# vlongle/pixie

Hardware: AMD Instinct MI355X
Metric: voxels/s (128^3 U-Net fwd) + MPM particle-steps/s (higher is better)
Workload: dtype f32 (operands split fp16 hi+lo, 3 f16 MFMAs/product, fp32 accumulate); 1 GPU; 128^3x64 feature grid -> SegmentationUNet+RegressionUNet forward (+argmax/one-hot combine), 1 scene per GPU per step; grid=128, feature_channels=64, parallelism=scene-parallel x1, executor=c+hip_graph

## Files before the change

### include/pixie_hip.h

```cpp
#ifndef PIXIE_HIP_H
#define PIXIE_HIP_H

#include <stdint.h>

#ifdef __cplusplus
extern "C" {
#endif

const char* pixie_last_error(void);
const char* pixie_build_arch(void);

typedef struct pixie_mpm pixie_mpm;

int pixie_mpm_create(pixie_mpm** out, int n_particles, int n_grid, double grid_lim);
int pixie_mpm_destroy(pixie_mpm* h);
int pixie_mpm_regrid(pixie_mpm* h, int n_grid, double grid_lim, void* stream);

int pixie_mpm_set_field(pixie_mpm* h, const char* name, const void* d_src, int64_t count, void* stream);
int pixie_mpm_get_field(pixie_mpm* h, const char* name, void* d_dst, int64_t count, void* stream);
int pixie_mpm_fill_field(pixie_mpm* h, const char* name, double value, void* stream);

int pixie_mpm_set_scalar(pixie_mpm* h, const char* key, double value);
int pixie_mpm_get_scalar(pixie_mpm* h, const char* key, double* value);

int pixie_mpm_update_mass(pixie_mpm* h, void* stream);
int pixie_mpm_finalize_mu_lam(pixie_mpm* h, int with_bulk, void* stream);
int pixie_mpm_apply_additional_params(pixie_mpm* h, const double point[3], const double size[3], double E,
                                      double nu, double density, int material, void* stream);
int pixie_mpm_apply_additional_params_batch(pixie_mpm* h, int64_t n_boxes, const float* d_boxes, const float* d_params,
                                            const int32_t* d_material, void* stream);

enum { PIXIE_BC_SURFACE = 0, PIXIE_BC_CUBOID = 1, PIXIE_BC_BBOX = 2 };
typedef struct pixie_bc_desc {
    int32_t type;
    int32_t surface_type;
    int32_t reset;
    int32_t pad_;
    double point[3], size[3], velocity[3], normal[3];
    double start_time, end_time, friction;
} pixie_bc_desc;
int pixie_mpm_add_bc(pixie_mpm* h, const pixie_bc_desc* bc);

enum { PIXIE_PM_IMPULSE = 0, PIXIE_PM_TRANSLATION = 1, PIXIE_PM_ROTATION = 2 };
typedef struct pixie_pmod_desc {
    int32_t type;
    int32_t pad_;
    double point[3], size[3];
    double force[3];
    double velocity[3];
    double normal[3], h1[3], h2[3];
    double half_height, radius, rotation_scale, translation_scale;
    double start_time, end_time;
} pixie_pmod_desc;
int pixie_mpm_add_particle_modifier(pixie_mpm* h, const pixie_pmod_desc* pm, void* stream);

int pixie_mpm_step(pixie_mpm* h, double dt, int n_substeps, void* stream);

typedef struct pixie_mpm_batch pixie_mpm_batch;
typedef struct pixie_batch_sched {
    double dt;
    int32_t steps_per_chunk;
    int32_t n_chunks;
    int32_t n_out;
    int32_t pad_;
    double shift[3], scale, mean[3];
    double inv_rotation[9];
    float* d_pos;
    float* d_cov;
} pixie_batch_sched;
int pixie_mpm_batch_create(pixie_mpm_batch** out, pixie_mpm* const* handles, int n_handles);
int pixie_mpm_batch_step(pixie_mpm_batch* b, double dt, int n_substeps, void* stream);
int pixie_mpm_batch_run(pixie_mpm_batch* b, const pixie_batch_sched* per_scene, int n_scenes, void* stream);
typedef struct pixie_batch_splat_out {
    float* d_log_scale;
    float* d_quat;
} pixie_batch_splat_out;
int pixie_mpm_batch_run_splats(pixie_mpm_batch* b, const pixie_batch_sched* per_scene, const pixie_batch_splat_out* splats ,
                               int n_scenes, void* stream);
int pixie_mpm_batch_destroy(pixie_mpm_batch* b);

int pixie_mpm_export_cov(pixie_mpm* h, float* d_cov , void* stream);
int pixie_mpm_export_R(pixie_mpm* h, float* d_R , void* stream);
int pixie_mpm_export_frame(pixie_mpm* h, int n_out, const double shift[3], double scale, const double mean[3],
                           const double inv_rotation[9], float* d_pos , float* d_cov ,
                           void* stream);
int pixie_splat_from_cov(const float* d_cov , int64_t n, float* d_log_scale , float* d_quat ,
                         void* stream);
int pixie_mpm_export_frame_splats(pixie_mpm* h, int n_out, const double shift[3], double scale, const double mean[3],
                                  const double inv_rotation[9], float* d_pos , float* d_cov ,
                                  float* d_log_scale , float* d_quat , void* stream);
int pixie_mpm_out_of_bounds(pixie_mpm* h, int64_t* count, void* stream);


typedef struct pixie_conv_desc {
    const float* d_in0; int32_t c0;
    const float* d_in1; int32_t c1;
    int32_t in_d, in_h, in_w;
    int32_t upsample;
    int32_t stride;
    int32_t ksize;
    const float* d_pro_a; const float* d_pro_b;
    const float* d_gamma; const float* d_beta;
    int32_t act;
    const float* d_w; const float* d_bias;
    int32_t c_out;
    const float* d_residual;
    float* d_out;
    const void* d_w16;
    const uint32_t* d_in_amax0; const uint32_t* d_in_amax1;
    float in_bound;
    float* d_out_stats;
    uint32_t* d_out_amax;
    void* d_workspace;
    int32_t out_d, out_h, out_w;
    const float* d_skip_in0; int32_t skip_c0;
    const float* d_skip_in1; int32_t skip_c1;
    const void* d_skip_w16; const float* d_skip_bias;
    const uint32_t* d_skip_amax0; const uint32_t* d_skip_amax1;
    int32_t w16_subpixel;
} pixie_conv_desc;

int pixie_conv_cout_padded(int c_out);
int pixie_conv_pack_weights(const float* d_w_oidhw, float* d_w_packed, int c_out, int c_in, int ksize, void* stream);
int64_t pixie_conv_packed16_bytes(int c_out, int c_in, int ksize);
int pixie_conv_pack_weights_f16x2(const float* d_w_oidhw, void* d_packed, int c_out, int c_in, int ksize, void* stream);
int64_t pixie_conv_subpixel_bytes(int c_out, int c_in);
int pixie_conv_pack_weights_subpixel(const float* d_w_oidhw, void* d_packed, int c_out, int c_in, void* stream);
int pixie_conv3d_forward(const pixie_conv_desc* desc, void* stream);
int64_t pixie_conv_stats_floats(const pixie_conv_desc* desc);
int64_t pixie_conv_workspace_bytes(const pixie_conv_desc* desc);
int pixie_stats_finalize(const float* d_stats, const pixie_conv_desc* desc, double* d_sums, void* stream);
int pixie_conv_skip_foldable(const pixie_conv_desc* desc);

int pixie_channel_sums(const float* d_x, int channels, int64_t spatial, double* d_sums, void* stream);
int pixie_channel_stats(const float* d_x, int channels, int64_t spatial, double* d_sums, uint32_t* d_amax, void* stream);
int pixie_tensor_amax(const float* d_x, int64_t count, uint32_t* d_slot, void* stream);
int pixie_norm_finalize(const double* d_sums, int channels, int64_t spatial, int mode, int groups, double eps,
                        const float* d_weight, const float* d_bias, float* d_a, float* d_b, void* stream);

int pixie_attention_forward(const float* d_qkv, float* d_out, int channels, int tokens, void* stream);

int pixie_channel_affine(const float* d_x, const float* d_a, const float* d_b, float* d_y, int channels,
                         int64_t spatial, void* stream);

int pixie_voxel_grid_to_ncdhw(const void* d_feat_dhwc_f16, int d, int h, int w, int channels, float* d_out_cdhw, void* stream);

int pixie_projector_conv0(const void* d_feat_dhwc_f16, int64_t voxels, int channels, int n_networks, const void* const* d_w16,
                          const float* const* d_bias, float* const* d_out, int c_out, void* stream);

int pixie_pack_fields(const float* d_cont, const int32_t* d_seg_pred, int64_t n_scenes, int64_t spatial, void* d_wire, int64_t wire_bytes,
                      void* stream);

int pixie_combine_predictions(const float* d_logits, int num_classes, const float* d_cont, int64_t spatial,
                              float* d_combined, int32_t* d_argmax , void* stream);

int pixie_combine_class_ids(const int32_t* d_seg_pred, int num_classes, const float* d_cont, int64_t spatial, float* d_combined,
                            void* stream);

typedef struct pixie_unet pixie_unet;
typedef struct pixie_unet_config {
    int32_t feature_channels, cond_dim, model_channels, num_res_blocks;
    int32_t n_channel_mult; int32_t channel_mult[8];
    int32_t n_attention_resolutions; int32_t attention_resolutions[8];
    int32_t grid_size;
    int32_t out_channels;
    int32_t precision;
} pixie_unet_config;

int pixie_unet_create(pixie_unet** out, const pixie_unet_config* cfg);
int pixie_unet_destroy(pixie_unet* h);
int pixie_unet_param_count(const pixie_unet* h);
int pixie_unet_param_info(const pixie_unet* h, int index, const char** key, int64_t* numel, int32_t* ndim, int64_t shape[5]);
int pixie_unet_set_param(pixie_unet* h, const char* key, const float* d_values, int64_t numel);
int64_t pixie_unet_workspace_bytes(pixie_unet* h, int d, int hh, int w);
int pixie_unet_forward(pixie_unet* h, const float* d_feat, const float* d_proj0, int d, int hh, int w, float* d_out,
                       void* d_workspace, int64_t workspace_bytes, void* stream);
int pixie_unet_set_option(pixie_unet* h, const char* key, int value);

typedef struct pixie_field_desc {
    const float* d_pred;
    const uint8_t* d_mask;
    const float* d_axis_x; const float* d_axis_y; const float* d_axis_z;
    int32_t n_classes, d, h, w;
    double min_spacing;
    double density_min, density_max, E_min, E_max, nu_min, nu_max;
} pixie_field_desc;
int pixie_field_to_particles(const pixie_field_desc* field, const float* d_pos, int n, int k, double nn_distance_threshold,
                             int weighted, int default_material, int default_part_label, float* d_density, float* d_E,
                             float* d_nu, int32_t* d_material, int32_t* d_part_label, float* d_conf, float* d_nearest,
                             void* d_scratch, void* stream);

int pixie_unscale_prediction(const float* d_pred, int channels, int64_t spatial, double density_min, double density_max,
                             double E_min, double E_max, double nu_min, double nu_max, float* d_out, void* stream);
int64_t pixie_field_points_scratch_bytes(const pixie_field_desc* field);
int pixie_field_points(const pixie_field_desc* field, int64_t capacity, float* d_xyz , float* d_density, float* d_E,
                       float* d_nu, int32_t* d_material, float* d_conf, int64_t* d_count, void* d_scratch, void* stream);

int pixie_dbscan_roots(const float* d_pos_sorted, const int32_t* d_orig_index, const int32_t* d_cell_start, int n, int nx, int ny, int nz,
                       const double lo[3], double cell_size, double eps, int min_samples, int32_t* d_core_scratch,
                       int32_t* d_parent_scratch, int32_t* d_root, void* stream);

int pixie_fill_densify(const float* d_pos, const float* d_opacity, const float* d_cov6, int n, int grid_n, double grid_dx,
                       int32_t* d_grid_count, float* d_grid_density, void* stream);
int pixie_fill_dense_cells(int32_t* d_grid_count, const float* d_grid_density, int grid_n, double grid_dx, double density_thres,
                           int max_particles_per_cell, float* d_new_particles , int64_t max_samples,
                           uint64_t* d_counter, uint32_t seed, void* stream);
int pixie_fill_internal_cells(int32_t* d_grid_count, const float* d_grid_density, int grid_n, double grid_dx, int max_particles_per_cell,
                              int exclude_dir, int ray_cast_dir, double threshold, float* d_new_particles, int64_t max_samples,
                              uint64_t* d_counter, uint32_t seed, void* stream);
int pixie_particle_volume(const float* d_pos, int n, int grid_n, double grid_dx, int32_t* d_grid_count_scratch, float* d_vol, void* stream);
int pixie_nearest_particle(const float* d_pos, int n, const float* d_new_pos, int n_new, int32_t* d_nearest, void* stream);

#ifdef PIXIE_DIAG
int pixie_mpm_phase(pixie_mpm* h, int phase, double dt, void* stream);

int pixie_mpm_kernel_times(pixie_mpm* h, double* particle_ms, double* grid_ms, int64_t* n_launches);

int pixie_conv_kernel_variant(const pixie_conv_desc* desc, int* slices);

int pixie_conv_tile_geometry(const pixie_conv_desc* desc, int32_t out[10]);
#endif

#ifdef __cplusplus
}
#endif
#endif
```

### pixie_amd/_lib.py

```python
from __future__ import annotations

import ctypes as C
import os

_HERE = os.path.dirname(os.path.abspath(__file__))
LIB_PATH = os.path.join(_HERE, "libpixie_hip.so")
DIAG_LIB_PATH = os.path.join(_HERE, "libpixie_hip_diag.so")


class PixieHipError(RuntimeError):
    pass


class BCDesc(C.Structure):
    _fields_ = [("type", C.c_int32), ("surface_type", C.c_int32), ("reset", C.c_int32), ("pad_", C.c_int32),
                ("point", C.c_double * 3), ("size", C.c_double * 3), ("velocity", C.c_double * 3),
                ("normal", C.c_double * 3), ("start_time", C.c_double), ("end_time", C.c_double),
                ("friction", C.c_double)]


class PModDesc(C.Structure):
    _fields_ = [("type", C.c_int32), ("pad_", C.c_int32),
                ("point", C.c_double * 3), ("size", C.c_double * 3), ("force", C.c_double * 3),
                ("velocity", C.c_double * 3), ("normal", C.c_double * 3), ("h1", C.c_double * 3),
                ("h2", C.c_double * 3), ("half_height", C.c_double), ("radius", C.c_double),
                ("rotation_scale", C.c_double), ("translation_scale", C.c_double),
                ("start_time", C.c_double), ("end_time", C.c_double)]


class ConvDesc(C.Structure):
    _fields_ = [("d_in0", C.c_void_p), ("c0", C.c_int32),
                ("d_in1", C.c_void_p), ("c1", C.c_int32),
                ("in_d", C.c_int32), ("in_h", C.c_int32), ("in_w", C.c_int32),
                ("upsample", C.c_int32), ("stride", C.c_int32), ("ksize", C.c_int32),
                ("d_pro_a", C.c_void_p), ("d_pro_b", C.c_void_p),
                ("d_gamma", C.c_void_p), ("d_beta", C.c_void_p),
                ("act", C.c_int32),
                ("d_w", C.c_void_p), ("d_bias", C.c_void_p),
                ("c_out", C.c_int32),
                ("d_residual", C.c_void_p), ("d_out", C.c_void_p),
                ("d_w16", C.c_void_p), ("d_in_amax0", C.c_void_p), ("d_in_amax1", C.c_void_p),
                ("in_bound", C.c_float),
                ("d_out_stats", C.c_void_p), ("d_out_amax", C.c_void_p),
                ("d_workspace", C.c_void_p),
                ("out_d", C.c_int32), ("out_h", C.c_int32), ("out_w", C.c_int32),
                ("d_skip_in0", C.c_void_p), ("skip_c0", C.c_int32),
                ("d_skip_in1", C.c_void_p), ("skip_c1", C.c_int32),
                ("d_skip_w16", C.c_void_p), ("d_skip_bias", C.c_void_p),
                ("d_skip_amax0", C.c_void_p), ("d_skip_amax1", C.c_void_p),
                ("w16_subpixel", C.c_int32)]


class UNetConfigC(C.Structure):
    _fields_ = [("feature_channels", C.c_int32), ("cond_dim", C.c_int32), ("model_channels", C.c_int32), ("num_res_blocks", C.c_int32),
                ("n_channel_mult", C.c_int32), ("channel_mult", C.c_int32 * 8),
                ("n_attention_resolutions", C.c_int32), ("attention_resolutions", C.c_int32 * 8),
                ("grid_size", C.c_int32), ("out_channels", C.c_int32), ("precision", C.c_int32)]


class BatchSched(C.Structure):
    _fields_ = [("dt", C.c_double), ("steps_per_chunk", C.c_int32), ("n_chunks", C.c_int32), ("n_out", C.c_int32), ("pad_", C.c_int32),
                ("shift", C.c_double * 3), ("scale", C.c_double), ("mean", C.c_double * 3), ("inv_rotation", C.c_double * 9),
                ("d_pos", C.c_void_p), ("d_cov", C.c_void_p)]


class BatchSplatOut(C.Structure):
    _fields_ = [("d_log_scale", C.c_void_p), ("d_quat", C.c_void_p)]


class FieldDesc(C.Structure):
    _fields_ = [("d_pred", C.c_void_p), ("d_mask", C.c_void_p),
                ("d_axis_x", C.c_void_p), ("d_axis_y", C.c_void_p), ("d_axis_z", C.c_void_p),
                ("n_classes", C.c_int32), ("d", C.c_int32), ("h", C.c_int32), ("w", C.c_int32),
                ("min_spacing", C.c_double),
                ("density_min", C.c_double), ("density_max", C.c_double), ("E_min", C.c_double), ("E_max", C.c_double),
                ("nu_min", C.c_double), ("nu_max", C.c_double)]


_VP, _I, _I64, _D, _S = C.c_void_p, C.c_int, C.c_int64, C.c_double, C.c_char_p
_D3 = C.POINTER(C.c_double)
SIGNATURES = {
    "pixie_last_error": (C.c_char_p, []),
    "pixie_build_arch": (C.c_char_p, []),
    "pixie_mpm_create": (_I, [C.POINTER(_VP), _I, _I, _D]),
    "pixie_mpm_destroy": (_I, [_VP]),
    "pixie_mpm_regrid": (_I, [_VP, _I, _D, _VP]),
    "pixie_mpm_set_field": (_I, [_VP, _S, _VP, _I64, _VP]),
    "pixie_mpm_get_field": (_I, [_VP, _S, _VP, _I64, _VP]),
    "pixie_mpm_fill_field": (_I, [_VP, _S, _D, _VP]),
    "pixie_mpm_set_scalar": (_I, [_VP, _S, _D]),
    "pixie_mpm_get_scalar": (_I, [_VP, _S, C.POINTER(_D)]),
    "pixie_mpm_update_mass": (_I, [_VP, _VP]),
    "pixie_mpm_finalize_mu_lam": (_I, [_VP, _I, _VP]),
    "pixie_mpm_apply_additional_params": (_I, [_VP, _D3, _D3, _D, _D, _D, _I, _VP]),
    "pixie_mpm_apply_additional_params_batch": (_I, [_VP, _I64, _VP, _VP, _VP, _VP]),
    "pixie_mpm_add_bc": (_I, [_VP, C.POINTER(BCDesc)]),
    "pixie_mpm_add_particle_modifier": (_I, [_VP, C.POINTER(PModDesc), _VP]),
    "pixie_mpm_step": (_I, [_VP, _D, _I, _VP]),
    "pixie_mpm_export_cov": (_I, [_VP, _VP, _VP]),
    "pixie_mpm_export_R": (_I, [_VP, _VP, _VP]),
    "pixie_mpm_export_frame": (_I, [_VP, _I, _D3, _D, _D3, C.POINTER(C.c_double), _VP, _VP, _VP]),
    "pixie_mpm_out_of_bounds": (_I, [_VP, C.POINTER(_I64), _VP]),
    "pixie_mpm_batch_create": (_I, [C.POINTER(_VP), C.POINTER(_VP), _I]),
    "pixie_mpm_batch_step": (_I, [_VP, _D, _I, _VP]),
    "pixie_mpm_batch_run": (_I, [_VP, C.POINTER(BatchSched), _I, _VP]),
    "pixie_mpm_batch_run_splats": (_I, [_VP, C.POINTER(BatchSched), C.POINTER(BatchSplatOut), _I, _VP]),
    "pixie_splat_from_cov": (_I, [_VP, _I64, _VP, _VP, _VP]),
    "pixie_mpm_export_frame_splats": (_I, [_VP, _I, _D3, _D, _D3, C.POINTER(C.c_double), _VP, _VP, _VP, _VP, _VP]),
    "pixie_mpm_batch_destroy": (_I, [_VP]),
    "pixie_pack_fields": (_I, [_VP, _VP, _I64, _I64, _VP, _I64, _VP]),
    "pixie_conv_cout_padded": (_I, [_I]),
    "pixie_conv_pack_weights": (_I, [_VP, _VP, _I, _I, _I, _VP]),
    "pixie_conv_packed16_bytes": (_I64, [_I, _I, _I]),
    "pixie_conv_pack_weights_f16x2": (_I, [_VP, _VP, _I, _I, _I, _VP]),
    "pixie_conv_subpixel_bytes": (_I64, [_I, _I]),
    "pixie_conv_pack_weights_subpixel": (_I, [_VP, _VP, _I, _I, _VP]),
    "pixie_conv3d_forward": (_I, [C.POINTER(ConvDesc), _VP]),
    "pixie_conv_stats_floats": (_I64, [C.POINTER(ConvDesc)]),
    "pixie_conv_workspace_bytes": (_I64, [C.POINTER(ConvDesc)]),
    "pixie_stats_finalize": (_I, [_VP, C.POINTER(ConvDesc), _VP, _VP]),
    "pixie_channel_stats": (_I, [_VP, _I, _I64, _VP, _VP, _VP]),
    "pixie_tensor_amax": (_I, [_VP, _I64, _VP, _VP]),
    "pixie_channel_sums": (_I, [_VP, _I, _I64, _VP, _VP]),
    "pixie_norm_finalize": (_I, [_VP, _I, _I64, _I, _I, _D, _VP, _VP, _VP, _VP, _VP]),
    "pixie_attention_forward": (_I, [_VP, _VP, _I, _I, _VP]),
    "pixie_channel_affine": (_I, [_VP, _VP, _VP, _VP, _I, _I64, _VP]),
    "pixie_projector_conv0": (_I, [_VP, _I64, _I, _I, C.POINTER(_VP), C.POINTER(_VP), C.POINTER(_VP), _I, _VP]),
    "pixie_conv_skip_foldable": (_I, [C.POINTER(ConvDesc)]),
    "pixie_unet_create": (_I, [C.POINTER(_VP), C.POINTER(UNetConfigC)]),
    "pixie_unet_destroy": (_I, [_VP]),
    "pixie_unet_param_count": (_I, [_VP]),
    "pixie_unet_param_info": (_I, [_VP, _I, C.POINTER(_S), C.POINTER(_I64), C.POINTER(C.c_int32), C.POINTER(_I64)]),
    "pixie_unet_set_param": (_I, [_VP, _S, _VP, _I64]),
    "pixie_unet_workspace_bytes": (_I64, [_VP, _I, _I, _I]),
    "pixie_unet_set_option": (_I, [_VP, _S, _I]),
    "pixie_unet_forward": (_I, [_VP, _VP, _VP, _I, _I, _I, _VP, _VP, _I64, _VP]),
    "pixie_combine_class_ids": (_I, [_VP, _I, _VP, _I64, _VP, _VP]),
    "pixie_combine_predictions": (_I, [_VP, _I, _VP, _I64, _VP, _VP, _VP]),
    "pixie_voxel_grid_to_ncdhw": (_I, [_VP, _I, _I, _I, _I, _VP, _VP]),
    "pixie_unscale_prediction": (_I, [_VP, _I, _I64, _D, _D, _D, _D, _D, _D, _VP, _VP]),
    "pixie_field_points_scratch_bytes": (_I64, [C.POINTER(FieldDesc)]),
    "pixie_field_points": (_I, [C.POINTER(FieldDesc), _I64, _VP, _VP, _VP, _VP, _VP, _VP, _VP, _VP, _VP]),
    "pixie_fill_densify": (_I, [_VP, _VP, _VP, _I, _I, _D, _VP, _VP, _VP]),
    "pixie_fill_dense_cells": (_I, [_VP, _VP, _I, _D, _D, _I, _VP, _I64, _VP, C.c_uint32, _VP]),
    "pixie_fill_internal_cells": (_I, [_VP, _VP, _I, _D, _I, _I, _I, _D, _VP, _I64, _VP, C.c_uint32, _VP]),
    "pixie_particle_volume": (_I, [_VP, _I, _I, _D, _VP, _VP, _VP]),
    "pixie_nearest_particle": (_I, [_VP, _I, _VP, _I, _VP, _VP]),
    "pixie_dbscan_roots": (_I, [_VP, _VP, _VP, _I, _I, _I, _I, C.POINTER(_D), _D, _D, _I, _VP, _VP, _VP, _VP]),
    "pixie_field_to_particles": (_I, [C.POINTER(FieldDesc), _VP, _I, _I, _D, _I, _I, _I, _VP, _VP, _VP, _VP, _VP, _VP, _VP, _VP, _VP]),
}

DIAG_SIGNATURES = {
    "pixie_mpm_phase": (_I, [_VP, _I, _D, _VP]),
    "pixie_mpm_kernel_times": (_I, [_VP, C.POINTER(_D), C.POINTER(_D), C.POINTER(_I64)]),
    "pixie_conv_kernel_variant": (C.c_int, [C.POINTER(ConvDesc), C.POINTER(C.c_int)]),
    "pixie_conv_tile_geometry": (C.c_int, [C.POINTER(ConvDesc), C.POINTER(C.c_int32)]),
}

_libs = {}


def load(diag: bool = False):
    if diag in _libs:
        return _libs[diag]
    path = DIAG_LIB_PATH if diag else LIB_PATH
    if not os.path.exists(path):
        raise PixieHipError(
            f"{path} not found: build it with `python -m pixie_amd.build` (hipcc, gfx950). "
            "pixie_amd has no CPU fallback.")
    import torch
    lib = C.CDLL(path)
    for name, (res, args) in list(SIGNATURES.items()) + (list(DIAG_SIGNATURES.items()) if diag else []):
        fn = getattr(lib, name)
        fn.restype = res
        fn.argtypes = args
    _libs[diag] = lib
    return lib


def check(rc: int, what: str = "", lib=None):
    if rc != 0:
        msg = (lib or load()).pixie_last_error()
        raise PixieHipError(f"{what}: {msg.decode() if msg else 'unknown error'}")


def current_stream_ptr():
    import torch
    try:
        return C.c_void_p(torch._C._cuda_getCurrentRawStream(torch.cuda.current_device()))
    except AttributeError:
        return C.c_void_p(torch.cuda.current_stream().cuda_stream)


def d3(v):
    return (C.c_double * 3)(*[float(x) for x in v])
```

### pixie_amd/csrc/conv3d_f16x3.hip

```cpp
#include <hip/hip_runtime.h>

#include <cstdlib>
#include <map>
#include <string>
#include <type_traits>

#include "../../include/pixie_hip.h"
#include "common.h"

namespace pixie {

typedef float f32x16 __attribute__((ext_vector_type(16)));
typedef _Float16 f16x8 __attribute__((ext_vector_type(8)));

constexpr int kW16HeaderU4 = 4;

struct Conv16Args {
    const float* in0; const float* in1;
    int c0, cin;
    int ID, IH, IW;
    int LD, LH, LW;
    int ups;
    int stride;
    int OD, OH, OW;
    const float* pro_a; const float* pro_b; const float* gamma; const float* beta;
    int act;
    const uint4* w16;
    const float* wf;
    const float* bias;
    int cout, coutp;
    const float* residual; float* out;
    const unsigned* amax0; const unsigned* amax1;
    float in_bound;
    int TX, TY, TZ, lTX, lTY;
    int tiles_x, tiles_y, tiles_z, n_tiles;
    int HX, HY, HZ, HYX, CS;
    unsigned mHX, mHYX;
    float* stats; unsigned* out_amax;
    float* partial; int chunks_per_slice;
    int epi_lds;
    const float* sk_in0; const float* sk_in1;
    int sk_c0, sk_cin;
    const uint4* sk_w16; const float* sk_bias;
    const unsigned* sk_amax0; const unsigned* sk_amax1;
};

__device__ __forceinline__ int fast_div16(int n, int d, unsigned magic) {
    return (d == 1) ? n : (int)__umulhi((unsigned)n, magic);
}
__device__ __forceinline__ float act16(float t, int act) {
    if (act == 1) return t > 0.0f ? t : 0.02f * t;
    if (act == 2) return t / (1.0f + __expf(-t));
    return t;
}
__device__ __forceinline__ int scale_exponent(float bound) {
    const unsigned bits = __float_as_uint(bound);
    const int eb = (int)((bits >> 23) & 0xffu) - 127;
    if (!(bound > 0.0f) || eb > 100) return 0;
    int e = 14 - eb;
    return e > 100 ? 100 : (e < -100 ? -100 : e);
}
__device__ __forceinline__ float pow2i(int e) { return __uint_as_float((unsigned)(e + 127) << 23); }

template <int KS, int MB, int NB, bool EX = false, bool SP = false>
__device__ __forceinline__ void conv3d_f16x3_body(const Conv16Args& A) {
    static_assert(!SP || (KS == 3 && NB == 4 && !EX), "sub-pixel path: 3^3, two x parities x two voxel blocks per wave");
    extern __shared__ uint4 smem16[];
    constexpr int PAD = (KS == 3) ? 1 : 0;
    constexpr int NW = 4, NT = 64 * NW;
    const int bufsz = 4 * A.CS;

    const int tid = threadIdx.x;
    const int lane = tid & 63;
    const int wave = tid >> 6;
    const int kh = lane >> 5;
    const int l31 = lane & 31;

    int t = blockIdx.x;
    {
        const int per = (A.n_tiles + 7) >> 3;
        const int cand = (t & 7) * per + (t >> 3);
        if ((A.n_tiles & 7) == 0) t = cand;
    }
    int par = 0;
    if constexpr (SP) { par = t & 3; t >>= 2; }
    const int py = par & 1, pz = par >> 1;
    const int tx = t % A.tiles_x; t /= A.tiles_x;
    const int ty = t % A.tiles_y;
    const int tz = t / A.tiles_y;
    const int ox0 = tx * A.TX, oy0 = ty * A.TY, oz0 = tz * A.TZ;
    const int cout0 = blockIdx.y * (MB * 32);
    const int lx0 = SP ? ox0 - 1 : ox0 * A.stride - PAD;
    const int ly0 = SP ? oy0 - 1 + py : oy0 * A.stride - PAD;
    const int lz0 = SP ? oz0 - 1 + pz : oz0 * A.stride - PAD;
    const size_t ISP = (size_t)A.ID * A.IH * A.IW;
    const size_t OSP = (size_t)A.OD * A.OH * A.OW;

    int voff[NB];
    int ovox[NB];
    bool valid[NB];
#pragma unroll
    for (int nb = 0; nb < NB; ++nb) {
        if constexpr (SP) {
            const int px = nb >> 1;
            const int j = (wave * 2 + (nb & 1)) * 32 + l31;
            int x = j & (A.TX - 1);
            int y = (j >> A.lTX) & (A.TY - 1);
            int z = j >> (A.lTX + A.lTY);
            const int gx = 2 * (ox0 + x) + px, gy = 2 * (oy0 + y) + py, gz = 2 * (oz0 + z) + pz;
            const bool v = (z < A.TZ) && (gx < A.OW) && (gy < A.OH) && (gz < A.OD);
            if (!v) { x = 0; y = 0; z = 0; }
            voff[nb] = (z * A.HY + y) * A.HX + x + px + kh * A.CS;
            ovox[nb] = v ? (gz * A.OH + gy) * A.OW + gx : 0;
            valid[nb] = v;
            continue;
        }
        const int j = (wave * NB + nb) * 32 + l31;
        int x = j & (A.TX - 1);
        int y = (j >> A.lTX) & (A.TY - 1);
        int z = j >> (A.lTX + A.lTY);
        const bool v = (z < A.TZ) && (ox0 + x < A.OW) && (oy0 + y < A.OH) && (oz0 + z < A.OD);
        if (!v) { x = 0; y = 0; z = 0; }
        voff[nb] = ((z * A.HY + y) * A.HX + x) * A.stride + kh * A.CS;
        ovox[nb] = ((oz0 + z) * A.OH + (oy0 + y)) * A.OW + ox0 + x;
        valid[nb] = v;
    }

    float bound = A.in_bound;
    if (A.amax0) {
        bound = __uint_as_float(*A.amax0);
        if (A.amax1) bound = fmaxf(bound, __uint_as_float(*A.amax1));
    }
    const int ex = EX ? 0 : scale_exponent(bound);
    const float sx = pow2i(ex);

    f32x16 acc[MB][NB];
#pragma unroll
    for (int mb = 0; mb < MB; ++mb)
#pragma unroll
        for (int nb = 0; nb < NB; ++nb)
#pragma unroll
            for (int r = 0; r < 16; ++r) acc[mb][nb][r] = 0.0f;

    const int KG = A.cin >> 3;
    const size_t tap_stride = (size_t)KG * A.coutp;
    const size_t plane = (size_t)(SP ? 64 : KS * KS * KS) * tap_stride;
    const uint4* wHi = A.w16 + kW16HeaderU4 + (size_t)kh * A.coutp + cout0 + l31 + (size_t)(par * 16) * tap_stride;
    const uint4* wLo = wHi + plane;
    const float* wF = A.wf + (size_t)kh * A.coutp + cout0 + l31;

    constexpr int TAPS = KS * KS * KS;
    auto stage_chunk = [&](int c_base, uint4* buf, int stid, int nthr) {
        uint4* bHi = buf;
        uint4* bLo = buf + 2 * A.CS;
        float pa[16], pb[16];
        {
            float pv = 0.0f;
            if (A.pro_a) pv = (lane & 16) ? A.pro_b[c_base + (lane & 15)] : A.pro_a[c_base + (lane & 15)];
#pragma unroll
            for (int j = 0; j < 16; ++j) {
                pa[j] = __int_as_float(__builtin_amdgcn_readlane(__float_as_int(pv), j));
                pb[j] = __int_as_float(__builtin_amdgcn_readlane(__float_as_int(pv), 16 + j));
            }
        }
        const bool has_aff = A.gamma != nullptr;
        for (int v0 = stid; v0 < A.CS; v0 += 2 * nthr) {
            float val[2][16];
            float gm[2], bt[2];
            int sidx[2];
            bool ok[2];
#pragma unroll
            for (int u = 0; u < 2; ++u) {
                const int vox = v0 + u * nthr;
                int rem = vox;
                const int hz = fast_div16(rem, A.HYX, A.mHYX);
                rem -= hz * A.HYX;
                const int hy = fast_div16(rem, A.HX, A.mHX);
                const int hx = rem - hy * A.HX;
                const int lz = lz0 + hz, ly = ly0 + hy, lx = lx0 + hx;
                ok[u] = vox < A.CS && (unsigned)lz < (unsigned)A.LD && (unsigned)ly < (unsigned)A.LH && (unsigned)lx < (unsigned)A.LW;
                sidx[u] = ok[u] ? ((lz >> A.ups) * A.IH + (ly >> A.ups)) * A.IW + (lx >> A.ups) : 0;
            }
#pragma unroll
            for (int u = 0; u < 2; ++u) {
#pragma unroll
                for (int j = 0; j < 16; ++j) {
                    const int cg = c_base + j;
                    const float* src = (cg < A.c0) ? (A.in0 + (size_t)cg * ISP) : (A.in1 + (size_t)(cg - A.c0) * ISP);
                    val[u][j] = src[sidx[u]];
                }
                gm[u] = 1.0f; bt[u] = 0.0f;
                if (has_aff) { gm[u] = A.gamma[sidx[u]]; bt[u] = A.beta[sidx[u]]; }
            }
            auto convert = [&](auto has_pro, auto act_c) {
#pragma unroll
                for (int u = 0; u < 2; ++u) {
                    const int vox = v0 + u * nthr;
                    if (EX) {
                        float* bF = reinterpret_cast<float*>(buf);
#pragma unroll
                        for (int j = 0; j < 16; ++j) {
                            float t = val[u][j];
                            if (decltype(has_pro)::value) t = t * pa[j] + pb[j];
                            t = t * gm[u] + bt[u];
                            const float sc = ok[u] ? act16(t, decltype(act_c)::value) : 0.0f;
                            if (vox < A.CS) bF[j * A.CS + vox] = sc;
                        }
                        continue;
                    }
                    f16x8 vh[2], vl[2];
#pragma unroll
                    for (int j = 0; j < 16; ++j) {
                        float t = val[u][j];
                        if (decltype(has_pro)::value) t = t * pa[j] + pb[j];
                        t = t * gm[u] + bt[u];
                        const float sc = ok[u] ? act16(t, decltype(act_c)::value) * sx : 0.0f;
                        const _Float16 h = (_Float16)sc;
                        vh[j >> 3][j & 7] = h;
                        vl[j >> 3][j & 7] = (_Float16)(sc - (float)h);
                    }
                    if (vox < A.CS) {
                        bHi[vox] = __builtin_bit_cast(uint4, vh[0]);
                        bHi[A.CS + vox] = __builtin_bit_cast(uint4, vh[1]);
                        bLo[vox] = __builtin_bit_cast(uint4, vl[0]);
                        bLo[A.CS + vox] = __builtin_bit_cast(uint4, vl[1]);
                    }
                }
            };
            using T = std::true_type; using F = std::false_type;
            if (A.pro_a) {
                if (A.act == 1) convert(T{}, std::integral_constant<int, 1>{});
                else if (A.act == 2) convert(T{}, std::integral_constant<int, 2>{});
                else convert(T{}, std::integral_constant<int, 0>{});
            } else {
                if (A.act == 1) convert(F{}, std::integral_constant<int, 1>{});
                else if (A.act == 2) convert(F{}, std::integral_constant<int, 2>{});
                else convert(F{}, std::integral_constant<int, 0>{});
            }
        }
    };
    auto mfma_chunk = [&](int c_base, const uint4* buf) {
        __builtin_amdgcn_s_setprio(3);
        if constexpr (EX) {
            const float* ldsF = reinterpret_cast<const float*>(buf);
            const size_t tapw = (size_t)A.cin * A.coutp;
            const float* wc = wF + (size_t)c_base * A.coutp;
            float a[8][MB], an[8][MB];
#pragma unroll
            for (int kp = 0; kp < 8; ++kp)
#pragma unroll
                for (int mb = 0; mb < MB; ++mb) a[kp][mb] = wc[(size_t)(2 * kp) * A.coutp + mb * 32];
#pragma unroll 1
            for (int zy = 0; zy < KS * KS; ++zy) {
                const int dz = zy / KS, dy = zy - dz * KS;
                const int rowoff = (dz * A.HY + dy) * A.HX;
#pragma unroll
                for (int dx = 0; dx < KS; ++dx) {
                    const int tap = zy * KS + dx;
                    const int nxt = (tap + 1 < TAPS) ? tap + 1 : tap;
#pragma unroll
                    for (int kp = 0; kp < 8; ++kp)
#pragma unroll
                        for (int mb = 0; mb < MB; ++mb) an[kp][mb] = wc[(size_t)nxt * tapw + (size_t)(2 * kp) * A.coutp + mb * 32];
                    __builtin_amdgcn_sched_barrier(0);
#pragma unroll
                    for (int kp = 0; kp < 8; ++kp) {
                        float b[NB];
#pragma unroll
                        for (int nb = 0; nb < NB; ++nb) b[nb] = ldsF[voff[nb] + rowoff + dx + 2 * kp * A.CS];
#pragma unroll
                        for (int mb = 0; mb < MB; ++mb)
#pragma unroll
                            for (int nb = 0; nb < NB; ++nb)
                                acc[mb][nb] = __builtin_amdgcn_mfma_f32_32x32x2f32(a[kp][mb], b[nb], acc[mb][nb], 0, 0, 0);
                    }
#pragma unroll
                    for (int kp = 0; kp < 8; ++kp)
#pragma unroll
                        for (int mb = 0; mb < MB; ++mb) a[kp][mb] = an[kp][mb];
                }
            }
            __builtin_amdgcn_s_setprio(0);
            return;
        }
        const uint4* ldsHi = buf;
        const uint4* ldsLo = buf + 2 * A.CS;
        const uint4* wh = wHi + (size_t)(c_base >> 3) * A.coutp;
        const uint4* wl = wLo + (size_t)(c_base >> 3) * A.coutp;
        if constexpr (SP) {
            f16x8 ah[MB], al[MB];
#pragma unroll
            for (int mb = 0; mb < MB; ++mb) {
                ah[mb] = __builtin_bit_cast(f16x8, wh[mb * 32]);
                al[mb] = __builtin_bit_cast(f16x8, wl[mb * 32]);
            }
#pragma unroll 1
            for (int zy = 0; zy < 4; ++zy) {
                const int rowoff = ((zy >> 1) * A.HY + (zy & 1)) * A.HX;
                const int zyn = zy < 3 ? zy + 1 : 3;
#pragma unroll
                for (int q = 0; q < 4; ++q) {
                    const int ex = q >> 1, px = q & 1;
                    const size_t nxt = (q < 3) ? (size_t)(((q + 1) & 1) * 8 + zy * 2 + ((q + 1) >> 1)) * tap_stride : (size_t)(zyn * 2) * tap_stride;
                    f16x8 ahn[MB], aln[MB];
#pragma unroll
                    for (int mb = 0; mb < MB; ++mb) {
                        ahn[mb] = __builtin_bit_cast(f16x8, wh[nxt + mb * 32]);
                        aln[mb] = __builtin_bit_cast(f16x8, wl[nxt + mb * 32]);
                    }
                    __builtin_amdgcn_sched_barrier(0);
                    f16x8 bh[2], bl[2];
#pragma unroll
                    for (int s = 0; s < 2; ++s) {
                        bh[s] = __builtin_bit_cast(f16x8, ldsHi[voff[px * 2 + s] + rowoff + ex]);
                        bl[s] = __builtin_bit_cast(f16x8, ldsLo[voff[px * 2 + s] + rowoff + ex]);
                    }
#pragma unroll
                    for (int mb = 0; mb < MB; ++mb)
#pragma unroll
                        for (int s = 0; s < 2; ++s)
                            acc[mb][px * 2 + s] = __builtin_amdgcn_mfma_f32_32x32x16_f16(al[mb], bh[s], acc[mb][px * 2 + s], 0, 0, 0);
#pragma unroll
                    for (int mb = 0; mb < MB; ++mb)
#pragma unroll
                        for (int s = 0; s < 2; ++s)
                            acc[mb][px * 2 + s] = __builtin_amdgcn_mfma_f32_32x32x16_f16(ah[mb], bl[s], acc[mb][px * 2 + s], 0, 0, 0);
#pragma unroll
                    for (int mb = 0; mb < MB; ++mb)
#pragma unroll
                        for (int s = 0; s < 2; ++s)
                            acc[mb][px * 2 + s] = __builtin_amdgcn_mfma_f32_32x32x16_f16(ah[mb], bh[s], acc[mb][px * 2 + s], 0, 0, 0);
#pragma unroll
                    for (int mb = 0; mb < MB; ++mb) { ah[mb] = ahn[mb]; al[mb] = aln[mb]; }
                }
            }
            __builtin_amdgcn_s_setprio(0);
            return;
        }
        f16x8 ah[MB], al[MB];
#pragma unroll
        for (int mb = 0; mb < MB; ++mb) {
            ah[mb] = __builtin_bit_cast(f16x8, wh[mb * 32]);
            al[mb] = __builtin_bit_cast(f16x8, wl[mb * 32]);
        }
#pragma unroll 1
        for (int zy = 0; zy < KS * KS; ++zy) {
            const int dz = zy / KS, dy = zy - dz * KS;
            const int rowoff = (dz * A.HY + dy) * A.HX;
#pragma unroll
            for (int dx = 0; dx < KS; ++dx) {
                const int tap = zy * KS + dx;
                const int nxt = (tap + 1 < TAPS) ? tap + 1 : tap;
                f16x8 ahn[MB], aln[MB];
#pragma unroll
                for (int mb = 0; mb < MB; ++mb) {
                    ahn[mb] = __builtin_bit_cast(f16x8, wh[(size_t)nxt * tap_stride + mb * 32]);
                    aln[mb] = __builtin_bit_cast(f16x8, wl[(size_t)nxt * tap_stride + mb * 32]);
                }
                __builtin_amdgcn_sched_barrier(0);
                f16x8 bh[NB], bl[NB];
#pragma unroll
                for (int nb = 0; nb < NB; ++nb) {
                    bh[nb] = __builtin_bit_cast(f16x8, ldsHi[voff[nb] + rowoff + dx]);
                    bl[nb] = __builtin_bit_cast(f16x8, ldsLo[voff[nb] + rowoff + dx]);
                }
#pragma unroll
                for (int mb = 0; mb < MB; ++mb)
#pragma unroll
                    for (int nb = 0; nb < NB; ++nb)
                        acc[mb][nb] = __builtin_amdgcn_mfma_f32_32x32x16_f16(al[mb], bh[nb], acc[mb][nb], 0, 0, 0);
#pragma unroll
                for (int mb = 0; mb < MB; ++mb)
#pragma unroll
                    for (int nb = 0; nb < NB; ++nb)
                        acc[mb][nb] = __builtin_amdgcn_mfma_f32_32x32x16_f16(ah[mb], bl[nb], acc[mb][nb], 0, 0, 0);
#pragma unroll
                for (int mb = 0; mb < MB; ++mb)
#pragma unroll
                    for (int nb = 0; nb < NB; ++nb)
                        acc[mb][nb] = __builtin_amdgcn_mfma_f32_32x32x16_f16(ah[mb], bh[nb], acc[mb][nb], 0, 0, 0);
#pragma unroll
                for (int mb = 0; mb < MB; ++mb) { ah[mb] = ahn[mb]; al[mb] = aln[mb]; }
            }
        }
        __builtin_amdgcn_s_setprio(0);
    };

    float inv2 = 0.0f;
    {
        const int c_begin = A.partial ? (int)blockIdx.z * A.chunks_per_slice * 16 : 0;
        const int c_end = A.partial ? min(A.cin, c_begin + A.chunks_per_slice * 16) : A.cin;
        for (int c_base = c_begin; c_base < c_end; c_base += 16) {
            __syncthreads();
            stage_chunk(c_base, smem16, tid, NT);
            __syncthreads();
            mfma_chunk(c_base, smem16);
        }
        if (!EX && !SP && A.sk_w16) {
            float sb = __uint_as_float(*A.sk_amax0);
            if (A.sk_amax1) sb = fmaxf(sb, __uint_as_float(*A.sk_amax1));
            const int ex2 = scale_exponent(sb);
            const float sx2 = pow2i(ex2);
            const float inv_main = __uint_as_float(A.w16[0].x) * pow2i(-ex);
            inv2 = __uint_as_float(A.sk_w16[0].x) * pow2i(-ex2);
            const float ratio = inv_main / inv2;
#pragma unroll
            for (int mb = 0; mb < MB; ++mb)
#pragma unroll
                for (int nb = 0; nb < NB; ++nb)
#pragma unroll
                    for (int r = 0; r < 16; ++r) acc[mb][nb][r] *= ratio;
            const int KG2 = A.sk_cin >> 3;
            const uint4* w2Hi = A.sk_w16 + kW16HeaderU4 + (size_t)kh * A.coutp + cout0 + l31;
            const uint4* w2Lo = w2Hi + (size_t)KG2 * A.coutp;
            const int centre = (KS == 3) ? (A.HY + 1) * A.HX + 1 : 0;
            const int tvox = A.TX * A.TY * A.TZ;
            for (int c2 = 0; c2 < A.sk_cin; c2 += 16) {
                f16x8 ah[MB], al[MB];
#pragma unroll
                for (int mb = 0; mb < MB; ++mb) {
                    ah[mb] = __builtin_bit_cast(f16x8, w2Hi[(size_t)(c2 >> 3) * A.coutp + mb * 32]);
                    al[mb] = __builtin_bit_cast(f16x8, w2Lo[(size_t)(c2 >> 3) * A.coutp + mb * 32]);
                }
                __syncthreads();
                uint4* bHi = smem16;
                uint4* bLo = smem16 + 2 * A.CS;
                for (int j = tid; j < tvox; j += NT) {
                    const int x = j & (A.TX - 1), y = (j >> A.lTX) & (A.TY - 1), z = j >> (A.lTX + A.lTY);
                    const bool okv = (ox0 + x < A.OW) && (oy0 + y < A.OH) && (oz0 + z < A.OD);
                    const size_t sidx = okv ? ((size_t)(oz0 + z) * A.IH + (oy0 + y)) * A.IW + ox0 + x : 0;
                    float val[16];
#pragma unroll
                    for (int q = 0; q < 16; ++q) {
                        const int cg = c2 + q;
                        const float* src = (cg < A.sk_c0) ? (A.sk_in0 + (size_t)cg * ISP) : (A.sk_in1 + (size_t)(cg - A.sk_c0) * ISP);
                        val[q] = src[sidx];
                    }
                    f16x8 vh[2], vl[2];
#pragma unroll
                    for (int q = 0; q < 16; ++q) {
                        const float sc = okv ? val[q] * sx2 : 0.0f;
                        const _Float16 hq = (_Float16)sc;
                        vh[q >> 3][q & 7] = hq;
                        vl[q >> 3][q & 7] = (_Float16)(sc - (float)hq);
                    }
                    const int slot = (z * A.HY + y) * A.HX + x + centre;
                    bHi[slot] = __builtin_bit_cast(uint4, vh[0]);
                    bHi[A.CS + slot] = __builtin_bit_cast(uint4, vh[1]);
                    bLo[slot] = __builtin_bit_cast(uint4, vl[0]);
                    bLo[A.CS + slot] = __builtin_bit_cast(uint4, vl[1]);
                }
                __syncthreads();
                f16x8 bh[NB], bl[NB];
#pragma unroll
                for (int nb = 0; nb < NB; ++nb) {
                    bh[nb] = __builtin_bit_cast(f16x8, bHi[voff[nb] + centre]);
                    bl[nb] = __builtin_bit_cast(f16x8, bLo[voff[nb] + centre]);
                }
#pragma unroll
                for (int mb = 0; mb < MB; ++mb)
#pragma unroll
                    for (int nb = 0; nb < NB; ++nb)
                        acc[mb][nb] = __builtin_amdgcn_mfma_f32_32x32x16_f16(al[mb], bh[nb], acc[mb][nb], 0, 0, 0);
#pragma unroll
                for (int mb = 0; mb < MB; ++mb)
#pragma unroll
                    for (int nb = 0; nb < NB; ++nb)
                        acc[mb][nb] = __builtin_amdgcn_mfma_f32_32x32x16_f16(ah[mb], bl[nb], acc[mb][nb], 0, 0, 0);
#pragma unroll
                for (int mb = 0; mb < MB; ++mb)
#pragma unroll
                    for (int nb = 0; nb < NB; ++nb)
                        acc[mb][nb] = __builtin_amdgcn_mfma_f32_32x32x16_f16(ah[mb], bh[nb], acc[mb][nb], 0, 0, 0);
            }
        }
    }

    const float inv = EX ? 1.0f : (A.sk_w16 ? inv2 : __uint_as_float(A.w16[0].x) * pow2i(-ex));
    if (A.partial) {
        float* dst = A.partial + (size_t)blockIdx.z * A.cout * OSP;
#pragma unroll
        for (int mb = 0; mb < MB; ++mb)
#pragma unroll
            for (int r = 0; r < 16; ++r) {
                const int co = cout0 + mb * 32 + (r & 3) + 8 * (r >> 2) + 4 * kh;
                if (co < A.cout) {
#pragma unroll
                    for (int nb = 0; nb < NB; ++nb)
                        if (valid[nb]) dst[(size_t)co * OSP + ovox[nb]] = acc[mb][nb][r] * inv;
                }
            }
        return;
    }
    float* red = reinterpret_cast<float*>(smem16);
    float wmax = 0.0f;
    const bool full = SP ? (A.epi_lds && cout0 + MB * 32 <= A.cout && (A.TX & 1) == 0 && (A.OW & 3) == 0 && NW * 64 <= A.TX * A.TY * A.TZ &&
                            2 * (ox0 + A.TX) <= A.OW && 2 * (oy0 + A.TY) <= A.OH && 2 * (oz0 + A.TZ) <= A.OD)
                         : (A.epi_lds && cout0 + MB * 32 <= A.cout && (A.TX & 3) == 0 && (A.OW & 3) == 0 && NW * NB * 32 <= A.TX * A.TY * A.TZ &&
                            ox0 + A.TX <= A.OW && oy0 + A.TY <= A.OH && oz0 + A.TZ <= A.OD);
    if (full) {
        __syncthreads();
        constexpr int LDO = NB * 32 + 4;
        float* ldsO = reinterpret_cast<float*>(smem16) + wave * (32 * LDO);
        red = reinterpret_cast<float*>(smem16) + NW * 32 * LDO;
        constexpr int LPR = NB * 8;
        constexpr int RPI = 32 / LPR;
        const int rsub = l31 / LPR, colq = 4 * (l31 % LPR), nbq = colq >> 5;
        const int jq = SP ? wave * 64 + (colq >> 1) : (wave * NB + nbq) * 32 + (colq & 31);
        const int xq = jq & (A.TX - 1), yq = (jq >> A.lTX) & (A.TY - 1), zq = jq >> (A.lTX + A.lTY);
        const size_t ovq = SP ? ((size_t)(2 * (oz0 + zq) + pz) * A.OH + (2 * (oy0 + yq) + py)) * A.OW + 2 * (ox0 + xq)
                              : ((size_t)(oz0 + zq) * A.OH + (oy0 + yq)) * A.OW + ox0 + xq;
        const bool has_res = A.residual != nullptr, has_stats = A.stats != nullptr;
#pragma unroll
        for (int mb = 0; mb < MB; ++mb) {
#pragma unroll
            for (int r = 0; r < 16; ++r)
#pragma unroll
                for (int nb = 0; nb < NB; ++nb)
                    ldsO[((r & 3) + 8 * (r >> 2) + 4 * kh) * LDO + (SP ? 2 * ((nb & 1) * 32 + l31) + (nb >> 1) : nb * 32 + l31)] = acc[mb][nb][r];
#pragma unroll 4
            for (int it = 0; it < 16 / RPI; ++it) {
                const int rowl = (2 * it + kh) * RPI + rsub;
                const int co = cout0 + mb * 32 + rowl;
                const float4 a4 = *reinterpret_cast<const float4*>(ldsO + rowl * LDO + colq);
                const float bv = (A.bias ? A.bias[co] : 0.0f) + (A.sk_bias ? A.sk_bias[co] : 0.0f);
                const size_t o = (size_t)co * OSP + ovq;
                float4 v4;
                v4.x = a4.x * inv + bv; v4.y = a4.y * inv + bv; v4.z = a4.z * inv + bv; v4.w = a4.w * inv + bv;
                if (has_res) {
                    const float4 r4 = *reinterpret_cast<const float4*>(A.residual + o);
                    v4.x += r4.x; v4.y += r4.y; v4.z += r4.z; v4.w += r4.w;
                }
                *reinterpret_cast<float4*>(A.out + o) = v4;
                if (has_stats) {
                    float s1 = (v4.x + v4.y) + (v4.z + v4.w);
                    float s2 = (v4.x * v4.x + v4.y * v4.y) + (v4.z * v4.z + v4.w * v4.w);
                    wmax = fmaxf(fmaxf(wmax, fmaxf(fabsf(v4.x), fabsf(v4.y))), fmaxf(fabsf(v4.z), fabsf(v4.w)));
#pragma unroll
                    for (int off = LPR / 2; off > 0; off >>= 1) { s1 += __shfl_xor(s1, off, 64); s2 += __shfl_xor(s2, off, 64); }
                    if ((l31 % LPR) == 0) { red[(wave * MB * 32 + mb * 32 + rowl) * 2] = s1; red[(wave * MB * 32 + mb * 32 + rowl) * 2 + 1] = s2; }
                }
            }
        }
    } else {
    if (A.stats) __syncthreads();
#pragma unroll
    for (int mb = 0; mb < MB; ++mb) {
#pragma unroll
        for (int r = 0; r < 16; ++r) {
            const int row = mb * 32 + (r & 3) + 8 * (r >> 2) + 4 * kh;
            const int co = cout0 + row;
            float s1 = 0.0f, s2 = 0.0f;
            if (co < A.cout) {
                const float bv = (A.bias ? A.bias[co] : 0.0f) + (A.sk_bias ? A.sk_bias[co] : 0.0f);
#pragma unroll
                for (int nb = 0; nb < NB; ++nb) {
                    if (valid[nb]) {
                        const size_t o = (size_t)co * OSP + ovox[nb];
                        float val = acc[mb][nb][r] * inv + bv;
                        if (A.residual) val += A.residual[o];
                        A.out[o] = val;
                        s1 += val; s2 += val * val; wmax = fmaxf(wmax, fabsf(val));
                    }
                }
            }
            if (A.stats) {
#pragma unroll
                for (int off = 16; off > 0; off >>= 1) { s1 += __shfl_xor(s1, off, 64); s2 += __shfl_xor(s2, off, 64); }
                if (l31 == 0) { red[(wave * MB * 32 + row) * 2] = s1; red[(wave * MB * 32 + row) * 2 + 1] = s2; }
            }
        }
    }
    }
    if (A.stats) {
        __syncthreads();
        if (tid < MB * 32 * 2) {
            float t = red[tid];
#pragma unroll
            for (int w = 1; w < NW; ++w) t += red[w * MB * 64 + tid];
            A.stats[((size_t)blockIdx.x * A.coutp + cout0) * 2 + tid] = t;
        }
        if (A.out_amax) {
#pragma unroll
            for (int off = 32; off > 0; off >>= 1) wmax = fmaxf(wmax, __shfl_xor(wmax, off, 64));
            if (lane == 0 && wmax > 0.0f) atomicMax(A.out_amax, __float_as_uint(wmax));
        }
    }
}

template <int KS, int MB, int NB>
__global__ __launch_bounds__(256, 2) void conv3d_f16x3_kernel(Conv16Args A) {
    conv3d_f16x3_body<KS, MB, NB>(A);
}
template <int KS, int MB, int NB>
__global__ __launch_bounds__(256, 2) void conv3d_exact_kernel(Conv16Args A) {
    conv3d_f16x3_body<KS, MB, NB, true>(A);
}
template <int MB>
__global__ __launch_bounds__(256, 2) void conv3d_f16x3_subpixel_kernel(Conv16Args A) {
    conv3d_f16x3_body<3, MB, 4, false, true>(A);
}
__global__ __launch_bounds__(256, 2) void conv3d_f16x3_c64_fullres_kernel(Conv16Args A) {
    conv3d_f16x3_body<3, 2, 4>(A);
}

__global__ __launch_bounds__(256) void stats_finalize_kernel(const float* __restrict__ stats, int n_tiles, int coutp, double* __restrict__ sums) {
    const int c = blockIdx.x;
    double s1 = 0.0, s2 = 0.0;
    for (int t = threadIdx.x; t < n_tiles; t += 256) {
        const float2 v = *reinterpret_cast<const float2*>(stats + ((size_t)t * coutp + c) * 2);
        s1 += v.x; s2 += v.y;
    }
    for (int off = 32; off > 0; off >>= 1) { s1 += __shfl_down(s1, off, 64); s2 += __shfl_down(s2, off, 64); }
    __shared__ double r[8];
    if ((threadIdx.x & 63) == 0) { r[2 * (threadIdx.x >> 6)] = s1; r[2 * (threadIdx.x >> 6) + 1] = s2; }
    __syncthreads();
    if (threadIdx.x == 0) { sums[2 * c] = r[0] + r[2] + r[4] + r[6]; sums[2 * c + 1] = r[1] + r[3] + r[5] + r[7]; }
}

__global__ __launch_bounds__(256) void splitk_reduce_kernel(const float* __restrict__ partial, int slices, long n_elems, long osp,
                                                            const float* __restrict__ bias, const float* residual, float* out) {
    const long i = (long)blockIdx.x * 256 + threadIdx.x;
    if (i >= n_elems) return;
    float v = partial[i];
    for (int s = 1; s < slices; ++s) v += partial[(size_t)s * n_elems + i];
    if (bias) v += bias[i / osp];
    if (residual) v += residual[i];
    out[i] = v;
}

__global__ __launch_bounds__(256) void amax_kernel(const float* __restrict__ x, long n, unsigned* __restrict__ slot) {
    float m = 0.0f;
    const long stride = (long)gridDim.x * 256 * 4;
    long i = ((long)blockIdx.x * 256 + threadIdx.x) * 4;
    if ((reinterpret_cast<size_t>(x) & 15) == 0) {
        for (; i + 3 < n; i += stride) {
            const float4 v = *reinterpret_cast<const float4*>(x + i);
            m = fmaxf(fmaxf(m, fabsf(v.x)), fmaxf(fabsf(v.y), fmaxf(fabsf(v.z), fabsf(v.w))));
        }
        for (long k = i; k < n && k < i + 4; ++k) m = fmaxf(m, fabsf(x[k]));
    } else {
        for (long k = (long)blockIdx.x * 256 + threadIdx.x; k < n; k += (long)gridDim.x * 256) m = fmaxf(m, fabsf(x[k]));
    }
    for (int off = 32; off > 0; off >>= 1) m = fmaxf(m, __shfl_down(m, off, 64));
    if ((threadIdx.x & 63) == 0 && m > 0.0f) atomicMax(slot, __float_as_uint(m));
}

__global__ void pack_weights_f16x2_kernel(const float* __restrict__ src, uint4* __restrict__ dst, int cout, int cin, int taps,
                                          int coutp, const unsigned* __restrict__ amax_bits) {
    const int KG = cin >> 3;
    const long total = (long)taps * KG * coutp;
    const long i = (long)blockIdx.x * blockDim.x + threadIdx.x;
    const int e = scale_exponent(__uint_as_float(*amax_bits));
    if (i == 0) dst[0] = make_uint4(__float_as_uint(pow2i(-e)), (unsigned)cout, (unsigned)cin, (unsigned)taps);
    if (i >= total) return;
    const float s = pow2i(e);
    const int co = (int)(i % coutp);
    const long row = i / coutp;
    const int kg = (int)(row % KG);
    const int tap = (int)(row / KG);
    f16x8 vh, vl;
#pragma unroll
    for (int j = 0; j < 8; ++j) {
        float w = 0.0f;
        if (co < cout) w = src[((long)co * cin + kg * 8 + j) * taps + tap] * s;
        const _Float16 h = (_Float16)w;
        vh[j] = h;
        vl[j] = (_Float16)(w - (float)h);
    }
    dst[kW16HeaderU4 + i] = __builtin_bit_cast(uint4, vh);
    dst[kW16HeaderU4 + total + i] = __builtin_bit_cast(uint4, vl);
}

__device__ __forceinline__ float subpixel_weight(const float* __restrict__ w27, int par, int tap) {
    int lo[3], hi[3];
#pragma unroll
    for (int ax = 0; ax < 3; ++ax) {
        const int p = (par >> (2 - ax)) & 1, e = (tap >> (2 - ax)) & 1;
        lo[ax] = e ? (p ? 2 : 1) : 0;
        hi[ax] = e ? 2 : (p ? 1 : 0);
    }
    float sum = 0.0f;
    for (int dz = lo[0]; dz <= hi[0]; ++dz)
        for (int dy = lo[1]; dy <= hi[1]; ++dy)
            for (int dx = lo[2]; dx <= hi[2]; ++dx) sum += w27[(dz * 3 + dy) * 3 + dx];
    return sum;
}
__global__ __launch_bounds__(256) void subpixel_amax_kernel(const float* __restrict__ src, long pairs, unsigned* __restrict__ slot) {
    const long i = (long)blockIdx.x * 256 + threadIdx.x;
    float m = 0.0f;
    if (i < pairs)
        for (int pt = 0; pt < 64; ++pt) m = fmaxf(m, fabsf(subpixel_weight(src + i * 27, pt >> 3, pt & 7)));
    for (int off = 32; off > 0; off >>= 1) m = fmaxf(m, __shfl_down(m, off, 64));
    if ((threadIdx.x & 63) == 0 && m > 0.0f) atomicMax(slot, __float_as_uint(m));
}
__global__ void pack_weights_subpixel_kernel(const float* __restrict__ src, uint4* __restrict__ dst, int cout, int cin, int coutp,
                                             const unsigned* __restrict__ amax_bits) {
    const int KG = cin >> 3;
    const long total = 64L * KG * coutp;
    const long i = (long)blockIdx.x * blockDim.x + threadIdx.x;
    const int e = scale_exponent(__uint_as_float(*amax_bits));
    if (i == 0) dst[0] = make_uint4(__float_as_uint(pow2i(-e)), (unsigned)cout, (unsigned)cin, 64u);
    if (i >= total) return;
    const float s = pow2i(e);
    const int co = (int)(i % coutp);
    const long row = i / coutp;
    const int kg = (int)(row % KG);
    const int pt = (int)(row / KG);
    f16x8 vh, vl;
#pragma unroll
    for (int j = 0; j < 8; ++j) {
        float w = 0.0f;
        if (co < cout) w = subpixel_weight(src + ((long)co * cin + kg * 8 + j) * 27, pt >> 3, pt & 7) * s;
        const _Float16 h = (_Float16)w;
        vh[j] = h;
        vl[j] = (_Float16)(w - (float)h);
    }
    dst[kW16HeaderU4 + i] = __builtin_bit_cast(uint4, vh);
    dst[kW16HeaderU4 + total + i] = __builtin_bit_cast(uint4, vl);
}

static unsigned magic_of16(int d) { return d <= 1 ? 0u : (unsigned)((0x100000000ull + (unsigned long long)d - 1) / (unsigned long long)d); }
static int ilog2_16(int v) { int l = 0; while ((1 << l) < v) ++l; return l; }
static int pow2_le16(int v, int cap) { int p = 1; while (p * 2 <= v && p * 2 <= cap) p *= 2; return p; }

template <int MB>
static int launch_subpixel(const Conv16Args& a, size_t lds_bytes, dim3 grid, hipStream_t st) {
    auto kern = conv3d_f16x3_subpixel_kernel<MB>;
    PX_CHECK_HIP(allow_max_dynamic_lds(reinterpret_cast<const void*>(kern)));
    hipLaunchKernelGGL(kern, grid, dim3(256), lds_bytes, st, a);
    PX_CHECK_HIP(hipGetLastError());
    return 0;
}

static bool conv16_subpixel(const pixie_conv_desc* d) {
    return d->d_w16 && d->w16_subpixel && d->upsample == 1 && d->ksize == 3 && d->stride == 1;
}

template <int KS, int MB, int NB>
static int launch_f16x3(const Conv16Args& a, size_t lds_bytes, dim3 grid, hipStream_t st) {
    auto kern = conv3d_f16x3_kernel<KS, MB, NB>;
    PX_CHECK_HIP(allow_max_dynamic_lds(reinterpret_cast<const void*>(kern)));
    hipLaunchKernelGGL(kern, grid, dim3(256), lds_bytes, st, a);
    PX_CHECK_HIP(hipGetLastError());
    return 0;
}

static void conv16_tiling(const pixie_conv_desc* d, Conv16Args& a, int& MB_out, int& NB_out, int* slices_out = nullptr) {
    a.ID = d->in_d; a.IH = d->in_h; a.IW = d->in_w;
    a.ups = d->upsample;
    a.LD = a.ID << a.ups; a.LH = a.IH << a.ups; a.LW = a.IW << a.ups;
    const int pad = d->ksize == 3 ? 1 : 0;
    a.stride = d->stride;
    a.OD = (a.LD + 2 * pad - d->ksize) / a.stride + 1; a.OH = (a.LH + 2 * pad - d->ksize) / a.stride + 1; a.OW = (a.LW + 2 * pad - d->ksize) / a.stride + 1;
    if (d->out_d > 0) a.OD = std::min(a.OD, (int)d->out_d);
    if (d->out_h > 0) a.OH = std::min(a.OH, (int)d->out_h);
    if (d->out_w > 0) a.OW = std::min(a.OW, (int)d->out_w);
    a.cout = d->c_out; a.coutp = pixie_conv_cout_padded(d->c_out);
    const int chunks = (d->c0 + d->c1) / 16;
    const int smax = d->d_workspace ? std::min(8, chunks / 2) : 1;
    if (conv16_subpixel(d)) {
        a.ups = 0; a.LD = a.ID; a.LH = a.IH; a.LW = a.IW;
        const int SD = (a.OD + 1) / 2, SH = (a.OH + 1) / 2, SW = (a.OW + 1) / 2;
        a.TX = pow2_le16(SW, 32);
        a.TY = pow2_le16(SH, std::max(1, std::min(4, 256 / a.TX)));
        a.TZ = std::max(1, std::min(SD, 256 / (a.TX * a.TY)));
        a.lTX = ilog2_16(a.TX); a.lTY = ilog2_16(a.TY);
        a.tiles_x = (SW + a.TX - 1) / a.TX; a.tiles_y = (SH + a.TY - 1) / a.TY; a.tiles_z = (SD + a.TZ - 1) / a.TZ;
        a.n_tiles = 4 * a.tiles_x * a.tiles_y * a.tiles_z;
        a.HX = a.TX + 2; a.HY = a.TY + 1; a.HZ = a.TZ + 1;
        a.HYX = a.HY * a.HX; a.CS = a.HZ * a.HYX;
        a.mHX = magic_of16(a.HX); a.mHYX = magic_of16(a.HYX);
        MB_out = (a.coutp >= 64) ? 2 : 1; NB_out = 4;
        int sl = 1;
        const long wgs = (long)a.n_tiles * ((a.coutp + MB_out * 32 - 1) / (MB_out * 32));
        while (sl * 2 <= smax && wgs * sl < 512) sl *= 2;
        if (slices_out) *slices_out = sl;
        return;
    }
    const long ovol = (long)a.OD * a.OH * a.OW;
    int MB = (a.coutp >= 64) ? 2 : 1;
    int NB = (a.stride == 2) ? 1 : 4;
    auto n_wg = [&](int mb, int nb) {
        const long tiles = (ovol + 128L * nb - 1) / (128L * nb);
        return tiles * ((a.coutp + mb * 32 - 1) / (mb * 32));
    };
    int slices = 1;
    if (smax >= 2 && n_wg(MB, NB) < 512) {
        bool found = false;
        for (int nb = NB; nb >= 1 && !found; nb /= 2) {
            for (int sl = 1; sl <= smax; sl *= 2)
                if (n_wg(MB, nb) * sl >= 512) { NB = nb; slices = sl; found = true; break; }
        }
        if (!found) { NB = 1; slices = 1; while (slices * 2 <= smax) slices *= 2; }
    } else {
        while (n_wg(MB, NB) < 512 && NB > 1) NB /= 2;
        if (n_wg(MB, NB) < 512 && MB > 1) MB = 1;
    }
    if (slices_out) *slices_out = slices;
    const int tile_vox = 128 * NB;
    a.TX = pow2_le16(a.OW, 32);
    a.TY = pow2_le16(a.OH, std::max(1, std::min(4, tile_vox / a.TX)));
    a.TZ = std::max(1, std::min(a.OD, tile_vox / (a.TX * a.TY)));
    a.lTX = ilog2_16(a.TX); a.lTY = ilog2_16(a.TY);
    a.tiles_x = (a.OW + a.TX - 1) / a.TX; a.tiles_y = (a.OH + a.TY - 1) / a.TY; a.tiles_z = (a.OD + a.TZ - 1) / a.TZ;
    a.n_tiles = a.tiles_x * a.tiles_y * a.tiles_z;
    a.HX = (a.TX - 1) * a.stride + d->ksize; a.HY = (a.TY - 1) * a.stride + d->ksize; a.HZ = (a.TZ - 1) * a.stride + d->ksize;
    a.HYX = a.HY * a.HX; a.CS = a.HZ * a.HYX;
    a.mHX = magic_of16(a.HX); a.mHYX = magic_of16(a.HYX);

    MB_out = MB; NB_out = NB;
}

static size_t conv16_epi_bytes(int MB, int NB) { return ((size_t)4 * 32 * (NB * 32 + 4) + (size_t)4 * MB * 32 * 2) * sizeof(float); }
static bool conv16_epi_lds(int MB, int NB, int slices) { return slices == 1 && conv16_epi_bytes(MB, NB) <= 80 * 1024; }

static void conv16_exact_tiling(const pixie_conv_desc* d, Conv16Args& a, int& MB_out, int& NB_out) {
    pixie_conv_desc probe = *d;
    probe.d_workspace = nullptr;
    probe.w16_subpixel = 0;
    int slices = 1;
    conv16_tiling(&probe, a, MB_out, NB_out, &slices);
}

int conv3d_f16x3_forward(const pixie_conv_desc* d, hipStream_t st) {
    PX_REQUIRE(d->stride == 1 || (d->stride == 2 && d->ksize == 3 && !d->upsample), "f16x3 conv: stride must be 1, or 2 for a 3^3 kernel");
    const int cin = d->c0 + d->c1;
    PX_REQUIRE(cin % 16 == 0 && d->c0 % 8 == 0, "f16x3 conv: c_in must be a multiple of 16 (got %d+%d)", d->c0, d->c1);
    PX_REQUIRE(d->d_in_amax0 != nullptr || d->in_bound > 0.0f, "f16x3 conv: needs d_in_amax0 or a positive in_bound");
    PX_REQUIRE(d->c1 == 0 || d->d_in_amax0 == nullptr || d->d_in_amax1 != nullptr, "f16x3 conv: second input needs its own amax slot");
    Conv16Args a{};
    a.in0 = d->d_in0; a.in1 = d->d_in1; a.c0 = d->c0; a.cin = cin;
    a.ID = d->in_d; a.IH = d->in_h; a.IW = d->in_w;
    a.ups = d->upsample;
    a.LD = a.ID << a.ups; a.LH = a.IH << a.ups; a.LW = a.IW << a.ups;
    const int pad = d->ksize == 3 ? 1 : 0;
    a.stride = d->stride;
    a.OD = (a.LD + 2 * pad - d->ksize) / a.stride + 1; a.OH = (a.LH + 2 * pad - d->ksize) / a.stride + 1; a.OW = (a.LW + 2 * pad - d->ksize) / a.stride + 1;
    if (d->out_d > 0) a.OD = std::min(a.OD, (int)d->out_d);
    if (d->out_h > 0) a.OH = std::min(a.OH, (int)d->out_h);
    if (d->out_w > 0) a.OW = std::min(a.OW, (int)d->out_w);
    a.pro_a = d->d_pro_a; a.pro_b = d->d_pro_b; a.gamma = d->d_gamma; a.beta = d->d_beta; a.act = d->act;
    a.w16 = reinterpret_cast<const uint4*>(d->d_w16); a.bias = d->d_bias; a.cout = d->c_out; a.coutp = pixie_conv_cout_padded(d->c_out);
    a.residual = d->d_residual; a.out = d->d_out;
    a.amax0 = d->d_in_amax0; a.amax1 = (d->c1 > 0) ? d->d_in_amax1 : nullptr; a.in_bound = d->in_bound;
    a.stats = d->d_out_stats; a.out_amax = d->d_out_amax;

    int MB = 0, NB = 0, slices = 1;
    const bool sp = d->w16_subpixel != 0;
    PX_REQUIRE(!sp || (conv16_subpixel(d) && !d->d_skip_w16), "f16x3 conv: sub-pixel weights need upsample = 1, ksize = 3, stride = 1 and no folded skip");
    conv16_tiling(d, a, MB, NB, &slices);
    if (d->d_skip_w16) {
        const int scin = d->skip_c0 + d->skip_c1;
        PX_REQUIRE(pixie_conv_skip_foldable(d), "f16x3 conv: this launch cannot fold a skip convolution (pixie_conv_skip_foldable)");
        PX_REQUIRE(d->d_skip_in0 && d->d_skip_amax0 && (d->skip_c1 == 0 || (d->d_skip_in1 && d->d_skip_amax1)), "f16x3 conv: folded skip needs its inputs and their amax slots");
        a.sk_in0 = d->d_skip_in0; a.sk_in1 = d->d_skip_in1; a.sk_c0 = d->skip_c0; a.sk_cin = scin;
        a.sk_w16 = reinterpret_cast<const uint4*>(d->d_skip_w16); a.sk_bias = d->d_skip_bias;
        a.sk_amax0 = d->d_skip_amax0; a.sk_amax1 = d->skip_c1 > 0 ? d->d_skip_amax1 : nullptr;
    }
    if (slices > 1) {
        a.partial = static_cast<float*>(d->d_workspace);
        a.chunks_per_slice = (cin / 16 + slices - 1) / slices;
        a.stats = nullptr; a.out_amax = nullptr;
    }

    size_t lds = (size_t)4 * a.CS * sizeof(uint4);
    PX_REQUIRE(lds <= 160 * 1024, "f16x3 conv: tile needs %zu B of LDS", lds);
    if (conv16_epi_lds(MB, NB, slices)) { a.epi_lds = 1; lds = std::max(lds, conv16_epi_bytes(MB, NB)); }
    const dim3 grid((unsigned)a.n_tiles, (unsigned)((a.coutp + MB * 32 - 1) / (MB * 32)), (unsigned)slices);
    if (slices > 1) {
        int rc = 1;
        if (sp) {
            rc = (MB == 2) ? launch_subpixel<2>(a, lds, grid, st) : launch_subpixel<1>(a, lds, grid, st);
        } else {
#define PX_CONV16_SK(KS_, MB_, NB_) \
            if (d->ksize == KS_ && MB == MB_ && NB == NB_) rc = launch_f16x3<KS_, MB_, NB_>(a, lds, grid, st);
            PX_CONV16_SK(3, 2, 4) PX_CONV16_SK(3, 2, 2) PX_CONV16_SK(3, 2, 1) PX_CONV16_SK(3, 1, 4) PX_CONV16_SK(3, 1, 2) PX_CONV16_SK(3, 1, 1)
            PX_CONV16_SK(1, 2, 4) PX_CONV16_SK(1, 2, 2) PX_CONV16_SK(1, 2, 1) PX_CONV16_SK(1, 1, 4) PX_CONV16_SK(1, 1, 2) PX_CONV16_SK(1, 1, 1)
#undef PX_CONV16_SK
        }
        if (rc) return rc;
        const long osp = (long)a.OD * a.OH * a.OW, n_elems = (long)a.cout * osp;
        hipLaunchKernelGGL(splitk_reduce_kernel, dim3((unsigned)((n_elems + 255) / 256)), dim3(256), 0, st, a.partial, slices, n_elems, osp,
                           a.bias, a.residual, a.out);
        PX_CHECK_HIP(hipGetLastError());
        return 0;
    }
    if (sp) return (MB == 2) ? launch_subpixel<2>(a, lds, grid, st) : launch_subpixel<1>(a, lds, grid, st);
    if (d->ksize == 3 && MB == 2 && NB == 4 && cin == 64 && d->c_out == 64 && d->stride == 1 && !d->upsample && d->c1 == 0 && !a.sk_w16 &&
        (long)a.OD * a.OH * a.OW >= 128L * 128 * 128) {
        auto kern = conv3d_f16x3_c64_fullres_kernel;
        PX_CHECK_HIP(allow_max_dynamic_lds(reinterpret_cast<const void*>(kern)));
        hipLaunchKernelGGL(kern, grid, dim3(256), lds, st, a);
        PX_CHECK_HIP(hipGetLastError());
        return 0;
    }
#define PX_CONV16_CASE(KS_, MB_, NB_) \
    if (d->ksize == KS_ && MB == MB_ && NB == NB_) return launch_f16x3<KS_, MB_, NB_>(a, lds, grid, st);
    PX_CONV16_CASE(3, 2, 4) PX_CONV16_CASE(3, 2, 2) PX_CONV16_CASE(3, 2, 1)
    PX_CONV16_CASE(3, 1, 4) PX_CONV16_CASE(3, 1, 2) PX_CONV16_CASE(3, 1, 1)
    PX_CONV16_CASE(1, 2, 4) PX_CONV16_CASE(1, 2, 2) PX_CONV16_CASE(1, 2, 1)
    PX_CONV16_CASE(1, 1, 4) PX_CONV16_CASE(1, 1, 2) PX_CONV16_CASE(1, 1, 1)
#undef PX_CONV16_CASE
    return set_error("f16x3 conv: no kernel variant for ksize=%d MB=%d NB=%d", d->ksize, MB, NB);
}

template <int KS, int MB, int NB>
static int launch_exact(const Conv16Args& a, size_t lds_bytes, dim3 grid, hipStream_t st) {
    auto kern = conv3d_exact_kernel<KS, MB, NB>;
    PX_CHECK_HIP(allow_max_dynamic_lds(reinterpret_cast<const void*>(kern)));
    hipLaunchKernelGGL(kern, grid, dim3(256), lds_bytes, st, a);
    PX_CHECK_HIP(hipGetLastError());
    return 0;
}

bool conv3d_exact_tiled_ok(const pixie_conv_desc* d) {
    const int cin = d->c0 + d->c1;
    return cin % 16 == 0 && (d->stride == 1 || (d->stride == 2 && d->ksize == 3 && !d->upsample)) && getenv("PIXIE_CONV_EXACT_V1") == nullptr;
}

int conv3d_exact_forward(const pixie_conv_desc* d, hipStream_t st) {
    Conv16Args a{};
    a.in0 = d->d_in0; a.in1 = d->d_in1; a.c0 = d->c0; a.cin = d->c0 + d->c1;
    a.pro_a = d->d_pro_a; a.pro_b = d->d_pro_b; a.gamma = d->d_gamma; a.beta = d->d_beta; a.act = d->act;
    a.wf = d->d_w; a.bias = d->d_bias;
    a.residual = d->d_residual; a.out = d->d_out;
    a.in_bound = 1.0f;
    int MB = 0, NB = 0;
    conv16_exact_tiling(d, a, MB, NB);
    size_t lds = (size_t)4 * a.CS * sizeof(uint4);
    PX_REQUIRE(lds <= 160 * 1024, "exact conv: tile needs %zu B of LDS", lds);
    if (conv16_epi_lds(MB, NB, 1)) { a.epi_lds = 1; lds = std::max(lds, conv16_epi_bytes(MB, NB)); }
    const dim3 grid((unsigned)a.n_tiles, (unsigned)((a.coutp + MB * 32 - 1) / (MB * 32)), 1u);
#define PX_CONVEX_CASE(KS_, MB_, NB_) \
    if (d->ksize == KS_ && MB == MB_ && NB == NB_) return launch_exact<KS_, MB_, NB_>(a, lds, grid, st);
    PX_CONVEX_CASE(3, 2, 4) PX_CONVEX_CASE(3, 2, 2) PX_CONVEX_CASE(3, 2, 1)
    PX_CONVEX_CASE(3, 1, 4) PX_CONVEX_CASE(3, 1, 2) PX_CONVEX_CASE(3, 1, 1)
    PX_CONVEX_CASE(1, 2, 4) PX_CONVEX_CASE(1, 2, 2) PX_CONVEX_CASE(1, 2, 1)
    PX_CONVEX_CASE(1, 1, 4) PX_CONVEX_CASE(1, 1, 2) PX_CONVEX_CASE(1, 1, 1)
#undef PX_CONVEX_CASE
    return set_error("exact conv: no kernel variant for ksize=%d MB=%d NB=%d", d->ksize, MB, NB);
}

}

using namespace pixie;

extern "C" int64_t pixie_conv_stats_floats(const pixie_conv_desc* d) {
    if (!d || !d->d_w16 || !(d->stride == 1 || (d->stride == 2 && d->ksize == 3)) || (d->ksize != 1 && d->ksize != 3)) return 0;
    Conv16Args a{};
    int MB = 0, NB = 0, slices = 1;
    conv16_tiling(d, a, MB, NB, &slices);
    return slices > 1 ? 0 : (int64_t)a.n_tiles * a.coutp * 2;
}

extern "C" int64_t pixie_conv_workspace_bytes(const pixie_conv_desc* d) {
    if (!d || !d->d_w16 || !(d->stride == 1 || (d->stride == 2 && d->ksize == 3)) || (d->ksize != 1 && d->ksize != 3)) return 0;
    pixie_conv_desc probe = *d;
    probe.d_workspace = reinterpret_cast<void*>(1);
    Conv16Args a{};
    int MB = 0, NB = 0, slices = 1;
    conv16_tiling(&probe, a, MB, NB, &slices);
    return slices > 1 ? (int64_t)slices * a.cout * a.OD * a.OH * a.OW * (int64_t)sizeof(float) : 0;
}

#ifdef PIXIE_DIAG
extern "C" int pixie_conv_kernel_variant(const pixie_conv_desc* d, int* slices_out) {
    if (slices_out) *slices_out = 1;
    if (!d || !d->d_w16 || !(d->stride == 1 || (d->stride == 2 && d->ksize == 3)) || (d->ksize != 1 && d->ksize != 3)) return 0;
    Conv16Args a{};
    int MB = 0, NB = 0, slices = 1;
    conv16_tiling(d, a, MB, NB, &slices);
    if (slices_out) *slices_out = slices;
    if (conv16_subpixel(d)) return 8300 + MB * 10 + NB;
    if (d->ksize == 3 && MB == 2 && NB == 4 && d->c0 + d->c1 == 64 && d->c_out == 64 && d->stride == 1 && !d->upsample && d->c1 == 0 && !d->d_skip_w16 &&
        (long)a.OD * a.OH * a.OW >= 128L * 128 * 128)
        return 9324;
    return d->ksize * 100 + MB * 10 + NB;
}

extern "C" int pixie_conv_tile_geometry(const pixie_conv_desc* d, int32_t out[10]) {
    if (!d || !out || (d->ksize != 1 && d->ksize != 3) || !(d->stride == 1 || (d->stride == 2 && d->ksize == 3 && !d->upsample))) return 1;
    if ((d->c0 + d->c1) % 16 != 0 || (d->d_w16 && d->c0 % 8 != 0)) return 1;
    if (!d->d_w16 && !conv3d_exact_tiled_ok(d)) return 1;
    Conv16Args a{};
    int MB = 0, NB = 0, slices = 1;
    if (d->d_w16) conv16_tiling(d, a, MB, NB, &slices);
    else conv16_exact_tiling(d, a, MB, NB);
    const int32_t v[10] = {a.TX, a.TY, a.TZ, a.tiles_x, a.tiles_y, a.tiles_z, conv16_epi_lds(MB, NB, slices) ? 1 : 0, slices, MB, NB};
    for (int i = 0; i < 10; ++i) out[i] = v[i];
    return 0;
}
#endif

extern "C" int pixie_conv_skip_foldable(const pixie_conv_desc* d) {
    if (!d || !d->d_w16 || d->stride != 1 || d->upsample || (d->ksize != 1 && d->ksize != 3)) return 0;
    const int scin = d->skip_c0 + d->skip_c1;
    if (scin <= 0 || scin % 16 != 0 || d->skip_c0 % 8 != 0 || (d->c0 + d->c1) % 16 != 0 || d->c0 % 8 != 0) return 0;
    Conv16Args a{};
    int MB = 0, NB = 0, slices = 1;
    conv16_tiling(d, a, MB, NB, &slices);
    return slices == 1 ? 1 : 0;
}

extern "C" int pixie_stats_finalize(const float* d_stats, const pixie_conv_desc* d, double* d_sums, void* stream) {
    PX_REQUIRE(d_stats && d && d_sums, "pixie_stats_finalize: null argument");
    Conv16Args a{};
    int MB = 0, NB = 0;
    conv16_tiling(d, a, MB, NB);
    hipLaunchKernelGGL(stats_finalize_kernel, dim3((unsigned)d->c_out), dim3(256), 0, as_stream(stream), d_stats, a.n_tiles, a.coutp, d_sums);
    PX_CHECK_HIP(hipGetLastError());
    return 0;
}

extern "C" int64_t pixie_conv_packed16_bytes(int c_out, int c_in, int ksize) {
    if (c_out <= 0 || c_in <= 0 || c_in % 8 != 0 || (ksize != 1 && ksize != 3)) return 0;
    const int64_t taps = (int64_t)ksize * ksize * ksize;
    return ((int64_t)kW16HeaderU4 + 2 * taps * (c_in / 8) * pixie_conv_cout_padded(c_out)) * (int64_t)sizeof(uint4);
}

extern "C" int pixie_tensor_amax(const float* d_x, int64_t count, uint32_t* d_slot, void* stream) {
    PX_REQUIRE(d_x && d_slot && count > 0, "pixie_tensor_amax: bad arguments");
    const int blocks = (int)std::min<int64_t>(2048, (count + 1023) / 1024);
    hipLaunchKernelGGL(amax_kernel, dim3(blocks), dim3(256), 0, as_stream(stream), d_x, (long)count, d_slot);
    PX_CHECK_HIP(hipGetLastError());
    return 0;
}

extern "C" int pixie_conv_pack_weights_f16x2(const float* d_w, void* d_packed, int c_out, int c_in, int ksize, void* stream) {
    PX_REQUIRE(d_w && d_packed && c_out > 0 && c_in > 0 && c_in % 8 == 0 && (ksize == 1 || ksize == 3),
               "pixie_conv_pack_weights_f16x2: bad arguments (c_in must be a multiple of 8)");
    hipStream_t st = as_stream(stream);
    const int taps = ksize * ksize * ksize;
    const int coutp = pixie_conv_cout_padded(c_out);
    unsigned* slot = reinterpret_cast<unsigned*>(d_packed) + 15;
    PX_CHECK_HIP(hipMemsetAsync(d_packed, 0, kW16HeaderU4 * sizeof(uint4), st));
    if (pixie_tensor_amax(d_w, (int64_t)c_out * c_in * taps, slot, stream)) return 1;
    const long total = (long)taps * (c_in / 8) * coutp;
    hipLaunchKernelGGL(pack_weights_f16x2_kernel, dim3(cdiv(total, 256)), dim3(256), 0, st, d_w, reinterpret_cast<uint4*>(d_packed), c_out,
                       c_in, taps, coutp, slot);
    PX_CHECK_HIP(hipGetLastError());
    return 0;
}

extern "C" int64_t pixie_conv_subpixel_bytes(int c_out, int c_in) {
    if (c_out <= 0 || c_in <= 0 || c_in % 16 != 0) return 0;
    return ((int64_t)kW16HeaderU4 + 2 * 64 * (int64_t)(c_in / 8) * pixie_conv_cout_padded(c_out)) * (int64_t)sizeof(uint4);
}

extern "C" int pixie_conv_pack_weights_subpixel(const float* d_w, void* d_packed, int c_out, int c_in, void* stream) {
    PX_REQUIRE(d_w && d_packed && c_out > 0 && c_in > 0 && c_in % 16 == 0,
               "pixie_conv_pack_weights_subpixel: bad arguments (c_in must be a multiple of 16)");
    hipStream_t st = as_stream(stream);
    const int coutp = pixie_conv_cout_padded(c_out);
    unsigned* slot = reinterpret_cast<unsigned*>(d_packed) + 15;
    PX_CHECK_HIP(hipMemsetAsync(d_packed, 0, kW16HeaderU4 * sizeof(uint4), st));
    const long pairs = (long)c_out * c_in;
    hipLaunchKernelGGL(subpixel_amax_kernel, dim3(cdiv(pairs, 256)), dim3(256), 0, st, d_w, pairs, slot);
    PX_CHECK_HIP(hipGetLastError());
    const long total = 64L * (c_in / 8) * coutp;
    hipLaunchKernelGGL(pack_weights_subpixel_kernel, dim3(cdiv(total, 256)), dim3(256), 0, st, d_w, reinterpret_cast<uint4*>(d_packed), c_out,
                       c_in, coutp, slot);
    PX_CHECK_HIP(hipGetLastError());
    return 0;
}
```

### pixie_amd/csrc/unet_exec.hip

```cpp
#include <hip/hip_runtime.h>

#include <algorithm>
#include <cmath>
#include <cstdlib>
#include <cstring>
#include <map>
#include <memory>
#include <stdexcept>
#include <string>
#include <tuple>
#include <unordered_map>
#include <vector>

#include "../../include/pixie_hip.h"
#include "common.h"

namespace pixie {
int channel_stats_prezeroed(const float* d_x, int channels, int64_t spatial, double* d_sums, uint32_t* d_amax, hipStream_t st);
int norm_finalize_cat(const double* d_sums0, int c0, const double* d_sums1, int c1, int64_t spatial, int mode, int groups, double eps,
                      const float* d_weight, const float* d_bias, float* d_a, float* d_b, hipStream_t st);
namespace {

enum { ACT_NONE = 0, ACT_LEAKY = 1, ACT_SILU = 2 };
enum Kind { CONV_IN, RES, DOWN, ATTN, UP };

struct Blk { Kind kind; std::string prefix; int cin, cout, sp; };
struct Plan {
    std::vector<std::vector<Blk>> in_blocks, out_blocks;
    std::vector<Blk> middle;
    int out_sp = 0;
};

struct Err : std::runtime_error { using std::runtime_error::runtime_error; };
[[noreturn]] void fail(const char* fmt, ...) {
    char buf[512];
    va_list ap; va_start(ap, fmt); vsnprintf(buf, sizeof buf, fmt, ap); va_end(ap);
    throw Err(buf);
}
void ok(int rc, const char* what) { if (rc != 0) fail("%s: %s", what, pixie_last_error()); }

bool has(const std::vector<int>& v, int x) { for (int e : v) if (e == x) return true; return false; }

struct Cfg {
    int feature_channels, cond_dim, model_channels, num_res_blocks;
    std::vector<int> mult, attn;
    int grid_size, out_channels, precision;
    bool has_projector() const { return feature_channels != cond_dim; }
    int projector_hidden() const { return feature_channels > cond_dim ? 128 : 0; }
};

Plan build_plan(const Cfg& c) {
    Plan p;
    const int mc = c.model_channels, nrb = c.num_res_blocks;
    auto name = [](const char* part, int idx, int sub) { return std::string("unet.") + part + "." + std::to_string(idx) + "." + std::to_string(sub); };
    p.in_blocks.push_back({Blk{CONV_IN, "unet.input_blocks.0.0", c.cond_dim, mc, c.grid_size}});
    std::vector<int> chans{mc}, sizes{c.grid_size};
    int ch = mc, ds = 1, sp = c.grid_size;
    for (size_t level = 0; level < c.mult.size(); ++level) {
        const int m = c.mult[level];
        for (int r = 0; r < nrb; ++r) {
            const int idx = (int)p.in_blocks.size();
            std::vector<Blk> seq{Blk{RES, name("input_blocks", idx, 0), ch, m * mc, sp}};
            ch = m * mc;
            if (has(c.attn, ds)) seq.push_back(Blk{ATTN, name("input_blocks", idx, 1), ch, ch, sp});
            p.in_blocks.push_back(seq);
            chans.push_back(ch);
        }
        if (level + 1 != c.mult.size()) {
            const int idx = (int)p.in_blocks.size();
            p.in_blocks.push_back({Blk{DOWN, name("input_blocks", idx, 0), ch, ch, sp}});
            chans.push_back(ch);
            sizes.push_back(sp);
            ds *= 2;
            sp = (sp + 1) / 2;
        }
    }
    p.middle = {Blk{RES, "unet.middle_block.0", ch, ch, sp}, Blk{ATTN, "unet.middle_block.1", ch, ch, sp}, Blk{RES, "unet.middle_block.2", ch, ch, sp}};
    for (int level = (int)c.mult.size() - 1; level >= 0; --level) {
        const int m = c.mult[level];
        for (int i = 0; i <= nrb; ++i) {
            const int idx = (int)p.out_blocks.size();
            const int ich = chans.back(); chans.pop_back();
            std::vector<Blk> seq{Blk{RES, name("output_blocks", idx, 0), ch + ich, mc * m, sp}};
            ch = mc * m;
            if (has(c.attn, ds)) seq.push_back(Blk{ATTN, name("output_blocks", idx, (int)seq.size()), ch, ch, sp});
            if (level && i == nrb) {
                seq.push_back(Blk{UP, name("output_blocks", idx, (int)seq.size()), ch, ch, sp});
                ds /= 2;
                sp = sizes.back(); sizes.pop_back();
            }
            p.out_blocks.push_back(seq);
        }
    }
    p.out_sp = sp;
    return p;
}

struct Param {
    std::string key;
    std::vector<int64_t> shape;
    int64_t numel = 1;
    bool norm = false;
    const float* d = nullptr;
    uint64_t version = 0;
};

std::vector<Param> param_table(const Cfg& c, const Plan& plan) {
    std::vector<Param> out;
    auto add = [&](const std::string& key, std::vector<int64_t> shape, bool norm) {
        Param p; p.key = key; p.shape = shape; p.norm = norm;
        for (int64_t s : shape) p.numel *= s;
        out.push_back(p);
    };
    auto conv = [&](const std::string& prefix, int cout, int cin, int k, int dims = 3) {
        std::vector<int64_t> s{cout, cin};
        for (int i = 0; i < dims; ++i) s.push_back(k);
        add(prefix + ".weight", s, false);
        add(prefix + ".bias", {cout}, false);
    };
    auto norm = [&](const std::string& prefix, std::vector<int64_t> shape) {
        add(prefix + ".weight", shape, true);
        add(prefix + ".bias", shape, true);
    };
    if (c.has_projector()) {
        const int hid = c.projector_hidden();
        if (!hid) {
            conv("projector.net.0", c.cond_dim, c.feature_channels, 1);
            norm("projector.net.1", {c.cond_dim});
        } else {
            conv("projector.net.0", hid, c.feature_channels, 1);
            norm("projector.net.1", {hid});
            conv("projector.net.3", hid, hid, 3);
            norm("projector.net.4", {hid});
            conv("projector.net.6", c.cond_dim, hid, 1);
            norm("projector.net.7", {c.cond_dim});
        }
    }
    auto emit = [&](const Blk& b) {
        const std::vector<int64_t> vol{b.sp, b.sp, b.sp};
        switch (b.kind) {
            case CONV_IN: conv(b.prefix, b.cout, b.cin, 3); break;
            case RES:
                norm(b.prefix + ".in_layers.0", vol);
                conv(b.prefix + ".in_layers.2", b.cout, b.cin, 3);
                norm(b.prefix + ".out_layers.0", vol);
                conv(b.prefix + ".out_layers.3", b.cout, b.cout, 3);
                if (b.cin != b.cout) conv(b.prefix + ".skip_connection", b.cout, b.cin, 1);
                break;
            case DOWN: conv(b.prefix + ".op", b.cout, b.cin, 3); break;
            case UP:   conv(b.prefix + ".conv", b.cout, b.cin, 3); break;
            case ATTN:
                norm(b.prefix + ".norm", {b.cin});
                conv(b.prefix + ".qkv", 3 * b.cin, b.cin, 1, 1);
                conv(b.prefix + ".proj_out", b.cin, b.cin, 1, 1);
                break;
        }
    };
    for (auto& seq : plan.in_blocks) for (auto& b : seq) emit(b);
    for (auto& b : plan.middle) emit(b);
    for (auto& seq : plan.out_blocks) for (auto& b : seq) emit(b);
    norm("unet.out.0", {plan.out_sp, plan.out_sp, plan.out_sp});
    conv("unet.out.2", c.out_channels, c.model_channels, 3);
    return out;
}

struct Arena {
    static constexpr int64_t kAlign = 256;
    char* base = nullptr;
    int64_t capacity = 0, peak = 0;
    std::map<int64_t, int64_t> free_;
    std::map<int64_t, int64_t> used_;

    void reset(char* b, int64_t cap) {
        base = b; capacity = cap; peak = 0;
        free_.clear(); used_.clear();
        free_[0] = cap;
    }
    int64_t alloc(int64_t bytes) {
        bytes = (bytes + kAlign - 1) / kAlign * kAlign;
        if (bytes == 0) bytes = kAlign;
        for (auto it = free_.begin(); it != free_.end(); ++it) {
            if (it->second < bytes) continue;
            const int64_t off = it->first, rest = it->second - bytes;
            free_.erase(it);
            if (rest > 0) free_[off + bytes] = rest;
            used_[off] = bytes;
            if (off + bytes > peak) peak = off + bytes;
            return off;
        }
        fail("pixie_unet_forward: the workspace is too small (%lld bytes; ask pixie_unet_workspace_bytes for this grid size)", (long long)capacity);
    }
    void release(int64_t off) {
        auto u = used_.find(off);
        if (u == used_.end()) return;
        int64_t size = u->second;
        used_.erase(u);
        auto next = free_.lower_bound(off);
        if (next != free_.end() && off + size == next->first) { size += next->second; next = free_.erase(next); }
        if (next != free_.begin()) {
            auto prev = std::prev(next);
            if (prev->first + prev->second == off) { prev->second += size; return; }
        }
        free_[off] = size;
    }
    template <class T> T* ptr(int64_t off) const { return reinterpret_cast<T*>(base + off); }
};

struct Exec;
struct Tens {
    Exec* ex = nullptr;
    float* p = nullptr;
    int64_t off = -1;
    int c = 0, d = 0, h = 0, w = 0;
    int64_t sums_off = -1;
    bool has_sums = false;
    double* sums = nullptr;
    uint32_t* slot = nullptr;
    int64_t spatial() const { return (int64_t)d * h * w; }
    ~Tens();
};
using TP = std::shared_ptr<Tens>;

struct Packed { void* d = nullptr; uint64_t version = ~0ull; };
struct Sized { int64_t bytes; int slots; int64_t zsum_doubles; };
struct Bound { float wmax = 0, bmax = 0; uint64_t wver = ~0ull, bver = ~0ull; };

}
}

using namespace pixie;

struct pixie_unet {
    Cfg cfg;
    Plan plan;
    std::vector<Param> params;
    std::unordered_map<std::string, int> index;
    std::unordered_map<std::string, Packed> packed32, packed16;
    std::unordered_map<std::string, Bound> bounds;
    uint32_t* d_bound_slots = nullptr;
    std::vector<uint32_t> h_bound_slots;
    std::map<std::tuple<int, int, int, bool>, Sized> sized;
    bool fuse_stats = true, split_k = true, fold_skip = true, subpixel = true;
    struct Replay { const float* feat; const float* proj0; float* out; void* ws; int d; uint64_t epoch; hipGraph_t graph; hipGraphExec_t exec; };
    bool use_graph = false;
    uint64_t epoch = 0;
    std::vector<Replay> replays;
    static constexpr size_t kMaxReplays = 4;
    void drop_replay(size_t i) {
        (void)hipGraphExecDestroy(replays[i].exec);
        (void)hipGraphDestroy(replays[i].graph);
        replays.erase(replays.begin() + (long)i);
    }

    const Param& param(const std::string& key) const {
        auto it = index.find(key);
        if (it == index.end()) fail("pixie_unet: no parameter named '%s'", key.c_str());
        return params[it->second];
    }
};

namespace pixie {
namespace {

struct Exec {
    pixie_unet* net = nullptr;
    Arena arena;
    bool dry = false;
    void* stream = nullptr;
    uint32_t* slots = nullptr;
    int slot_next = 0, slot_cap = 0;
    double* zsums = nullptr;
    int64_t zsum_next = 0, zsum_cap = 0;

    TP make(int c, int d, int h, int w) {
        auto t = std::make_shared<Tens>();
        t->ex = this; t->c = c; t->d = d; t->h = h; t->w = w;
        t->off = arena.alloc((int64_t)c * d * h * w * sizeof(float));
        t->p = arena.ptr<float>(t->off);
        return t;
    }
    TP external(const float* p, int c, int d, int h, int w) {
        auto t = std::make_shared<Tens>();
        t->ex = this; t->p = const_cast<float*>(p); t->c = c; t->d = d; t->h = h; t->w = w;
        return t;
    }
    uint32_t* new_slot() {
        if (!dry && slot_next >= slot_cap) fail("pixie_unet_forward: out of |x|max slots (internal sizing error)");
        return dry ? (slot_next++, nullptr) : slots + slot_next++;
    }
    struct Scratch {
        Exec* ex; int64_t off;
        Scratch(Exec* e, int64_t bytes) : ex(e), off(e->arena.alloc(bytes)) {}
        ~Scratch() { ex->arena.release(off); }
        template <class T> T* as() const { return ex->arena.ptr<T>(off); }
    };

    const float* P(const std::string& key) {
        const Param& p = net->param(key);
        if (!dry && !p.d) fail("pixie_unet_forward: parameter '%s' was never set", key.c_str());
        return p.d;
    }
    const void* w16(const std::string& key, bool subpixel = false) {
        const Param& p = net->param(key + ".weight");
        if (dry) return nullptr;
        Packed& e = net->packed16[subpixel ? key + "#subpixel" : key];
        if (e.version != p.version) {
            const int cout = (int)p.shape[0], cin = (int)p.shape[1], k = (int)p.shape[2];
            const int64_t nb = subpixel ? (k == 3 ? pixie_conv_subpixel_bytes(cout, cin) : 0) : pixie_conv_packed16_bytes(cout, cin, k);
            if (nb <= 0) fail("pixie_unet: '%s' cannot take the f16x3 packing (c_in %d)", key.c_str(), cin);
            if (!e.d && hipMalloc(&e.d, (size_t)nb) != hipSuccess) fail("pixie_unet: hipMalloc of %lld bytes failed", (long long)nb);
            if (!p.d) fail("pixie_unet_forward: parameter '%s.weight' was never set", key.c_str());
            if (subpixel) ok(pixie_conv_pack_weights_subpixel(p.d, e.d, cout, cin, stream), "pixie_conv_pack_weights_subpixel");
            else ok(pixie_conv_pack_weights_f16x2(p.d, e.d, cout, cin, k, stream), "pixie_conv_pack_weights_f16x2");
            e.version = p.version;
        }
        return e.d;
    }
    const float* w32(const std::string& key) {
        const Param& p = net->param(key + ".weight");
        if (dry) return nullptr;
        Packed& e = net->packed32[key];
        if (e.version != p.version) {
            const int cout = (int)p.shape[0], cin = (int)p.shape[1], k = (int)p.shape[2];
            int64_t taps = 1;
            for (size_t i = 2; i < p.shape.size(); ++i) taps *= p.shape[i];
            const int64_t nb = taps * cin * pixie_conv_cout_padded(cout) * (int64_t)sizeof(float);
            if (!e.d && hipMalloc(&e.d, (size_t)nb) != hipSuccess) fail("pixie_unet: hipMalloc of %lld bytes failed", (long long)nb);
            if (!p.d) fail("pixie_unet_forward: parameter '%s.weight' was never set", key.c_str());
            ok(pixie_conv_pack_weights(p.d, static_cast<float*>(e.d), cout, cin, k, stream), "pixie_conv_pack_weights");
            e.version = p.version;
        }
        return static_cast<const float*>(e.d);
    }
    float norm_bound(const std::string& key, int64_t count) {
        if (dry) return 1.0f;
        const Bound& b = net->bounds[key];
        return (float)(std::sqrt((double)count) * (double)b.wmax + (double)b.bmax + 1e-30);
    }

    void stats(const TP& t) {
        if (t->has_sums) return;
        t->has_sums = true;
        if (!dry && zsum_next + 2 * t->c > zsum_cap) fail("pixie_unet_forward: out of statistics space (internal sizing error)");
        t->sums = dry ? nullptr : zsums + zsum_next;
        zsum_next += 2 * t->c;
        t->slot = new_slot();
        if (!dry) ok(channel_stats_prezeroed(t->p, t->c, t->spatial(), t->sums, t->slot, as_stream(stream)), "pixie_channel_stats");
    }
    struct AB { std::shared_ptr<Scratch> mem; float* a; float* b; };
    AB norm_finalize(const double* sums, int c, int64_t spatial, int mode, int groups, const float* w, const float* b) {
        AB r;
        const int cpad = (c + 63) / 64 * 64;
        r.mem = std::make_shared<Scratch>(this, (int64_t)(cpad + c) * sizeof(float));
        r.a = r.mem->as<float>();
        r.b = r.a + cpad;
        if (!dry) ok(pixie_norm_finalize(sums, c, spatial, mode, groups, 1e-5, w, b, r.a, r.b, stream), "pixie_norm_finalize");
        return r;
    }

    bool f16_ok(const std::vector<TP>& parts, int stride) const {
        int cin = 0;
        for (auto& t : parts) cin += t->c;
        return net->cfg.precision == 0 && (stride == 1 || stride == 2) && cin % 16 == 0 && parts[0]->c % 8 == 0;
    }
    bool skip_foldable(const TP& x, int cout, int ksize, const std::vector<TP>& sp) const {
        pixie_conv_desc d;
        std::memset(&d, 0, sizeof d);
        d.c0 = x->c; d.in_d = x->d; d.in_h = x->h; d.in_w = x->w;
        d.stride = 1; d.ksize = ksize; d.c_out = cout;
        d.d_w16 = reinterpret_cast<const void*>(0x100);
        d.d_workspace = net->split_k ? reinterpret_cast<void*>(0x100) : nullptr;
        d.skip_c0 = sp[0]->c; d.skip_c1 = sp.size() > 1 ? sp[1]->c : 0;
        return pixie_conv_skip_foldable(&d) != 0;
    }

    struct ConvOpt {
        int stride = 1; bool upsample = false;
        const AB* pro = nullptr; std::string affine_store;
        int act = ACT_NONE; TP residual; float bound = 0.0f;
        int out_d = 0, out_h = 0, out_w = 0;
        float* out_ptr = nullptr;
        const std::vector<TP>* skip_parts = nullptr; std::string skip_key;
    };
    TP conv(const std::vector<TP>& parts, const std::string& wkey, int cout, int ksize, const ConvOpt& o) {
        const TP& x0 = parts[0];
        const Tens* x1 = parts.size() > 1 ? parts[1].get() : nullptr;
        const int up = o.upsample ? 2 : 1, pad = ksize == 3 ? 1 : 0;
        int od = (x0->d * up + 2 * pad - ksize) / o.stride + 1;
        int oh = (x0->h * up + 2 * pad - ksize) / o.stride + 1;
        int ow = (x0->w * up + 2 * pad - ksize) / o.stride + 1;
        pixie_conv_desc desc;
        std::memset(&desc, 0, sizeof desc);
        if (o.out_d) {
            od = std::min(od, o.out_d); oh = std::min(oh, o.out_h); ow = std::min(ow, o.out_w);
            desc.out_d = od; desc.out_h = oh; desc.out_w = ow;
        }
        const bool f16 = f16_ok(parts, o.stride);
        const bool raw = !o.pro && o.affine_store.empty();
        if (f16 && raw) for (auto& t : parts) stats(t);

        TP out = o.out_ptr ? external(o.out_ptr, cout, od, oh, ow) : make(cout, od, oh, ow);
        desc.d_in0 = x0->p; desc.c0 = x0->c;
        desc.d_in1 = x1 ? x1->p : nullptr; desc.c1 = x1 ? x1->c : 0;
        desc.in_d = x0->d; desc.in_h = x0->h; desc.in_w = x0->w;
        desc.upsample = o.upsample ? 1 : 0;
        desc.stride = o.stride;
        desc.ksize = ksize;
        if (o.pro) { desc.d_pro_a = o.pro->a; desc.d_pro_b = o.pro->b; }
        if (!o.affine_store.empty()) { desc.d_gamma = P(o.affine_store + ".weight"); desc.d_beta = P(o.affine_store + ".bias"); }
        desc.act = o.act;
        desc.d_bias = P(wkey + ".bias");
        desc.c_out = cout;
        desc.d_residual = o.residual ? o.residual->p : nullptr;
        desc.d_out = out->p;
        if (!f16) {
            desc.d_w = w32(wkey);
            if (!dry) ok(pixie_conv3d_forward(&desc, stream), "pixie_conv3d_forward");
            return out;
        }
        const bool sub = net->subpixel && o.upsample && ksize == 3 && o.stride == 1;
        desc.d_w16 = w16(wkey, sub);
        desc.w16_subpixel = sub ? 1 : 0;
        if (o.skip_parts) {
            const std::vector<TP>& sp = *o.skip_parts;
            desc.d_skip_in0 = sp[0]->p; desc.skip_c0 = sp[0]->c;
            desc.d_skip_in1 = sp.size() > 1 ? sp[1]->p : nullptr; desc.skip_c1 = sp.size() > 1 ? sp[1]->c : 0;
            desc.d_skip_w16 = w16(o.skip_key);
            desc.d_skip_bias = P(o.skip_key + ".bias");
            desc.d_skip_amax0 = sp[0]->slot; desc.d_skip_amax1 = sp.size() > 1 ? sp[1]->slot : nullptr;
            if (dry) desc.d_skip_w16 = reinterpret_cast<const void*>(0x100);
        }
        if (raw) {
            desc.d_in_amax0 = parts[0]->slot;
            desc.d_in_amax1 = x1 ? parts[1]->slot : nullptr;
        } else {
            desc.in_bound = o.bound;
        }
        std::unique_ptr<Scratch> workspace, tile_stats;
        if (dry) { desc.d_w16 = reinterpret_cast<const void*>(0x100); }
        if (net->split_k) {
            const int64_t wsb = pixie_conv_workspace_bytes(&desc);
            if (wsb > 0) { workspace.reset(new Scratch(this, wsb)); desc.d_workspace = workspace->as<void>(); if (dry) desc.d_workspace = reinterpret_cast<void*>(0x100); }
        }
        bool have_stats = false;
        if (net->fuse_stats) {
            uint32_t* slot = new_slot();
            const int64_t nfl = pixie_conv_stats_floats(&desc);
            if (nfl > 0) {
                tile_stats.reset(new Scratch(this, nfl * (int64_t)sizeof(float)));
                desc.d_out_stats = tile_stats->as<float>();
                desc.d_out_amax = slot;
                have_stats = true;
                out->slot = slot;
            }
        }
        if (!dry) ok(pixie_conv3d_forward(&desc, stream), "pixie_conv3d_forward");
        if (have_stats) {
            out->sums_off = arena.alloc((int64_t)cout * 2 * sizeof(double));
            out->sums = arena.ptr<double>(out->sums_off);
            out->has_sums = true;
            if (!dry) ok(pixie_stats_finalize(desc.d_out_stats, &desc, out->sums, stream), "pixie_stats_finalize");
        }
        return out;
    }

    AB norm_finalize_parts(const std::vector<TP>& parts, int64_t spatial) {
        for (auto& t : parts) stats(t);
        if (parts.size() == 1) return norm_finalize(parts[0]->sums, parts[0]->c, spatial, 0, 1, nullptr, nullptr);
        const int c0 = parts[0]->c, c1 = parts[1]->c, c = c0 + c1;
        AB r;
        const int cpad = (c + 63) / 64 * 64;
        r.mem = std::make_shared<Scratch>(this, (int64_t)(cpad + c) * sizeof(float));
        r.a = r.mem->as<float>();
        r.b = r.a + cpad;
        if (!dry) ok(norm_finalize_cat(parts[0]->sums, c0, parts[1]->sums, c1, spatial, 0, 1, 1e-5, nullptr, nullptr, r.a, r.b, as_stream(stream)),
                     "pixie_norm_finalize");
        return r;
    }
    TP res(const Blk& b, const std::vector<TP>& parts) {
        const std::string& p = b.prefix;
        const int64_t spatial = parts[0]->spatial();
        AB pro = norm_finalize_parts(parts, spatial);
        ConvOpt o1; o1.pro = &pro; o1.affine_store = p + ".in_layers.0"; o1.act = ACT_LEAKY; o1.bound = norm_bound(p + ".in_layers.0", spatial);
        TP h = conv(parts, p + ".in_layers.2", b.cout, 3, o1);
        stats(h);
        AB pro2 = norm_finalize(h->sums, b.cout, spatial, 0, 1, nullptr, nullptr);
        TP skip = parts[0];
        ConvOpt o2; o2.pro = &pro2; o2.affine_store = p + ".out_layers.0"; o2.act = ACT_LEAKY; o2.bound = norm_bound(p + ".out_layers.0", spatial);
        if (b.cin != b.cout) {
            if (net->fold_skip && f16_ok({h}, 1) && f16_ok(parts, 1) && skip_foldable(h, b.cout, 3, parts)) {
                skip.reset();
                for (auto& t : parts) stats(t);
                o2.skip_parts = &parts; o2.skip_key = p + ".skip_connection";
            } else {
                skip = conv(parts, p + ".skip_connection", b.cout, 1, ConvOpt{});
            }
        }
        o2.residual = skip;
        return conv({h}, p + ".out_layers.3", b.cout, 3, o2);
    }
    TP attn(const Blk& b, const TP& x) {
        const std::string& p = b.prefix;
        const int c = x->c;
        const int64_t spatial = x->spatial();
        stats(x);
        AB pro = norm_finalize(x->sums, c, spatial, 1, 32, P(p + ".norm.weight"), P(p + ".norm.bias"));
        ConvOpt o; o.pro = &pro; o.bound = norm_bound(p + ".norm", spatial * (c / 32));
        TP qkv = conv({x}, p + ".qkv", 3 * c, 1, o);
        TP att = make(c, x->d, x->h, x->w);
        if (!dry) ok(pixie_attention_forward(qkv->p, att->p, c, (int)spatial, stream), "pixie_attention_forward");
        qkv.reset();
        ConvOpt o2; o2.residual = x;
        return conv({att}, p + ".proj_out", c, 1, o2);
    }
    TP block(const Blk& b, const std::vector<TP>& parts, const Tens* up_to) {
        if (b.kind == RES) return res(b, parts);
        const TP& x = parts[0];
        if (b.kind == ATTN) return attn(b, x);
        if (b.kind == DOWN) { ConvOpt o; o.stride = 2; return conv({x}, b.prefix + ".op", b.cout, 3, o); }
        if (b.kind == UP) {
            ConvOpt o; o.upsample = true;
            if (up_to) { o.out_d = up_to->d; o.out_h = up_to->h; o.out_w = up_to->w; }
            return conv({x}, b.prefix + ".conv", b.cout, 3, o);
        }
        fail("pixie_unet: unexpected block kind");
    }

    TP forward(const float* d_feat, const float* d_proj0, int D, int H, int W, float* d_out) {
        const Cfg& c = net->cfg;
        const int64_t spatial = (int64_t)D * H * W;
        TP x;
        AB pro_in; const AB* pro_in_p = nullptr;
        int act_in = ACT_NONE; float bound_in = 0.0f;
        if (c.has_projector()) {
            const std::string q = "projector.net.";
            const int hid = c.projector_hidden();
            if (!hid) {
                const int g = std::max(c.cond_dim / 2, 1);
                x = conv({external(d_feat, c.feature_channels, D, H, W)}, q + "0", c.cond_dim, 1, ConvOpt{});
                stats(x);
                pro_in = norm_finalize(x->sums, c.cond_dim, spatial, 1, g, P(q + "1.weight"), P(q + "1.bias"));
                act_in = ACT_SILU;
                bound_in = norm_bound(q + "1", spatial * (c.cond_dim / g));
            } else {
                if (d_proj0) x = external(d_proj0, hid, D, H, W);
                else x = conv({external(d_feat, c.feature_channels, D, H, W)}, q + "0", hid, 1, ConvOpt{});
                stats(x);
                AB pro = norm_finalize(x->sums, hid, spatial, 1, 32, P(q + "1.weight"), P(q + "1.bias"));
                ConvOpt o; o.pro = &pro; o.act = ACT_SILU; o.bound = norm_bound(q + "1", spatial * (hid / 32));
                x = conv({x}, q + "3", hid, 3, o);
                stats(x);
                AB pro2 = norm_finalize(x->sums, hid, spatial, 1, 32, P(q + "4.weight"), P(q + "4.bias"));
                ConvOpt o2; o2.pro = &pro2; o2.act = ACT_SILU; o2.bound = norm_bound(q + "4", spatial * (hid / 32));
                x = conv({x}, q + "6", c.cond_dim, 1, o2);
                stats(x);
                pro_in = norm_finalize(x->sums, c.cond_dim, spatial, 1, 32, P(q + "7.weight"), P(q + "7.bias"));
                bound_in = norm_bound(q + "7", spatial * std::max(c.cond_dim / 32, 1));
            }
            pro_in_p = &pro_in;
        } else {
            x = external(d_feat, c.feature_channels, D, H, W);
        }
        const Plan& plan = net->plan;
        std::vector<TP> hs;
        const Blk& first = plan.in_blocks[0][0];
        ConvOpt of; of.pro = pro_in_p; of.act = act_in; of.bound = bound_in;
        TP h = conv({x}, first.prefix, first.cout, 3, of);
        x.reset();
        pro_in = AB{};
        hs.push_back(h);
        for (size_t i = 1; i < plan.in_blocks.size(); ++i) {
            for (const Blk& b : plan.in_blocks[i]) h = block(b, {h}, nullptr);
            hs.push_back(h);
        }
        for (const Blk& b : plan.middle) h = block(b, {h}, nullptr);
        for (auto& seq : plan.out_blocks) {
            TP skip = hs.back(); hs.pop_back();
            if (skip->d != h->d || skip->h != h->h || skip->w != h->w) fail("pixie_unet_forward: skip tensor and decoder tensor differ in size");
            std::vector<TP> parts{h, skip};
            h.reset(); skip.reset();
            for (const Blk& b : seq) {
                TP nh = block(b, parts, (b.kind == UP && !hs.empty()) ? hs.back().get() : nullptr);
                parts.clear();
                parts.push_back(nh);
            }
            h = parts[0];
        }
        stats(h);
        AB pro = norm_finalize(h->sums, h->c, h->spatial(), 0, 1, nullptr, nullptr);
        ConvOpt oo; oo.pro = &pro; oo.affine_store = "unet.out.0"; oo.act = ACT_LEAKY; oo.bound = norm_bound("unet.out.0", h->spatial());
        oo.out_ptr = d_out;
        return conv({h}, "unet.out.2", c.out_channels, 3, oo);
    }
};

Tens::~Tens() {
    if (!ex) return;
    if (off >= 0) ex->arena.release(off);
    if (sums_off >= 0) ex->arena.release(sums_off);
}

void refresh_bounds(pixie_unet* net, void* stream) {
    std::vector<std::pair<std::string, int>> todo;
    int n_norm = 0;
    for (const Param& p : net->params) {
        if (!p.norm || p.key.size() < 7 || p.key.compare(p.key.size() - 7, 7, ".weight") != 0) continue;
        const std::string key = p.key.substr(0, p.key.size() - 7);
        const Param& pb = net->param(key + ".bias");
        Bound& b = net->bounds[key];
        if (b.wver != p.version || b.bver != pb.version) todo.push_back({key, 2 * n_norm});
        ++n_norm;
    }
    if (todo.empty()) return;
    const size_t bytes = (size_t)2 * n_norm * sizeof(uint32_t);
    if (!net->d_bound_slots && hipMalloc(&net->d_bound_slots, bytes) != hipSuccess) fail("pixie_unet: hipMalloc failed");
    net->h_bound_slots.assign((size_t)2 * n_norm, 0u);
    hipStream_t s = as_stream(stream);
    if (hipMemsetAsync(net->d_bound_slots, 0, bytes, s) != hipSuccess) fail("pixie_unet: hipMemsetAsync failed");
    for (auto& t : todo) {
        const Param& pw = net->param(t.first + ".weight");
        const Param& pb = net->param(t.first + ".bias");
        if (!pw.d || !pb.d) fail("pixie_unet_forward: parameter '%s' was never set", t.first.c_str());
        ok(pixie_tensor_amax(pw.d, pw.numel, net->d_bound_slots + t.second, stream), "pixie_tensor_amax");
        ok(pixie_tensor_amax(pb.d, pb.numel, net->d_bound_slots + t.second + 1, stream), "pixie_tensor_amax");
    }
    if (hipMemcpyAsync(net->h_bound_slots.data(), net->d_bound_slots, bytes, hipMemcpyDeviceToHost, s) != hipSuccess ||
        hipStreamSynchronize(s) != hipSuccess)
        fail("pixie_unet: reading the normalisation bounds back failed: %s", hipGetErrorString(hipGetLastError()));
    for (auto& t : todo) {
        Bound& b = net->bounds[t.first];
        std::memcpy(&b.wmax, &net->h_bound_slots[t.second], 4);
        std::memcpy(&b.bmax, &net->h_bound_slots[t.second + 1], 4);
        b.wver = net->param(t.first + ".weight").version;
        b.bver = net->param(t.first + ".bias").version;
    }
}

__global__ void zero_head_kernel(uint4* p, int64_t n16) {
    const int64_t i = (int64_t)blockIdx.x * 256 + threadIdx.x;
    if (i < n16) p[i] = make_uint4(0u, 0u, 0u, 0u);
}

constexpr int64_t kSlotAlign = 256;
int64_t slot_region_bytes(int n_slots) { return ((int64_t)n_slots * 4 + kSlotAlign - 1) / kSlotAlign * kSlotAlign; }
int64_t zsum_region_bytes(int64_t n_doubles) { return (n_doubles * 8 + kSlotAlign - 1) / kSlotAlign * kSlotAlign; }

Sized size_pass(pixie_unet* net, int D, int H, int W, bool from_proj0) {
    auto key = std::make_tuple(D, H, W, from_proj0);
    auto it = net->sized.find(key);
    if (it != net->sized.end()) return it->second;
    Exec ex;
    ex.net = net; ex.dry = true; ex.stream = nullptr;
    ex.arena.reset(reinterpret_cast<char*>(0x10000000), (int64_t)1 << 50);
    {
        const float* fake = reinterpret_cast<const float*>(0x100);
        TP out = ex.forward(from_proj0 ? nullptr : fake, from_proj0 ? fake : nullptr, D, H, W, reinterpret_cast<float*>(0x100));
    }
    Sized r{ex.arena.peak + slot_region_bytes(ex.slot_next) + zsum_region_bytes(ex.zsum_next), ex.slot_next, ex.zsum_next};
    net->sized[key] = r;
    return r;
}

template <class F> int guarded(F f) {
    try { return f(); }
    catch (const std::exception& e) { return set_error("%s", e.what()); }
}

}
}

extern "C" int pixie_unet_create(pixie_unet** out, const pixie_unet_config* c) {
    PX_REQUIRE(out && c, "pixie_unet_create: null argument");
    PX_REQUIRE(c->n_channel_mult >= 1 && c->n_channel_mult <= 8 && c->n_attention_resolutions >= 0 && c->n_attention_resolutions <= 8,
               "pixie_unet_create: channel_mult needs 1..8 entries, attention_resolutions 0..8");
    PX_REQUIRE(c->feature_channels > 0 && c->cond_dim > 0 && c->model_channels > 0 && c->num_res_blocks > 0 && c->grid_size > 0 && c->out_channels > 0,
               "pixie_unet_create: non-positive size");
    PX_REQUIRE(c->precision == 0 || c->precision == 1, "pixie_unet_create: precision is 0 (f16x3) or 1 (exact fp32)");
    return guarded([&] {
        std::unique_ptr<pixie_unet> n(new pixie_unet);
        n->cfg.feature_channels = c->feature_channels; n->cfg.cond_dim = c->cond_dim; n->cfg.model_channels = c->model_channels;
        n->cfg.num_res_blocks = c->num_res_blocks; n->cfg.grid_size = c->grid_size; n->cfg.out_channels = c->out_channels;
        n->cfg.precision = c->precision;
        n->cfg.mult.assign(c->channel_mult, c->channel_mult + c->n_channel_mult);
        n->cfg.attn.assign(c->attention_resolutions, c->attention_resolutions + c->n_attention_resolutions);
        n->plan = build_plan(n->cfg);
        n->params = param_table(n->cfg, n->plan);
        for (size_t i = 0; i < n->params.size(); ++i) n->index[n->params[i].key] = (int)i;
        const char* fs = getenv("PIXIE_FUSE_STATS"); n->fuse_stats = !(fs && fs[0] == '0');
        const char* sk = getenv("PIXIE_CONV_SPLIT_K"); n->split_k = !(sk && sk[0] == '0');
        const char* fk = getenv("PIXIE_FOLD_SKIP"); n->fold_skip = !(fk && fk[0] == '0');
        const char* sx = getenv("PIXIE_CONV_SUBPIXEL"); n->subpixel = !(sx && sx[0] == '0');
        *out = n.release();
        return 0;
    });
}

extern "C" int pixie_unet_destroy(pixie_unet* h) {
    if (!h) return 0;
    for (auto& kv : h->packed16) if (kv.second.d) (void)hipFree(kv.second.d);
    for (auto& kv : h->packed32) if (kv.second.d) (void)hipFree(kv.second.d);
    if (h->d_bound_slots) (void)hipFree(h->d_bound_slots);
    while (!h->replays.empty()) h->drop_replay(0);
    delete h;
    return 0;
}

extern "C" int pixie_unet_param_count(const pixie_unet* h) { return h ? (int)h->params.size() : 0; }

extern "C" int pixie_unet_param_info(const pixie_unet* h, int i, const char** key, int64_t* numel, int32_t* ndim, int64_t shape[5]) {
    PX_REQUIRE(h && i >= 0 && i < (int)h->params.size(), "pixie_unet_param_info: index out of range");
    const Param& p = h->params[i];
    if (key) *key = p.key.c_str();
    if (numel) *numel = p.numel;
    if (ndim) *ndim = (int32_t)p.shape.size();
    if (shape) for (size_t k = 0; k < p.shape.size() && k < 5; ++k) shape[k] = p.shape[k];
    return 0;
}

extern "C" int pixie_unet_set_param(pixie_unet* h, const char* key, const float* d_values, int64_t numel) {
    PX_REQUIRE(h && key && d_values, "pixie_unet_set_param: null argument");
    auto it = h->index.find(key);
    PX_REQUIRE(it != h->index.end(), "pixie_unet_set_param: unexpected key '%s' (the reference's load_state_dict(strict=True) raises here too)", key);
    Param& p = h->params[it->second];
    PX_REQUIRE(numel == p.numel, "pixie_unet_set_param: '%s' has %lld elements, got %lld", key, (long long)p.numel, (long long)numel);
    p.d = d_values;
    ++p.version;
    ++h->epoch;
    return 0;
}

extern "C" int64_t pixie_unet_workspace_bytes(pixie_unet* h, int d, int hh, int w) {
    if (!h || d <= 0 || hh <= 0 || w <= 0) { set_error("pixie_unet_workspace_bytes: bad argument"); return -1; }
    int64_t bytes = -1;
    const int rc = guarded([&] {
        bytes = size_pass(h, d, hh, w, false).bytes;
        if (h->cfg.projector_hidden() > 0) bytes = std::max(bytes, size_pass(h, d, hh, w, true).bytes);
        return 0;
    });
    return rc == 0 ? bytes : -1;
}

extern "C" int pixie_unet_forward(pixie_unet* h, const float* d_feat, const float* d_proj0, int d, int hh, int w, float* d_out,
                                  void* d_workspace, int64_t workspace_bytes, void* stream) {
    PX_REQUIRE(h && d_out && d_workspace && (d_feat || d_proj0), "pixie_unet_forward: null argument");
    PX_REQUIRE(d == h->cfg.grid_size && hh == d && w == d,
               "pixie_unet_forward: the network was built for a %d^3 grid (its LayerNorm parameters have that shape), got %d x %d x %d", h->cfg.grid_size, d, hh, w);
    PX_REQUIRE(!d_proj0 || h->cfg.projector_hidden() > 0, "pixie_unet_forward: d_proj0 needs the hidden-128 projector (feature_channels > cond_dim)");
    PX_REQUIRE(d_feat || (d_proj0 && h->cfg.has_projector()), "pixie_unet_forward: d_feat is null");
    return guarded([&] {
        const auto sized = size_pass(h, d, hh, w, d_proj0 != nullptr);
        if (workspace_bytes < sized.bytes)
            fail("pixie_unet_forward: workspace of %lld bytes, this grid needs %lld (pixie_unet_workspace_bytes)", (long long)workspace_bytes, (long long)sized.bytes);
        auto launch_all = [&] {
            Exec ex;
            ex.net = h; ex.dry = false; ex.stream = stream;
            const int64_t slot_bytes = slot_region_bytes(sized.slots), head_bytes = slot_bytes + zsum_region_bytes(sized.zsum_doubles);
            ex.slots = static_cast<uint32_t*>(d_workspace);
            ex.slot_cap = sized.slots;
            ex.zsums = reinterpret_cast<double*>(static_cast<char*>(d_workspace) + slot_bytes);
            ex.zsum_cap = sized.zsum_doubles;
            hipLaunchKernelGGL(zero_head_kernel, dim3((unsigned)((head_bytes / 16 + 255) / 256)), dim3(256), 0, as_stream(stream),
                               static_cast<uint4*>(d_workspace), head_bytes / 16);
            if (hipGetLastError() != hipSuccess) fail("pixie_unet_forward: clearing the workspace head failed");
            ex.arena.reset(static_cast<char*>(d_workspace) + head_bytes, workspace_bytes - head_bytes);
            TP out = ex.forward(d_feat, d_proj0, d, hh, w, d_out);
        };
        if (h->use_graph) {
            for (size_t i = 0; i < h->replays.size(); ++i) {
                const pixie_unet::Replay& r = h->replays[i];
                if (r.feat != d_feat || r.proj0 != d_proj0 || r.out != d_out || r.ws != d_workspace || r.d != d) continue;
                if (r.epoch != h->epoch) { h->drop_replay(i); break; }
                if (hipGraphLaunch(r.exec, as_stream(stream)) != hipSuccess) fail("pixie_unet_forward: hipGraphLaunch failed: %s", hipGetErrorString(hipGetLastError()));
                if (i + 1 != h->replays.size()) std::rotate(h->replays.begin() + (long)i, h->replays.begin() + (long)i + 1, h->replays.end());
                return 0;
            }
        }
        if (h->use_graph && as_stream(stream) == nullptr)
            fail("pixie_unet_forward: option \"graph\" needs a non-default stream (the legacy stream cannot be captured); pass a created stream or set graph = 0");
        refresh_bounds(h, stream);
        launch_all();
        if (h->use_graph) {
            hipStream_t st = as_stream(stream);
            if (hipStreamBeginCapture(st, hipStreamCaptureModeThreadLocal) != hipSuccess)
                fail("pixie_unet_forward: cannot capture on this stream (graph replay needs a non-default stream): %s", hipGetErrorString(hipGetLastError()));
            hipGraph_t graph = nullptr;
            try { launch_all(); }
            catch (...) { (void)hipStreamEndCapture(st, &graph); if (graph) (void)hipGraphDestroy(graph); throw; }
            if (hipStreamEndCapture(st, &graph) != hipSuccess || !graph) fail("pixie_unet_forward: hipStreamEndCapture failed: %s", hipGetErrorString(hipGetLastError()));
            hipGraphExec_t exec = nullptr;
            if (hipGraphInstantiate(&exec, graph, nullptr, nullptr, 0) != hipSuccess) { (void)hipGraphDestroy(graph); fail("pixie_unet_forward: hipGraphInstantiate failed"); }
            if (h->replays.size() >= pixie_unet::kMaxReplays) h->drop_replay(0);
            h->replays.push_back(pixie_unet::Replay{d_feat, d_proj0, d_out, d_workspace, d, h->epoch, graph, exec});
        }
        return 0;
    });
}

extern "C" int pixie_unet_set_option(pixie_unet* h, const char* key, int value) {
    PX_REQUIRE(h && key, "pixie_unet_set_option: null argument");
    const std::string k(key);
    if (k == "graph") {
        h->use_graph = value != 0;
        if (!h->use_graph) while (!h->replays.empty()) h->drop_replay(0);
        return 0;
    }
    return set_error("pixie_unet_set_option: unknown key '%s' (known: graph)", key);
}
```

### pixie_amd/unet.py

```python
from __future__ import annotations

import ctypes as C
import math
import os
import warnings
import weakref
from typing import Dict, List, Optional, Sequence, Tuple

import torch
import torch.nn as nn

from . import _lib
from ._lib import ConvDesc, check
from .unet_plan import Block, UNetConfig, UNetPlan, build_plan, param_shapes, is_norm_key

ACT_NONE, ACT_LEAKY, ACT_SILU = 0, 1, 2
DEFAULT_PRECISION = os.environ.get("PIXIE_CONV_PRECISION", "f16x3")
_ZERO_INIT_SUFFIXES = (".out_layers.3.weight", ".out_layers.3.bias", ".proj_out.weight", ".proj_out.bias",
                       "unet.out.2.weight", "unet.out.2.bias")


def _ptr(t: Optional[torch.Tensor]):
    return C.c_void_p(t.data_ptr()) if t is not None else C.c_void_p(0)


def _addr(t: Optional[torch.Tensor]):
    return t.data_ptr() if t is not None else None


def fill_conv_desc(lib, alloc, parts: Sequence[torch.Tensor], packed_w, bias, cout: int, ksize: int, *, stride: int = 1,
                   upsample: bool = False, pro=None, affine=None, act: int = 0, residual=None, w16=None, in_amax=None,
                   in_bound: float = 0.0, out_amax=None, out_size=None, skip=None, subpixel: bool = False, split_k: bool = True,
                   addr=_addr):
    x0 = parts[0]
    x1 = parts[1] if len(parts) > 1 else None
    cin0, d, h, w = x0.shape
    up = 2 if upsample else 1
    pad = 1 if ksize == 3 else 0
    od = (d * up + 2 * pad - ksize) // stride + 1
    oh = (h * up + 2 * pad - ksize) // stride + 1
    ow = (w * up + 2 * pad - ksize) // stride + 1
    desc = ConvDesc()
    if out_size is not None:
        od, oh, ow = min(od, int(out_size[0])), min(oh, int(out_size[1])), min(ow, int(out_size[2]))
        desc.out_d, desc.out_h, desc.out_w = od, oh, ow
    out = alloc((cout, od, oh, ow), torch.float32)
    desc.d_in0 = addr(x0); desc.c0 = cin0
    desc.d_in1 = addr(x1)
    desc.c1 = x1.shape[0] if x1 is not None else 0
    desc.in_d, desc.in_h, desc.in_w = d, h, w
    desc.upsample = 1 if upsample else 0
    desc.stride = stride
    desc.ksize = ksize
    desc.d_pro_a = addr(pro[0]) if pro is not None else None
    desc.d_pro_b = addr(pro[1]) if pro is not None else None
    desc.d_gamma = addr(affine[0]) if affine is not None else None
    desc.d_beta = addr(affine[1]) if affine is not None else None
    desc.act = act
    desc.d_w = addr(packed_w)
    desc.d_w16 = addr(w16)
    desc.w16_subpixel = 1 if subpixel else 0
    desc.d_in_amax0 = addr(in_amax[0]) if in_amax else None
    desc.d_in_amax1 = addr(in_amax[1]) if in_amax and len(in_amax) > 1 else None
    desc.in_bound = float(in_bound)
    desc.d_bias = addr(bias)
    desc.c_out = cout
    desc.d_residual = addr(residual)
    desc.d_out = addr(out)
    if skip is not None:
        sp = skip["parts"]
        desc.d_skip_in0 = addr(sp[0]); desc.skip_c0 = sp[0].shape[0]
        desc.d_skip_in1 = addr(sp[1]) if len(sp) > 1 else None
        desc.skip_c1 = sp[1].shape[0] if len(sp) > 1 else 0
        desc.d_skip_w16 = addr(skip["w16"])
        desc.d_skip_bias = addr(skip["bias"])
        desc.d_skip_amax0 = addr(skip["amax"][0])
        desc.d_skip_amax1 = addr(skip["amax"][1]) if len(sp) > 1 else None
    stats = workspace = None
    if w16 is not None and split_k:
        wsb = lib.pixie_conv_workspace_bytes(C.byref(desc))
        if wsb > 0:
            workspace = alloc((wsb,), torch.uint8)
            desc.d_workspace = addr(workspace)
    if out_amax is not None and w16 is not None:
        nfl = lib.pixie_conv_stats_floats(C.byref(desc))
        if nfl > 0:
            stats = alloc((nfl,), torch.float32)
            desc.d_out_stats = addr(stats)
            desc.d_out_amax = addr(out_amax)
    return desc, out, stats, workspace


class HipOps:

    def __init__(self, device: torch.device):
        if device.type != "cuda":
            raise _lib.PixieHipError("pixie_amd U-Net operators run on a HIP device only (no CPU fallback)")
        self.device = device
        self.lib = _lib.load()
        self.split_k = os.environ.get("PIXIE_CONV_SPLIT_K", "1") != "0"
        self.record_variant = False
        self.last_variant = (0, 1)

    @property
    def stream(self):
        return _lib.current_stream_ptr()

    def pack_conv(self, weight: torch.Tensor) -> torch.Tensor:
        cout, cin = weight.shape[0], weight.shape[1]
        k = weight.shape[2]
        coutp = self.lib.pixie_conv_cout_padded(cout)
        w = weight.detach().to(self.device, torch.float32).contiguous()
        taps = 1
        for s in weight.shape[2:]:
            taps *= int(s)
        packed = torch.empty((taps, cin, coutp), device=self.device, dtype=torch.float32)
        check(self.lib.pixie_conv_pack_weights(_ptr(w), _ptr(packed), cout, cin, k, self.stream), "pixie_conv_pack_weights")
        return packed

    def pack_conv16(self, weight: torch.Tensor) -> torch.Tensor:
        cout, cin, k = weight.shape[0], weight.shape[1], weight.shape[2]
        nbytes = self.lib.pixie_conv_packed16_bytes(cout, cin, k)
        if nbytes <= 0:
            raise _lib.PixieHipError(f"f16x3 packing needs c_in % 8 == 0 (got {cin})")
        w = weight.detach().to(self.device, torch.float32).contiguous()
        packed = torch.empty(nbytes, device=self.device, dtype=torch.uint8)
        check(self.lib.pixie_conv_pack_weights_f16x2(_ptr(w), _ptr(packed), cout, cin, k, self.stream), "pixie_conv_pack_weights_f16x2")
        return packed

    def pack_conv_subpixel(self, weight: torch.Tensor) -> torch.Tensor:
        cout, cin = weight.shape[0], weight.shape[1]
        nbytes = self.lib.pixie_conv_subpixel_bytes(cout, cin) if tuple(weight.shape[2:]) == (3, 3, 3) else 0
        if nbytes <= 0:
            raise _lib.PixieHipError(f"sub-pixel packing needs a 3x3x3 weight with c_in % 16 == 0 (got {tuple(weight.shape)})")
        w = weight.detach().to(self.device, torch.float32).contiguous()
        packed = torch.empty(nbytes, device=self.device, dtype=torch.uint8)
        check(self.lib.pixie_conv_pack_weights_subpixel(_ptr(w), _ptr(packed), cout, cin, self.stream), "pixie_conv_pack_weights_subpixel")
        return packed

    @staticmethod
    def f16x3_ok(parts: Sequence[torch.Tensor], stride: int) -> bool:
        cin = sum(int(p.shape[0]) for p in parts)
        return stride in (1, 2) and cin % 16 == 0 and int(parts[0].shape[0]) % 8 == 0

    def conv(self, parts: Sequence[torch.Tensor], packed_w: Optional[torch.Tensor], bias: Optional[torch.Tensor], cout: int, ksize: int,
             stride: int = 1, upsample: bool = False, pro: Optional[Tuple[torch.Tensor, torch.Tensor]] = None,
             affine: Optional[Tuple[torch.Tensor, torch.Tensor]] = None, act: int = ACT_NONE,
             residual: Optional[torch.Tensor] = None, w16: Optional[torch.Tensor] = None,
             in_amax: Optional[Sequence[torch.Tensor]] = None, in_bound: float = 0.0,
             out_amax: Optional[torch.Tensor] = None, out_size: Optional[Tuple[int, int, int]] = None,
             skip: Optional[dict] = None, subpixel: bool = False):
        desc, out, stats, _ = fill_conv_desc(
            self.lib, lambda shape, dtype: torch.empty(shape, device=self.device, dtype=dtype), parts, packed_w, bias, cout, ksize,
            stride=stride, upsample=upsample, pro=pro, affine=affine, act=act, residual=residual, w16=w16, in_amax=in_amax,
            in_bound=in_bound, out_amax=out_amax, out_size=out_size, skip=skip, subpixel=subpixel, split_k=self.split_k)
        sums = None
        if self.record_variant:
            sl = C.c_int(1)
            self.last_variant = (int(_lib.load(diag=True).pixie_conv_kernel_variant(C.byref(desc), C.byref(sl))), int(sl.value))
        check(self.lib.pixie_conv3d_forward(C.byref(desc), self.stream), "pixie_conv3d_forward")
        if desc.d_out_stats:
            sums = torch.empty((cout, 2), device=self.device, dtype=torch.float64)
            check(self.lib.pixie_stats_finalize(_ptr(stats), C.byref(desc), _ptr(sums), self.stream), "pixie_stats_finalize")
        if out_amax is not None:
            return out, sums
        return out

    def skip_foldable(self, x: torch.Tensor, cout: int, ksize: int, skip_parts: Sequence[torch.Tensor]) -> bool:
        desc = ConvDesc()
        desc.c0 = x.shape[0]
        desc.in_d, desc.in_h, desc.in_w = (int(v) for v in x.shape[1:])
        desc.stride, desc.ksize, desc.c_out = 1, ksize, cout
        desc.d_w16 = 1
        desc.d_workspace = 1 if self.split_k else None
        desc.skip_c0 = skip_parts[0].shape[0]
        desc.skip_c1 = skip_parts[1].shape[0] if len(skip_parts) > 1 else 0
        return bool(self.lib.pixie_conv_skip_foldable(C.byref(desc)))

    def channel_sums(self, x: torch.Tensor) -> torch.Tensor:
        c = x.shape[0]
        spatial = x.numel() // c
        sums = torch.empty((c, 2), device=self.device, dtype=torch.float64)
        check(self.lib.pixie_channel_sums(_ptr(x), c, spatial, _ptr(sums), self.stream), "pixie_channel_sums")
        return sums

    def channel_stats(self, x: torch.Tensor, amax_slot: torch.Tensor) -> torch.Tensor:
        c = x.shape[0]
        spatial = x.numel() // c
        sums = torch.empty((c, 2), device=self.device, dtype=torch.float64)
        check(self.lib.pixie_channel_stats(_ptr(x), c, spatial, _ptr(sums), _ptr(amax_slot), self.stream), "pixie_channel_stats")
        return sums

    def norm_finalize(self, sums: torch.Tensor, spatial: int, mode: int, groups: int = 1, eps: float = 1e-5,
                      weight: Optional[torch.Tensor] = None, bias: Optional[torch.Tensor] = None):
        c = sums.shape[0]
        a = torch.empty(c, device=self.device, dtype=torch.float32)
        b = torch.empty(c, device=self.device, dtype=torch.float32)
        check(self.lib.pixie_norm_finalize(_ptr(sums), c, spatial, mode, groups, eps, _ptr(weight), _ptr(bias), _ptr(a), _ptr(b),
                                           self.stream), "pixie_norm_finalize")
        return a, b

    def attention(self, qkv: torch.Tensor, channels: int, tokens: int) -> torch.Tensor:
        out = torch.empty((channels, tokens), device=self.device, dtype=torch.float32)
        check(self.lib.pixie_attention_forward(_ptr(qkv), _ptr(out), channels, tokens, self.stream), "pixie_attention_forward")
        return out

    def projector_conv0(self, grid_dhwc_f16: torch.Tensor, nets: Sequence[Tuple[torch.Tensor, Optional[torch.Tensor]]], cout: int):
        d, h, w, c = (int(v) for v in grid_dhwc_f16.shape)
        g = grid_dhwc_f16.contiguous()
        outs = [torch.empty((cout, d, h, w), device=self.device, dtype=torch.float32) for _ in nets]
        n = len(nets)
        w_arr = (C.c_void_p * n)(*[t[0].data_ptr() for t in nets])
        b_arr = (C.c_void_p * n)(*[(t[1].data_ptr() if t[1] is not None else None) for t in nets])
        o_arr = (C.c_void_p * n)(*[o.data_ptr() for o in outs])
        check(self.lib.pixie_projector_conv0(_ptr(g), d * h * w, c, n, w_arr, b_arr, o_arr, cout, self.stream), "pixie_projector_conv0")
        return outs

    def combine(self, logits: torch.Tensor, cont: torch.Tensor):
        ncls = logits.shape[0]
        spatial = logits.numel() // ncls
        combined = torch.empty((3 + ncls,) + tuple(logits.shape[1:]), device=self.device, dtype=torch.float32)
        amax = torch.empty(tuple(logits.shape[1:]), device=self.device, dtype=torch.int32)
        check(self.lib.pixie_combine_predictions(_ptr(logits), ncls, _ptr(cont), spatial, _ptr(combined), _ptr(amax), self.stream),
              "pixie_combine_predictions")
        return combined, amax


class UNetRunner:

    def __init__(self, cfg: UNetConfig, params: Dict[str, torch.Tensor], ops, precision: Optional[str] = None):
        self.cfg = cfg
        self.plan: UNetPlan = build_plan(cfg)
        self.p = params
        self.ops = ops
        self.precision = precision or DEFAULT_PRECISION
        if self.precision not in ("f16x3", "f32"):
            raise ValueError(f"unknown conv precision {self.precision!r}")
        self._packed: Dict[str, Tuple[int, int, torch.Tensor]] = {}
        self._packed16: Dict[str, Tuple[int, int, torch.Tensor]] = {}
        self._bounds: Dict[str, Tuple[int, int, float, float]] = {}
        self.fuse_stats = os.environ.get("PIXIE_FUSE_STATS", "1") != "0"
        self.fold_skip = os.environ.get("PIXIE_FOLD_SKIP", "1") != "0"
        self.subpixel = os.environ.get("PIXIE_CONV_SUBPIXEL", "1") != "0"

    @property
    def _f16x3(self) -> bool:
        return self.precision == "f16x3" and hasattr(self.ops, "pack_conv16")

    def _w(self, key: str) -> torch.Tensor:
        t = self.p[key + ".weight"]
        ent = self._packed.get(key)
        if ent is None or ent[0] != t.data_ptr() or ent[1] != t._version:
            self._packed[key] = (t.data_ptr(), t._version, self.ops.pack_conv(t))
        return self._packed[key][2]

    def _w16(self, key: str, subpixel: bool = False) -> torch.Tensor:
        t = self.p[key + ".weight"]
        ck = key + "#subpixel" if subpixel else key
        ent = self._packed16.get(ck)
        if ent is None or ent[0] != t.data_ptr() or ent[1] != t._version:
            self._packed16[ck] = (t.data_ptr(), t._version, self.ops.pack_conv_subpixel(t) if subpixel else self.ops.pack_conv16(t))
        return self._packed16[ck][2]

    def _b(self, key: str) -> torch.Tensor:
        return self.p[key + ".bias"]

    def _absmax(self, key: str) -> Tuple[float, float]:
        w, bb = self.p[key + ".weight"], self.p[key + ".bias"]
        ent = self._bounds.get(key)
        if ent is None or ent[0] != w._version or ent[1] != bb._version:
            self._bounds[key] = (w._version, bb._version, float(w.abs().max()), float(bb.abs().max()))
            ent = self._bounds[key]
        return ent[2], ent[3]

    def _norm_bound(self, key: str, count: int) -> float:
        wmax, bmax = self._absmax(key)
        return math.sqrt(float(count)) * wmax + bmax + 1e-30

    _SLOT_POOL = 1024

    @classmethod
    def _new_slot(cls, cache: dict, device) -> torch.Tensor:
        pool = cache.get("_slots")
        if pool is None or cache["_next"] >= pool.numel():
            pool = cache["_slots"] = torch.zeros(cls._SLOT_POOL, dtype=torch.int32, device=device)
            cache["_next"] = 0
        i = cache["_next"]
        cache["_next"] = i + 1
        return pool[i:i + 1]

    @staticmethod
    def _remember(cache: dict, t: torch.Tensor, sums, slot) -> None:
        k = id(t)
        cache[k] = (sums, slot)
        weakref.finalize(t, cache.pop, k, None)

    def _stats(self, cache: dict, t: torch.Tensor):
        k = id(t)
        if k not in cache:
            if hasattr(self.ops, "channel_stats"):
                slot = self._new_slot(cache, t.device)
                self._remember(cache, t, self.ops.channel_stats(t, slot), slot)
            else:
                self._remember(cache, t, self.ops.channel_sums(t), None)
        return cache[k]

    def _sums(self, cache: dict, t: torch.Tensor) -> torch.Tensor:
        return self._stats(cache, t)[0]

    def _amax(self, cache: dict, t: torch.Tensor) -> torch.Tensor:
        return self._stats(cache, t)[1]

    def _conv(self, cache: dict, parts: List[torch.Tensor], wkey: str, cout: int, ksize: int, *, stride: int = 1,
              upsample: bool = False, pro=None, affine_key: Optional[str] = None, act: int = ACT_NONE,
              residual: Optional[torch.Tensor] = None, bound: float = 0.0, out_size=None, skip=None) -> torch.Tensor:
        ops = self.ops
        affine = (self.p[affine_key + ".weight"], self.p[affine_key + ".bias"]) if affine_key else None
        if not (self._f16x3 and ops.f16x3_ok(parts, stride)):
            return ops.conv(parts, self._w(wkey), self._b(wkey), cout, ksize, stride=stride, upsample=upsample, pro=pro,
                            affine=affine, act=act, residual=residual, **({"out_size": out_size} if out_size is not None else {}))
        if pro is None and affine is None:
            kw = dict(in_amax=[self._amax(cache, t) for t in parts])
        else:
            kw = dict(in_bound=bound)
        if out_size is not None:
            kw["out_size"] = out_size
        if skip is not None:
            kw["skip"] = skip
        sub = self.subpixel and upsample and ksize == 3 and stride == 1 and hasattr(ops, "pack_conv_subpixel")
        if sub:
            kw["subpixel"] = True
        if self.fuse_stats:
            slot = self._new_slot(cache, parts[0].device)
            out, sums = ops.conv(parts, None, self._b(wkey), cout, ksize, stride=stride, upsample=upsample, pro=pro, affine=affine,
                                 act=act, residual=residual, w16=self._w16(wkey, sub), out_amax=slot, **kw)
            if sums is not None:
                self._remember(cache, out, sums, slot)
            return out
        return ops.conv(parts, None, self._b(wkey), cout, ksize, stride=stride, upsample=upsample, pro=pro, affine=affine,
                        act=act, residual=residual, w16=self._w16(wkey, sub), **kw)

    def _res(self, b: Block, parts: List[torch.Tensor], cache: dict) -> torch.Tensor:
        ops, p = self.ops, b.prefix
        spatial = parts[0][0].numel()
        sums = torch.cat([self._sums(cache, t) for t in parts], dim=0) if len(parts) > 1 else self._sums(cache, parts[0])
        pro = ops.norm_finalize(sums, spatial, 0)
        h = self._conv(cache, parts, p + ".in_layers.2", b.cout, 3, pro=pro, affine_key=p + ".in_layers.0", act=ACT_LEAKY,
                       bound=self._norm_bound(p + ".in_layers.0", spatial))
        pro2 = ops.norm_finalize(self._sums(cache, h), spatial, 0)
        fold = None
        if b.cin != b.cout:
            if (self.fold_skip and self._f16x3 and ops.f16x3_ok([h], 1) and ops.f16x3_ok(parts, 1)
                    and ops.skip_foldable(h, b.cout, 3, parts)):
                skip = None
                fold = dict(parts=parts, w16=self._w16(p + ".skip_connection"), bias=self._b(p + ".skip_connection"),
                            amax=[self._amax(cache, t) for t in parts])
            else:
                skip = self._conv(cache, parts, p + ".skip_connection", b.cout, 1)
        else:
            skip = parts[0]
        return self._conv(cache, [h], p + ".out_layers.3", b.cout, 3, pro=pro2, affine_key=p + ".out_layers.0", act=ACT_LEAKY,
                          residual=skip, bound=self._norm_bound(p + ".out_layers.0", spatial), skip=fold)

    def _attn(self, b: Block, x: torch.Tensor, cache: dict) -> torch.Tensor:
        ops, p = self.ops, b.prefix
        c = x.shape[0]
        spatial = x[0].numel()
        pro = ops.norm_finalize(self._sums(cache, x), spatial, 1, groups=32, weight=self.p[p + ".norm.weight"],
                                bias=self.p[p + ".norm.bias"])
        qkv = self._conv(cache, [x], p + ".qkv", 3 * c, 1, pro=pro, bound=self._norm_bound(p + ".norm", spatial * (c // 32)))
        att = ops.attention(qkv.reshape(3 * c, spatial), c, spatial).reshape(x.shape)
        return self._conv(cache, [att], p + ".proj_out", c, 1, residual=x)

    def _block(self, b: Block, parts: List[torch.Tensor], cache: dict, up_size=None) -> torch.Tensor:
        if b.kind == "res":
            return self._res(b, parts, cache)
        assert len(parts) == 1
        x = parts[0]
        if b.kind == "attn":
            return self._attn(b, x, cache)
        if b.kind == "down":
            return self._conv(cache, [x], b.prefix + ".op", b.cout, 3, stride=2)
        if b.kind == "up":
            return self._conv(cache, [x], b.prefix + ".conv", b.cout, 3, upsample=True, out_size=up_size)
        raise ValueError(b.kind)

    def _stem(self, feat: Optional[torch.Tensor], cache: dict, proj0: Optional[torch.Tensor] = None) -> torch.Tensor:
        cfg, ops = self.cfg, self.ops
        spatial = (proj0 if proj0 is not None else feat)[0].numel()
        x = feat
        pro_in, act_in, bound_in = None, ACT_NONE, 0.0
        if cfg.has_projector:
            q = "projector.net."
            if cfg.projector_hidden is None:
                g = max(cfg.cond_dim // 2, 1)
                x = self._conv(cache, [x], q + "0", cfg.cond_dim, 1)
                pro_in = ops.norm_finalize(self._sums(cache, x), spatial, 1, groups=g,
                                           weight=self.p[q + "1.weight"], bias=self.p[q + "1.bias"])
                act_in = ACT_SILU
                bound_in = self._norm_bound(q + "1", spatial * (cfg.cond_dim // g))
            else:
                hid = cfg.projector_hidden
                x = proj0 if proj0 is not None else self._conv(cache, [x], q + "0", hid, 1)
                pro = ops.norm_finalize(self._sums(cache, x), spatial, 1, groups=32, weight=self.p[q + "1.weight"], bias=self.p[q + "1.bias"])
                x = self._conv(cache, [x], q + "3", hid, 3, pro=pro, act=ACT_SILU, bound=self._norm_bound(q + "1", spatial * (hid // 32)))
                pro = ops.norm_finalize(self._sums(cache, x), spatial, 1, groups=32, weight=self.p[q + "4.weight"], bias=self.p[q + "4.bias"])
                x = self._conv(cache, [x], q + "6", cfg.cond_dim, 1, pro=pro, act=ACT_SILU, bound=self._norm_bound(q + "4", spatial * (hid // 32)))
                pro_in = ops.norm_finalize(self._sums(cache, x), spatial, 1, groups=32, weight=self.p[q + "7.weight"], bias=self.p[q + "7.bias"])
                bound_in = self._norm_bound(q + "7", spatial * max(cfg.cond_dim // 32, 1))
        first = self.plan.input_blocks[0][0]
        return self._conv(cache, [x], first.prefix, first.cout, 3, pro=pro_in, act=act_in, bound=bound_in)

    def _head(self, h: torch.Tensor, cache: dict) -> torch.Tensor:
        pro = self.ops.norm_finalize(self._sums(cache, h), h[0].numel(), 0)
        return self._conv(cache, [h], "unet.out.2", self.cfg.out_channels, 3, pro=pro, affine_key="unet.out.0", act=ACT_LEAKY,
                          bound=self._norm_bound("unet.out.0", h[0].numel()))

    def forward(self, feat: Optional[torch.Tensor], taps: Optional[dict] = None, proj0: Optional[torch.Tensor] = None) -> torch.Tensor:
        cache: dict = {}
        only = set(taps) if taps else None

        def tap(key, t):
            if taps is not None and (only is None or key in only):
                taps[key] = t

        plan = self.plan
        hs: List[torch.Tensor] = []
        h = self._stem(feat, cache, proj0)
        hs.append(h)
        tap("unet.input_blocks.0", h)
        for seq in plan.input_blocks[1:]:
            for b in seq:
                h = self._block(b, [h], cache)
            hs.append(h)
            tap(seq[0].prefix.rsplit(".", 1)[0], h)
        for b in plan.middle:
            h = self._block(b, [h], cache)
            tap(b.prefix, h)
        for seq in plan.output_blocks:
            skip = hs.pop()
            assert tuple(skip.shape[1:]) == tuple(h.shape[1:]), (skip.shape, h.shape)
            parts = [h, skip]
            for b in seq:
                h = self._block(b, parts, cache, up_size=tuple(hs[-1].shape[1:]) if (b.kind == "up" and hs) else None)
                parts = [h]
            tap(seq[0].prefix.rsplit(".", 1)[0], h)
        return self._head(h, cache)


class UNetHandle:

    def __init__(self, cfg: UNetConfig, precision: str, device: torch.device):
        if device.type != "cuda":
            raise _lib.PixieHipError("pixie_amd U-Net runs on a HIP device only (no CPU fallback)")
        if precision not in ("f16x3", "f32"):
            raise ValueError(f"unknown conv precision {precision!r}")
        self.lib = _lib.load()
        self.cfg, self.precision, self.device = cfg, precision, device
        c = _lib.UNetConfigC()
        c.feature_channels, c.cond_dim, c.model_channels, c.num_res_blocks = cfg.feature_channels, cfg.cond_dim, cfg.model_channels, cfg.num_res_blocks
        c.n_channel_mult = len(cfg.channel_mult)
        for i, m in enumerate(cfg.channel_mult):
            c.channel_mult[i] = int(m)
        c.n_attention_resolutions = len(cfg.attention_resolutions)
        for i, m in enumerate(cfg.attention_resolutions):
            c.attention_resolutions[i] = int(m)
        c.grid_size, c.out_channels, c.precision = cfg.grid_size, cfg.out_channels, 0 if precision == "f16x3" else 1
        self._h = C.c_void_p()
        check(self.lib.pixie_unet_create(C.byref(self._h), C.byref(c)), "pixie_unet_create")
        weakref.finalize(self, self.lib.pixie_unet_destroy, self._h)
        self._seen: Dict[str, Tuple[int, int]] = {}
        self._keep: Dict[str, torch.Tensor] = {}

    def keys(self) -> List[str]:
        out = []
        for i in range(self.lib.pixie_unet_param_count(self._h)):
            key = C.c_char_p()
            check(self.lib.pixie_unet_param_info(self._h, i, C.byref(key), None, None, None), "pixie_unet_param_info")
            out.append(key.value.decode())
        return out

    def load(self, params: Dict[str, torch.Tensor]) -> None:
        for key, t in params.items():
            tag = (t.data_ptr(), t._version)
            if self._seen.get(key) == tag:
                continue
            v = t.detach()
            if v.device != self.device or v.dtype != torch.float32 or not v.is_contiguous():
                v = v.to(self.device, torch.float32).contiguous()
            self._keep[key] = v
            check(self.lib.pixie_unet_set_param(self._h, key.encode(), _ptr(v), v.numel()), "pixie_unet_set_param")
            self._seen[key] = tag

    def workspace_bytes(self, d: int, h: int, w: int) -> int:
        n = int(self.lib.pixie_unet_workspace_bytes(self._h, d, h, w))
        if n < 0:
            raise _lib.PixieHipError(self.lib.pixie_last_error().decode())
        return n

    def forward(self, feat: Optional[torch.Tensor], proj0: Optional[torch.Tensor] = None, workspace: Optional[torch.Tensor] = None) -> torch.Tensor:
        src = proj0 if proj0 is not None else feat
        d, h, w = (int(v) for v in src.shape[1:])
        out = torch.empty((self.cfg.out_channels, d, h, w), device=self.device, dtype=torch.float32)
        nbytes = self.workspace_bytes(d, h, w)
        if workspace is None:
            workspace = torch.empty(nbytes, device=self.device, dtype=torch.uint8)
        elif workspace.dtype != torch.uint8 or workspace.device != self.device or workspace.numel() < nbytes or not workspace.is_contiguous():
            raise ValueError(f"workspace must be a contiguous uint8 tensor of >= {nbytes} bytes on {self.device}")
        check(self.lib.pixie_unet_forward(self._h, _ptr(feat), _ptr(proj0), d, h, w, _ptr(out), _ptr(workspace), nbytes,
                                          _lib.current_stream_ptr()), "pixie_unet_forward")
        return out


class _Node(nn.Module):
    """Empty container used to reproduce the reference's state_dict key hierarchy."""


class _PixieUNet(nn.Module):
    def __init__(self, cfg: UNetConfig):
        super().__init__()
        self.cfg = cfg
        shapes = param_shapes(cfg)
        gen = torch.Generator().manual_seed(0)
        for key, shape in shapes.items():
            parts = key.split(".")
            node = self
            for name in parts[:-1]:
                if name not in node._modules:
                    node.add_module(name, _Node())
                node = node._modules[name]
            node.register_parameter(parts[-1], nn.Parameter(self._init(key, shape, shapes, gen), requires_grad=False))
        self._runner: Optional[UNetRunner] = None
        self._handle: Optional[UNetHandle] = None
        self.executor = os.environ.get("PIXIE_UNET_EXECUTOR", "c")
        self.conv_precision = DEFAULT_PRECISION
        self.use_graph = os.environ.get("PIXIE_UNET_GRAPH", "1") == "1"
        self._graphs: dict = {}
        self._plist = None

    @staticmethod
    def _init(key, shape, shapes, gen) -> torch.Tensor:
        if is_norm_key(key):
            return torch.ones(shape) if key.endswith(".weight") else torch.zeros(shape)
        if key.endswith(_ZERO_INIT_SUFFIXES):
            return torch.zeros(shape)
        wshape = shapes[key[: key.rfind(".")] + ".weight"]
        bound = 1.0 / math.sqrt(float(torch.tensor(wshape[1:]).prod()))
        return (torch.rand(shape, generator=gen) * 2.0 - 1.0) * bound

    def _params(self) -> Dict[str, torch.Tensor]:
        return {k: v for k, v in self.named_parameters()}

    def load_numpy_state(self, sd) -> None:
        self.load_state_dict({k: torch.from_numpy(v) for k, v in sd.items()}, strict=True)

    @torch.no_grad()
    def forward(self, feat_grid: torch.Tensor, taps: Optional[dict] = None) -> torch.Tensor:
        if feat_grid.dim() != 5 or feat_grid.shape[1] != self.cfg.feature_channels:
            raise ValueError(f"expected (N,{self.cfg.feature_channels},D,H,W), got {tuple(feat_grid.shape)}")
        dev = next(self.parameters()).device
        if dev.type != "cuda" or feat_grid.device != dev:
            raise _lib.PixieHipError("model and input must live on the same HIP device (no CPU fallback)")
        with torch.cuda.device(dev):
            self._prepare(dev)
            x = feat_grid.detach().to(torch.float32).contiguous()
            if self.use_graph and taps is None:
                return torch.stack([self._forward_graphed(x[n]) for n in range(x.shape[0])], dim=0)
            outs = [self._forward_one(x[n], taps=taps if n == 0 else None) for n in range(x.shape[0])]
            return torch.stack(outs, dim=0)

    def _prepare(self, dev) -> None:
        params = self._params()
        if self._runner is None or self._runner.ops.device != dev or self._runner.precision != self.conv_precision:
            self._runner = UNetRunner(self.cfg, params, HipOps(dev), precision=self.conv_precision)
        else:
            self._runner.p = params
        if self.executor == "c":
            if self._handle is None or self._handle.device != dev or self._handle.precision != self.conv_precision:
                self._handle = UNetHandle(self.cfg, self.conv_precision, dev)
            self._handle.load(params)
        elif self.executor != "python":
            raise ValueError(f"unknown executor {self.executor!r} (PIXIE_UNET_EXECUTOR is 'c' or 'python')")

    def _forward_one(self, x: Optional[torch.Tensor], taps: Optional[dict] = None, proj0: Optional[torch.Tensor] = None) -> torch.Tensor:
        if self.executor == "c" and taps is None:
            return self._handle.forward(x, proj0)
        return self._runner.forward(x, taps, proj0)

    def _apply(self, fn, *args, **kwargs):
        self._plist = None
        return super()._apply(fn, *args, **kwargs)

    def _param_list(self) -> List[torch.Tensor]:
        refs = self.__dict__.get("_plist")
        if refs is None:
            refs = self._plist = [(m._parameters, name) for m in self.modules() for name, p in m._parameters.items() if p is not None]
        return [d[name] for d, name in refs]

    def load_state_dict(self, state_dict, strict: bool = True, assign: bool = False):
        self._plist = None
        return super().load_state_dict(state_dict, strict=strict, assign=assign)

    def _forward_graphed(self, x: Optional[torch.Tensor], proj0: Optional[torch.Tensor] = None) -> torch.Tensor:
        src = proj0 if proj0 is not None else x
        base = (tuple(src.shape), tuple(src.stride()), src.dtype, proj0 is not None, self.executor, self.conv_precision, src.device.index,
                tuple((id(p), p.data_ptr(), p._version) for p in self._param_list()))
        run = (lambda t: self._forward_one(None, proj0=t)) if proj0 is not None else (lambda t: self._forward_one(t))
        if self._graphs.get("base") != base:
            self._graphs = {"base": base, "first_ptr": None}
        ent = self._graphs.get(src.data_ptr()) or self._graphs.get("copy")
        if ent is None:
            out = run(src)
            if self._graphs["first_ptr"] is None:
                self._graphs["first_ptr"] = src.data_ptr()
                return out
            in_place = (proj0 is None and self._graphs["first_ptr"] == src.data_ptr() and "copy" not in self._graphs
                        and os.environ.get("PIXIE_UNET_GRAPH_INPLACE", "1") == "1")
            try:
                static_in = src if in_place else src.clone()
                side = torch.cuda.Stream(src.device)
                side.wait_stream(torch.cuda.current_stream())
                with torch.cuda.stream(side):
                    run(static_in)
                torch.cuda.current_stream().wait_stream(side)
                graph = torch.cuda.CUDAGraph()
                with torch.cuda.graph(graph, capture_error_mode="thread_local"):
                    static_out = run(static_in)
            except RuntimeError as exc:
                warnings.warn(f"pixie_amd: HIP-graph capture of the U-Net forward failed ({exc}); continuing with eager launches",
                              RuntimeWarning)
                self.use_graph = False
                return out
            if in_place:
                ent = self._graphs[src.data_ptr()] = (graph, None, static_out)
            else:
                ent = self._graphs["copy"] = (graph, static_in, static_out)
        graph, static_in, static_out = ent
        if static_in is not None:
            static_in.copy_(src)
        graph.replay()
        return static_out.clone()


class SegmentationUNet(_PixieUNet):

    def __init__(self, feature_channels: int, cond_dim: int, model_channels: int, num_res_blocks: int,
                 channel_mult: Tuple[int, ...], attention_resolutions: Tuple[int, ...], grid_size: int, num_classes: int):
        super().__init__(UNetConfig(feature_channels, cond_dim, model_channels, num_res_blocks, tuple(channel_mult),
                                    tuple(attention_resolutions), grid_size, num_classes))


class RegressionUNet(_PixieUNet):

    def __init__(self, feature_channels: int, cond_dim: int, model_channels: int, num_res_blocks: int,
                 channel_mult: Tuple[int, ...], attention_resolutions: Tuple[int, ...], grid_size: int, out_channels: int = 3):
        super().__init__(UNetConfig(feature_channels, cond_dim, model_channels, num_res_blocks, tuple(channel_mult),
                                    tuple(attention_resolutions), grid_size, out_channels))


@torch.no_grad()
def predict_material_field_from_voxel_grid(seg_network: "SegmentationUNet", cont_network: "RegressionUNet", grid_dhwc_f16: torch.Tensor,
                                           dual_stream: Optional[bool] = None):
    dev = next(seg_network.parameters()).device
    g = grid_dhwc_f16
    if g.dim() != 4 or g.dtype != torch.float16 or g.device != dev or dev.type != "cuda":
        raise ValueError("expected a (D, H, W, C) float16 tensor on the networks' HIP device")
    nets = (seg_network, cont_network)
    for net in nets:
        if net.cfg.projector_hidden is None or net.cfg.feature_channels != g.shape[3] or net.conv_precision != "f16x3":
            raise ValueError("the fused grid path needs the hidden-128 projector, matching feature_channels and conv_precision 'f16x3'")
        net._prepare(dev)
    ops = seg_network._runner.ops
    q = "projector.net.0"
    packed = [(net._runner._w16(q), net._runner._b(q)) for net in nets]
    x_seg, x_cont = ops.projector_conv0(g, packed, seg_network.cfg.projector_hidden)
    if dual_stream is None:
        dual_stream = _dual_stream_default(seg_network, cont_network, int(g.shape[0]) * int(g.shape[1]) * int(g.shape[2]))

    def fwd(net, p0):
        return net._forward_graphed(None, p0) if net.use_graph else net._forward_one(None, proj0=p0)

    if dual_stream:
        cur = torch.cuda.current_stream()
        s1, s2 = _side_streams(dev)
        s1.wait_stream(cur); s2.wait_stream(cur)
        with torch.cuda.stream(s1):
            seg_logits = fwd(seg_network, x_seg)[None]
        with torch.cuda.stream(s2):
            cont_pred = fwd(cont_network, x_cont)[None]
        x_seg.record_stream(s1); x_cont.record_stream(s2)
        cur.wait_stream(s1); cur.wait_stream(s2)
        seg_logits.record_stream(cur); cont_pred.record_stream(cur)
    else:
        seg_logits = fwd(seg_network, x_seg)[None]
        cont_pred = fwd(cont_network, x_cont)[None]
    combined, seg_pred = ops.combine(seg_logits[0].contiguous(), cont_pred[0].contiguous())
    return combined[None], seg_pred[None], seg_logits, cont_pred


_SIDE_STREAMS: Dict[str, Tuple[torch.cuda.Stream, torch.cuda.Stream]] = {}


def _dual_stream_default(seg_network, cont_network, voxels: int) -> bool:
    env = os.environ.get("PIXIE_DUAL_STREAM")
    if env is not None:
        return env == "1"
    return not (seg_network.use_graph and cont_network.use_graph and voxels >= 128 ** 3)


def _side_streams(device):
    key = str(device)
    if key not in _SIDE_STREAMS:
        _SIDE_STREAMS[key] = (torch.cuda.Stream(device), torch.cuda.Stream(device))
    return _SIDE_STREAMS[key]


@torch.no_grad()
def predict_material_field(seg_network: SegmentationUNet, cont_network: RegressionUNet, feat_grid: torch.Tensor,
                           dual_stream: Optional[bool] = None):
    if feat_grid.is_cuda and feat_grid.device.index != torch.cuda.current_device():
        with torch.cuda.device(feat_grid.device):
            return predict_material_field(seg_network, cont_network, feat_grid, dual_stream)
    if dual_stream is None:
        dual_stream = _dual_stream_default(seg_network, cont_network, int(feat_grid[0, 0].numel()))
    if dual_stream and feat_grid.is_cuda:
        cur = torch.cuda.current_stream()
        s1, s2 = _side_streams(feat_grid.device)
        s1.wait_stream(cur); s2.wait_stream(cur)
        with torch.cuda.stream(s1):
            seg_logits = seg_network(feat_grid)
        with torch.cuda.stream(s2):
            cont_pred = cont_network(feat_grid)
        feat_grid.record_stream(s1); feat_grid.record_stream(s2)
        cur.wait_stream(s1); cur.wait_stream(s2)
        seg_logits.record_stream(cur); cont_pred.record_stream(cur)
    else:
        seg_logits = seg_network(feat_grid)
        cont_pred = cont_network(feat_grid)
    ops = seg_network._runner.ops
    combined, seg_pred = [], []
    for n in range(feat_grid.shape[0]):
        cmb, am = ops.combine(seg_logits[n].contiguous(), cont_pred[n].contiguous())
        combined.append(cmb)
        seg_pred.append(am)
    return torch.stack(combined), torch.stack(seg_pred), seg_logits, cont_pred
```

Before: 24.26 million voxels/s.

## Fuse norm statistics into split-K reduce and merge stats/norm finalize kernels

```diff
diff --git a/include/pixie_hip.h b/include/pixie_hip.h
--- a/include/pixie_hip.h
+++ b/include/pixie_hip.h
@@ -118,6 +118,8 @@
     const void* d_skip_w16; const float* d_skip_bias;
     const uint32_t* d_skip_amax0; const uint32_t* d_skip_amax1;
     int32_t w16_subpixel;
+    double* d_split_sums;
+    uint32_t* d_split_amax;
 } pixie_conv_desc;
 
 int pixie_conv_cout_padded(int c_out);
@@ -130,6 +132,8 @@
 int64_t pixie_conv_stats_floats(const pixie_conv_desc* desc);
 int64_t pixie_conv_workspace_bytes(const pixie_conv_desc* desc);
 int pixie_stats_finalize(const float* d_stats, const pixie_conv_desc* desc, double* d_sums, void* stream);
+int pixie_stats_norm_finalize(const float* d_stats, const pixie_conv_desc* desc, double* d_sums, int64_t spatial, int mode, int groups,
+                              double eps, const float* d_weight, const float* d_bias, float* d_a, float* d_b, void* stream);
 int pixie_conv_skip_foldable(const pixie_conv_desc* desc);
 
 int pixie_channel_sums(const float* d_x, int channels, int64_t spatial, double* d_sums, void* stream);
diff --git a/pixie_amd/_lib.py b/pixie_amd/_lib.py
--- a/pixie_amd/_lib.py
+++ b/pixie_amd/_lib.py
@@ -48,7 +48,8 @@
                 ("d_skip_in1", C.c_void_p), ("skip_c1", C.c_int32),
                 ("d_skip_w16", C.c_void_p), ("d_skip_bias", C.c_void_p),
                 ("d_skip_amax0", C.c_void_p), ("d_skip_amax1", C.c_void_p),
-                ("w16_subpixel", C.c_int32)]
+                ("w16_subpixel", C.c_int32),
+                ("d_split_sums", C.c_void_p), ("d_split_amax", C.c_void_p)]
 
 
 class UNetConfigC(C.Structure):
@@ -119,6 +120,7 @@
     "pixie_conv_stats_floats": (_I64, [C.POINTER(ConvDesc)]),
     "pixie_conv_workspace_bytes": (_I64, [C.POINTER(ConvDesc)]),
     "pixie_stats_finalize": (_I, [_VP, C.POINTER(ConvDesc), _VP, _VP]),
+    "pixie_stats_norm_finalize": (_I, [_VP, C.POINTER(ConvDesc), _VP, _I64, _I, _I, _D, _VP, _VP, _VP, _VP, _VP]),
     "pixie_channel_stats": (_I, [_VP, _I, _I64, _VP, _VP, _VP]),
     "pixie_tensor_amax": (_I, [_VP, _I64, _VP, _VP]),
     "pixie_channel_sums": (_I, [_VP, _I, _I64, _VP, _VP]),
diff --git a/pixie_amd/csrc/conv3d_f16x3.hip b/pixie_amd/csrc/conv3d_f16x3.hip
--- a/pixie_amd/csrc/conv3d_f16x3.hip
+++ b/pixie_amd/csrc/conv3d_f16x3.hip
@@ -618,15 +618,108 @@
     if (threadIdx.x == 0) { sums[2 * c] = r[0] + r[2] + r[4] + r[6]; sums[2 * c + 1] = r[1] + r[3] + r[5] + r[7]; }
 }
 
-__global__ __launch_bounds__(256) void splitk_reduce_kernel(const float* __restrict__ partial, int slices, long n_elems, long osp,
-                                                            const float* __restrict__ bias, const float* residual, float* out) {
-    const long i = (long)blockIdx.x * 256 + threadIdx.x;
-    if (i >= n_elems) return;
-    float v = partial[i];
-    for (int s = 1; s < slices; ++s) v += partial[(size_t)s * n_elems + i];
-    if (bias) v += bias[i / osp];
-    if (residual) v += residual[i];
-    out[i] = v;
+__device__ inline void norm_ab(double s1, double s2, double cnt, int mode, double eps, const float* weight, const float* bias, int c,
+                               float* a, float* b) {
+    const double mean = s1 / cnt;
+    double var = s2 / cnt - mean * mean;
+    if (var < 0.0) var = 0.0;
+    const double rstd = 1.0 / sqrt(var + eps);
+    if (mode == 0) {
+        a[c] = (float)rstd;
+        b[c] = (float)(-mean * rstd);
+    } else {
+        const double w = weight ? (double)weight[c] : 1.0;
+        const double bb = bias ? (double)bias[c] : 0.0;
+        a[c] = (float)(rstd * w);
+        b[c] = (float)(bb - mean * rstd * w);
+    }
+}
+
+__global__ __launch_bounds__(256) void stats_norm_finalize_kernel(const float* __restrict__ stats, int n_tiles, int coutp, int cpg, double spatial,
+                                                                  int mode, double eps, const float* __restrict__ weight,
+                                                                  const float* __restrict__ bias, double* __restrict__ sums,
+                                                                  float* __restrict__ a, float* __restrict__ b) {
+    __shared__ double r[8];
+    double g1 = 0.0, g2 = 0.0;
+    for (int k = 0; k < cpg; ++k) {
+        const int c = blockIdx.x * cpg + k;
+        double s1 = 0.0, s2 = 0.0;
+        for (int t = threadIdx.x; t < n_tiles; t += 256) {
+            const float2 v = *reinterpret_cast<const float2*>(stats + ((size_t)t * coutp + c) * 2);
+            s1 += v.x; s2 += v.y;
+        }
+        for (int off = 32; off > 0; off >>= 1) { s1 += __shfl_down(s1, off, 64); s2 += __shfl_down(s2, off, 64); }
+        if ((threadIdx.x & 63) == 0) { r[2 * (threadIdx.x >> 6)] = s1; r[2 * (threadIdx.x >> 6) + 1] = s2; }
+        __syncthreads();
+        if (threadIdx.x == 0) {
+            const double t1 = r[0] + r[2] + r[4] + r[6], t2 = r[1] + r[3] + r[5] + r[7];
+            sums[2 * c] = t1; sums[2 * c + 1] = t2;
+            g1 += t1; g2 += t2;
+        }
+        __syncthreads();
+    }
+    if (threadIdx.x == 0)
+        for (int k = 0; k < cpg; ++k) norm_ab(g1, g2, spatial * cpg, mode, eps, weight, bias, blockIdx.x * cpg + k, a, b);
+}
+
+__global__ __launch_bounds__(256) void splitk_reduce_kernel(const float* __restrict__ partial, int slices, long n_elems, long osp, long seg,
+                                                            const float* __restrict__ bias, const float* residual, float* out,
+                                                            double* __restrict__ sums, unsigned* __restrict__ amax) {
+    const int c = blockIdx.y;
+    const long begin = (long)blockIdx.x * seg;
+    const long end = begin + seg < osp ? begin + seg : osp;
+    const long base = (long)c * osp;
+    const bool has_bias = bias != nullptr;
+    const float bv = has_bias ? bias[c] : 0.0f;
+    double s1 = 0.0, s2 = 0.0;
+    float mx = 0.0f;
+    const bool vec_ok = (osp & 3) == 0 && ((reinterpret_cast<size_t>(partial) | reinterpret_cast<size_t>(out) | reinterpret_cast<size_t>(residual)) & 15) == 0;
+    if (vec_ok) {
+        float a1 = 0.f, a2 = 0.f;
+        int cnt = 0;
+        for (long i = base + begin + (long)threadIdx.x * 4; i < base + end; i += 256 * 4) {
+            float4 v = *reinterpret_cast<const float4*>(partial + i);
+            for (int s = 1; s < slices; ++s) {
+                const float4 p = *reinterpret_cast<const float4*>(partial + (size_t)s * n_elems + i);
+                v.x += p.x; v.y += p.y; v.z += p.z; v.w += p.w;
+            }
+            if (has_bias) { v.x += bv; v.y += bv; v.z += bv; v.w += bv; }
+            if (residual) {
+                const float4 q = *reinterpret_cast<const float4*>(residual + i);
+                v.x += q.x; v.y += q.y; v.z += q.z; v.w += q.w;
+            }
+            *reinterpret_cast<float4*>(out + i) = v;
+            a1 += (v.x + v.y) + (v.z + v.w);
+            a2 += (v.x * v.x + v.y * v.y) + (v.z * v.z + v.w * v.w);
+            mx = fmaxf(fmaxf(mx, fabsf(v.x)), fmaxf(fabsf(v.y), fmaxf(fabsf(v.z), fabsf(v.w))));
+            if (++cnt == 64) { s1 += a1; s2 += a2; a1 = 0.f; a2 = 0.f; cnt = 0; }
+        }
+        s1 += a1; s2 += a2;
+    } else {
+        for (long i = base + begin + threadIdx.x; i < base + end; i += 256) {
+            float v = partial[i];
+            for (int s = 1; s < slices; ++s) v += partial[(size_t)s * n_elems + i];
+            if (has_bias) v += bv;
+            if (residual) v += residual[i];
+            out[i] = v;
+            s1 += v; s2 += (double)v * v; mx = fmaxf(mx, fabsf(v));
+        }
+    }
+    if (!sums) return;
+    for (int off = 32; off > 0; off >>= 1) {
+        s1 += __shfl_down(s1, off, 64);
+        s2 += __shfl_down(s2, off, 64);
+        mx = fmaxf(mx, __shfl_down(mx, off, 64));
+    }
+    if (amax && (threadIdx.x & 63) == 0 && mx > 0.0f) atomicMax(amax, __float_as_uint(mx));
+    __shared__ double red[8];
+    const int lane = threadIdx.x & 63, wave = threadIdx.x >> 6;
+    if (lane == 0) { red[2 * wave] = s1; red[2 * wave + 1] = s2; }
+    __syncthreads();
+    if (threadIdx.x == 0) {
+        atomicAdd(&sums[2 * c], red[0] + red[2] + red[4] + red[6]);
+        atomicAdd(&sums[2 * c + 1], red[1] + red[3] + red[5] + red[7]);
+    }
 }
 
 __global__ __launch_bounds__(256) void amax_kernel(const float* __restrict__ x, long n, unsigned* __restrict__ slot) {
@@ -881,8 +974,11 @@
         }
         if (rc) return rc;
         const long osp = (long)a.OD * a.OH * a.OW, n_elems = (long)a.cout * osp;
-        hipLaunchKernelGGL(splitk_reduce_kernel, dim3((unsigned)((n_elems + 255) / 256)), dim3(256), 0, st, a.partial, slices, n_elems, osp,
-                           a.bias, a.residual, a.out);
+        long segs = std::min((osp + 2047) / 2048, std::max(1L, 4096L / a.cout));
+        const long seg = ((osp + segs - 1) / segs + 3) & ~3L;
+        segs = (osp + seg - 1) / seg;
+        hipLaunchKernelGGL(splitk_reduce_kernel, dim3((unsigned)segs, (unsigned)a.cout), dim3(256), 0, st, a.partial, slices, n_elems, osp, seg,
+                           a.bias, a.residual, a.out, d->d_split_sums, reinterpret_cast<unsigned*>(d->d_split_amax));
         PX_CHECK_HIP(hipGetLastError());
         return 0;
     }
@@ -1013,6 +1109,20 @@
     return 0;
 }
 
+extern "C" int pixie_stats_norm_finalize(const float* d_stats, const pixie_conv_desc* d, double* d_sums, int64_t spatial, int mode, int groups,
+                                         double eps, const float* d_weight, const float* d_bias, float* d_a, float* d_b, void* stream) {
+    PX_REQUIRE(d_stats && d && d_sums && d_a && d_b && spatial > 0, "pixie_stats_norm_finalize: bad arguments");
+    PX_REQUIRE(mode == 0 || (mode == 1 && groups > 0 && d->c_out % groups == 0), "pixie_stats_norm_finalize: bad mode/groups");
+    Conv16Args a{};
+    int MB = 0, NB = 0;
+    conv16_tiling(d, a, MB, NB);
+    const int cpg = mode == 0 ? 1 : d->c_out / groups;
+    hipLaunchKernelGGL(stats_norm_finalize_kernel, dim3((unsigned)(d->c_out / cpg)), dim3(256), 0, as_stream(stream), d_stats, a.n_tiles, a.coutp,
+                       cpg, (double)spatial, mode, eps, d_weight, d_bias, d_sums, d_a, d_b);
+    PX_CHECK_HIP(hipGetLastError());
+    return 0;
+}
+
 extern "C" int64_t pixie_conv_packed16_bytes(int c_out, int c_in, int ksize) {
     if (c_out <= 0 || c_in <= 0 || c_in % 8 != 0 || (ksize != 1 && ksize != 3)) return 0;
     const int64_t taps = (int64_t)ksize * ksize * ksize;
diff --git a/pixie_amd/csrc/unet_exec.hip b/pixie_amd/csrc/unet_exec.hip
--- a/pixie_amd/csrc/unet_exec.hip
+++ b/pixie_amd/csrc/unet_exec.hip
@@ -206,6 +206,13 @@
     template <class T> T* ptr(int64_t off) const { return reinterpret_cast<T*>(base + off); }
 };
 
+struct TileStats {
+    Arena* arena; int64_t off; pixie_conv_desc desc;
+    TileStats(Arena* a, int64_t bytes) : arena(a), off(a->alloc(bytes)) {}
+    ~TileStats() { arena->release(off); }
+    float* p() const { return arena->ptr<float>(off); }
+};
+
 struct Exec;
 struct Tens {
     Exec* ex = nullptr;
@@ -216,6 +223,8 @@
     bool has_sums = false;
     double* sums = nullptr;
     uint32_t* slot = nullptr;
+    bool has_slot = false;
+    std::shared_ptr<TileStats> pending;
     int64_t spatial() const { return (int64_t)d * h * w; }
     ~Tens();
 };
@@ -288,12 +297,6 @@
         if (!dry && slot_next >= slot_cap) fail("pixie_unet_forward: out of |x|max slots (internal sizing error)");
         return dry ? (slot_next++, nullptr) : slots + slot_next++;
     }
-    struct Scratch {
-        Exec* ex; int64_t off;
-        Scratch(Exec* e, int64_t bytes) : ex(e), off(e->arena.alloc(bytes)) {}
-        ~Scratch() { ex->arena.release(off); }
-        template <class T> T* as() const { return ex->arena.ptr<T>(off); }
-    };
 
     const float* P(const std::string& key) {
         const Param& p = net->param(key);
@@ -338,13 +341,24 @@
         return (float)(std::sqrt((double)count) * (double)b.wmax + (double)b.bmax + 1e-30);
     }
 
+    struct Scratch {
+        Exec* ex; int64_t off;
+        Scratch(Exec* e, int64_t bytes) : ex(e), off(e->arena.alloc(bytes)) {}
+        ~Scratch() { ex->arena.release(off); }
+        template <class T> T* as() const { return ex->arena.ptr<T>(off); }
+    };
     void stats(const TP& t) {
+        if (t->pending) {
+            if (!dry) ok(pixie_stats_finalize(t->pending->p(), &t->pending->desc, t->sums, stream), "pixie_stats_finalize");
+            t->pending.reset();
+        }
         if (t->has_sums) return;
         t->has_sums = true;
         if (!dry && zsum_next + 2 * t->c > zsum_cap) fail("pixie_unet_forward: out of statistics space (internal sizing error)");
         t->sums = dry ? nullptr : zsums + zsum_next;
         zsum_next += 2 * t->c;
         t->slot = new_slot();
+        t->has_slot = true;
         if (!dry) ok(channel_stats_prezeroed(t->p, t->c, t->spatial(), t->sums, t->slot, as_stream(stream)), "pixie_channel_stats");
     }
     struct AB { std::shared_ptr<Scratch> mem; float* a; float* b; };
@@ -357,6 +371,20 @@
         if (!dry) ok(pixie_norm_finalize(sums, c, spatial, mode, groups, 1e-5, w, b, r.a, r.b, stream), "pixie_norm_finalize");
         return r;
     }
+
+    AB norm_of(const TP& t, int64_t spatial, int mode, int groups, const float* w, const float* b) {
+        if (!t->pending) { stats(t); return norm_finalize(t->sums, t->c, spatial, mode, groups, w, b); }
+        AB r;
+        const int cpad = (t->c + 63) / 64 * 64;
+        r.mem = std::make_shared<Scratch>(this, (int64_t)(cpad + t->c) * sizeof(float));
+        r.a = r.mem->as<float>();
+        r.b = r.a + cpad;
+        if (!dry) ok(pixie_stats_norm_finalize(t->pending->p(), &t->pending->desc, t->sums, spatial, mode, groups, 1e-5, w, b, r.a, r.b, stream),
+                     "pixie_stats_norm_finalize");
+        t->pending.reset();
+        return r;
+    }
+    void amax(const TP& t) { if (!t->has_slot) stats(t); }
 
     bool f16_ok(const std::vector<TP>& parts, int stride) const {
         int cin = 0;
@@ -397,7 +425,7 @@
         }
         const bool f16 = f16_ok(parts, o.stride);
         const bool raw = !o.pro && o.affine_store.empty();
-        if (f16 && raw) for (auto& t : parts) stats(t);
+        if (f16 && raw) for (auto& t : parts) amax(t);
 
         TP out = o.out_ptr ? external(o.out_ptr, cout, od, oh, ow) : make(cout, od, oh, ow);
         desc.d_in0 = x0->p; desc.c0 = x0->c;
@@ -436,7 +464,8 @@
         } else {
             desc.in_bound = o.bound;
         }
-        std::unique_ptr<Scratch> workspace, tile_stats;
+        std::unique_ptr<Scratch> workspace;
+        std::shared_ptr<TileStats> tile_stats;
         if (dry) { desc.d_w16 = reinterpret_cast<const void*>(0x100); }
         if (net->split_k) {
             const int64_t wsb = pixie_conv_workspace_bytes(&desc);
@@ -447,11 +476,21 @@
             uint32_t* slot = new_slot();
             const int64_t nfl = pixie_conv_stats_floats(&desc);
             if (nfl > 0) {
-                tile_stats.reset(new Scratch(this, nfl * (int64_t)sizeof(float)));
-                desc.d_out_stats = tile_stats->as<float>();
+                tile_stats = std::make_shared<TileStats>(&arena, nfl * (int64_t)sizeof(float));
+                desc.d_out_stats = tile_stats->p();
                 desc.d_out_amax = slot;
                 have_stats = true;
                 out->slot = slot;
+                out->has_slot = true;
+            } else if (workspace) {
+                if (!dry && zsum_next + 2 * cout > zsum_cap) fail("pixie_unet_forward: out of statistics space (internal sizing error)");
+                out->sums = dry ? nullptr : zsums + zsum_next;
+                zsum_next += 2 * cout;
+                out->slot = slot;
+                out->has_slot = true;
+                out->has_sums = true;
+                desc.d_split_sums = out->sums;
+                desc.d_split_amax = slot;
             }
         }
         if (!dry) ok(pixie_conv3d_forward(&desc, stream), "pixie_conv3d_forward");
@@ -459,14 +498,15 @@
             out->sums_off = arena.alloc((int64_t)cout * 2 * sizeof(double));
             out->sums = arena.ptr<double>(out->sums_off);
             out->has_sums = true;
-            if (!dry) ok(pixie_stats_finalize(desc.d_out_stats, &desc, out->sums, stream), "pixie_stats_finalize");
+            tile_stats->desc = desc;
+            out->pending = tile_stats;
         }
         return out;
     }
 
     AB norm_finalize_parts(const std::vector<TP>& parts, int64_t spatial) {
+        if (parts.size() == 1) return norm_of(parts[0], spatial, 0, 1, nullptr, nullptr);
         for (auto& t : parts) stats(t);
-        if (parts.size() == 1) return norm_finalize(parts[0]->sums, parts[0]->c, spatial, 0, 1, nullptr, nullptr);
         const int c0 = parts[0]->c, c1 = parts[1]->c, c = c0 + c1;
         AB r;
         const int cpad = (c + 63) / 64 * 64;
@@ -483,14 +523,13 @@
         AB pro = norm_finalize_parts(parts, spatial);
         ConvOpt o1; o1.pro = &pro; o1.affine_store = p + ".in_layers.0"; o1.act = ACT_LEAKY; o1.bound = norm_bound(p + ".in_layers.0", spatial);
         TP h = conv(parts, p + ".in_layers.2", b.cout, 3, o1);
-        stats(h);
-        AB pro2 = norm_finalize(h->sums, b.cout, spatial, 0, 1, nullptr, nullptr);
+        AB pro2 = norm_of(h, spatial, 0, 1, nullptr, nullptr);
         TP skip = parts[0];
         ConvOpt o2; o2.pro = &pro2; o2.affine_store = p + ".out_layers.0"; o2.act = ACT_LEAKY; o2.bound = norm_bound(p + ".out_layers.0", spatial);
         if (b.cin != b.cout) {
             if (net->fold_skip && f16_ok({h}, 1) && f16_ok(parts, 1) && skip_foldable(h, b.cout, 3, parts)) {
                 skip.reset();
-                for (auto& t : parts) stats(t);
+                for (auto& t : parts) amax(t);
                 o2.skip_parts = &parts; o2.skip_key = p + ".skip_connection";
             } else {
                 skip = conv(parts, p + ".skip_connection", b.cout, 1, ConvOpt{});
@@ -503,8 +542,7 @@
         const std::string& p = b.prefix;
         const int c = x->c;
         const int64_t spatial = x->spatial();
-        stats(x);
-        AB pro = norm_finalize(x->sums, c, spatial, 1, 32, P(p + ".norm.weight"), P(p + ".norm.bias"));
+        AB pro = norm_of(x, spatial, 1, 32, P(p + ".norm.weight"), P(p + ".norm.bias"));
         ConvOpt o; o.pro = &pro; o.bound = norm_bound(p + ".norm", spatial * (c / 32));
         TP qkv = conv({x}, p + ".qkv", 3 * c, 1, o);
         TP att = make(c, x->d, x->h, x->w);
@@ -538,23 +576,19 @@
             if (!hid) {
                 const int g = std::max(c.cond_dim / 2, 1);
                 x = conv({external(d_feat, c.feature_channels, D, H, W)}, q + "0", c.cond_dim, 1, ConvOpt{});
-                stats(x);
-                pro_in = norm_finalize(x->sums, c.cond_dim, spatial, 1, g, P(q + "1.weight"), P(q + "1.bias"));
+                pro_in = norm_of(x, spatial, 1, g, P(q + "1.weight"), P(q + "1.bias"));
                 act_in = ACT_SILU;
                 bound_in = norm_bound(q + "1", spatial * (c.cond_dim / g));
             } else {
                 if (d_proj0) x = external(d_proj0, hid, D, H, W);
                 else x = conv({external(d_feat, c.feature_channels, D, H, W)}, q + "0", hid, 1, ConvOpt{});
-                stats(x);
-                AB pro = norm_finalize(x->sums, hid, spatial, 1, 32, P(q + "1.weight"), P(q + "1.bias"));
+                AB pro = norm_of(x, spatial, 1, 32, P(q + "1.weight"), P(q + "1.bias"));
                 ConvOpt o; o.pro = &pro; o.act = ACT_SILU; o.bound = norm_bound(q + "1", spatial * (hid / 32));
                 x = conv({x}, q + "3", hid, 3, o);
-                stats(x);
-                AB pro2 = norm_finalize(x->sums, hid, spatial, 1, 32, P(q + "4.weight"), P(q + "4.bias"));
+                AB pro2 = norm_of(x, spatial, 1, 32, P(q + "4.weight"), P(q + "4.bias"));
                 ConvOpt o2; o2.pro = &pro2; o2.act = ACT_SILU; o2.bound = norm_bound(q + "4", spatial * (hid / 32));
                 x = conv({x}, q + "6", c.cond_dim, 1, o2);
-                stats(x);
-                pro_in = norm_finalize(x->sums, c.cond_dim, spatial, 1, 32, P(q + "7.weight"), P(q + "7.bias"));
+                pro_in = norm_of(x, spatial, 1, 32, P(q + "7.weight"), P(q + "7.bias"));
                 bound_in = norm_bound(q + "7", spatial * std::max(c.cond_dim / 32, 1));
             }
             pro_in_p = &pro_in;
@@ -586,8 +620,7 @@
             }
             h = parts[0];
         }
-        stats(h);
-        AB pro = norm_finalize(h->sums, h->c, h->spatial(), 0, 1, nullptr, nullptr);
+        AB pro = norm_of(h, h->spatial(), 0, 1, nullptr, nullptr);
         ConvOpt oo; oo.pro = &pro; oo.affine_store = "unet.out.0"; oo.act = ACT_LEAKY; oo.bound = norm_bound("unet.out.0", h->spatial());
         oo.out_ptr = d_out;
         return conv({h}, "unet.out.2", c.out_channels, 3, oo);
diff --git a/pixie_amd/unet.py b/pixie_amd/unet.py
--- a/pixie_amd/unet.py
+++ b/pixie_amd/unet.py
@@ -31,7 +31,7 @@
 def fill_conv_desc(lib, alloc, parts: Sequence[torch.Tensor], packed_w, bias, cout: int, ksize: int, *, stride: int = 1,
                    upsample: bool = False, pro=None, affine=None, act: int = 0, residual=None, w16=None, in_amax=None,
                    in_bound: float = 0.0, out_amax=None, out_size=None, skip=None, subpixel: bool = False, split_k: bool = True,
-                   addr=_addr):
+                   addr=_addr, split_sums=None):
     x0 = parts[0]
     x1 = parts[1] if len(parts) > 1 else None
     cin0, d, h, w = x0.shape
@@ -88,7 +88,22 @@
             stats = alloc((nfl,), torch.float32)
             desc.d_out_stats = addr(stats)
             desc.d_out_amax = addr(out_amax)
+        elif workspace is not None and split_sums is not None:
+            stats = split_sums(cout)
+            desc.d_split_sums = addr(stats)
+            desc.d_split_amax = addr(out_amax)
     return desc, out, stats, workspace
+
+
+class PendingStats:
+
+    def __init__(self, ops, stats, desc, cout):
+        self.ops, self.stats, self.desc, self.cout = ops, stats, desc, cout
+
+    def finalize(self) -> torch.Tensor:
+        sums = torch.empty((self.cout, 2), device=self.ops.device, dtype=torch.float64)
+        check(self.ops.lib.pixie_stats_finalize(_ptr(self.stats), C.byref(self.desc), _ptr(sums), self.ops.stream), "pixie_stats_finalize")
+        return sums
 
 
 class HipOps:
@@ -99,6 +114,7 @@
         self.device = device
         self.lib = _lib.load()
         self.split_k = os.environ.get("PIXIE_CONV_SPLIT_K", "1") != "0"
+        self.fold_stats = True
         self.record_variant = False
         self.last_variant = (0, 1)
 
@@ -149,19 +165,23 @@
              residual: Optional[torch.Tensor] = None, w16: Optional[torch.Tensor] = None,
              in_amax: Optional[Sequence[torch.Tensor]] = None, in_bound: float = 0.0,
              out_amax: Optional[torch.Tensor] = None, out_size: Optional[Tuple[int, int, int]] = None,
-             skip: Optional[dict] = None, subpixel: bool = False):
+             skip: Optional[dict] = None, subpixel: bool = False, lazy_stats: bool = False, split_stats: bool = False):
         desc, out, stats, _ = fill_conv_desc(
             self.lib, lambda shape, dtype: torch.empty(shape, device=self.device, dtype=dtype), parts, packed_w, bias, cout, ksize,
             stride=stride, upsample=upsample, pro=pro, affine=affine, act=act, residual=residual, w16=w16, in_amax=in_amax,
-            in_bound=in_bound, out_amax=out_amax, out_size=out_size, skip=skip, subpixel=subpixel, split_k=self.split_k)
+            in_bound=in_bound, out_amax=out_amax, out_size=out_size, skip=skip, subpixel=subpixel, split_k=self.split_k,
+            split_sums=(lambda c: torch.zeros((c, 2), device=self.device, dtype=torch.float64)) if split_stats else None)
         sums = None
         if self.record_variant:
             sl = C.c_int(1)
             self.last_variant = (int(_lib.load(diag=True).pixie_conv_kernel_variant(C.byref(desc), C.byref(sl))), int(sl.value))
         check(self.lib.pixie_conv3d_forward(C.byref(desc), self.stream), "pixie_conv3d_forward")
         if desc.d_out_stats:
-            sums = torch.empty((cout, 2), device=self.device, dtype=torch.float64)
-            check(self.lib.pixie_stats_finalize(_ptr(stats), C.byref(desc), _ptr(sums), self.stream), "pixie_stats_finalize")
+            sums = PendingStats(self, stats, desc, cout)
+            if not lazy_stats:
+                sums = sums.finalize()
+        elif desc.d_split_sums:
+            sums = stats
         if out_amax is not None:
             return out, sums
         return out
@@ -199,6 +219,16 @@
         check(self.lib.pixie_norm_finalize(_ptr(sums), c, spatial, mode, groups, eps, _ptr(weight), _ptr(bias), _ptr(a), _ptr(b),
                                            self.stream), "pixie_norm_finalize")
         return a, b
+
+    def stats_norm_finalize(self, pending: PendingStats, spatial: int, mode: int, groups: int = 1, eps: float = 1e-5,
+                            weight: Optional[torch.Tensor] = None, bias: Optional[torch.Tensor] = None):
+        c = pending.cout
+        sums = torch.empty((c, 2), device=self.device, dtype=torch.float64)
+        a = torch.empty(c, device=self.device, dtype=torch.float32)
+        b = torch.empty(c, device=self.device, dtype=torch.float32)
+        check(self.lib.pixie_stats_norm_finalize(_ptr(pending.stats), C.byref(pending.desc), _ptr(sums), spatial, mode, groups, eps,
+                                                 _ptr(weight), _ptr(bias), _ptr(a), _ptr(b), self.stream), "pixie_stats_norm_finalize")
+        return sums, (a, b)
 
     def attention(self, qkv: torch.Tensor, channels: int, tokens: int) -> torch.Tensor:
         out = torch.empty((channels, tokens), device=self.device, dtype=torch.float32)
@@ -303,13 +333,25 @@
                 self._remember(cache, t, self.ops.channel_stats(t, slot), slot)
             else:
                 self._remember(cache, t, self.ops.channel_sums(t), None)
+        sums, slot = cache[k]
+        if isinstance(sums, PendingStats):
+            self._remember(cache, t, sums.finalize(), slot)
         return cache[k]
 
     def _sums(self, cache: dict, t: torch.Tensor) -> torch.Tensor:
         return self._stats(cache, t)[0]
 
     def _amax(self, cache: dict, t: torch.Tensor) -> torch.Tensor:
-        return self._stats(cache, t)[1]
+        ent = cache.get(id(t))
+        return ent[1] if ent is not None and ent[1] is not None else self._stats(cache, t)[1]
+
+    def _norm(self, cache: dict, t: torch.Tensor, spatial: int, mode: int, **kw):
+        ent = cache.get(id(t))
+        if ent is not None and isinstance(ent[0], PendingStats):
+            sums, ab = self.ops.stats_norm_finalize(ent[0], spatial, mode, **kw)
+            self._remember(cache, t, sums, ent[1])
+            return ab
+        return self.ops.norm_finalize(self._sums(cache, t), spatial, mode, **kw)
 
     def _conv(self, cache: dict, parts: List[torch.Tensor], wkey: str, cout: int, ksize: int, *, stride: int = 1,
               upsample: bool = False, pro=None, affine_key: Optional[str] = None, act: int = ACT_NONE,
@@ -333,7 +375,8 @@
         if self.fuse_stats:
             slot = self._new_slot(cache, parts[0].device)
             out, sums = ops.conv(parts, None, self._b(wkey), cout, ksize, stride=stride, upsample=upsample, pro=pro, affine=affine,
-                                 act=act, residual=residual, w16=self._w16(wkey, sub), out_amax=slot, **kw)
+                                 act=act, residual=residual, w16=self._w16(wkey, sub), out_amax=slot, **kw,
+                                 **({"lazy_stats": True, "split_stats": True} if getattr(ops, "fold_stats", False) else {}))
             if sums is not None:
                 self._remember(cache, out, sums, slot)
             return out
@@ -343,11 +386,13 @@
     def _res(self, b: Block, parts: List[torch.Tensor], cache: dict) -> torch.Tensor:
         ops, p = self.ops, b.prefix
         spatial = parts[0][0].numel()
-        sums = torch.cat([self._sums(cache, t) for t in parts], dim=0) if len(parts) > 1 else self._sums(cache, parts[0])
-        pro = ops.norm_finalize(sums, spatial, 0)
+        if len(parts) > 1:
+            pro = ops.norm_finalize(torch.cat([self._sums(cache, t) for t in parts], dim=0), spatial, 0)
+        else:
+            pro = self._norm(cache, parts[0], spatial, 0)
         h = self._conv(cache, parts, p + ".in_layers.2", b.cout, 3, pro=pro, affine_key=p + ".in_layers.0", act=ACT_LEAKY,
                        bound=self._norm_bound(p + ".in_layers.0", spatial))
-        pro2 = ops.norm_finalize(self._sums(cache, h), spatial, 0)
+        pro2 = self._norm(cache, h, spatial, 0)
         fold = None
         if b.cin != b.cout:
             if (self.fold_skip and self._f16x3 and ops.f16x3_ok([h], 1) and ops.f16x3_ok(parts, 1)
@@ -366,8 +411,7 @@
         ops, p = self.ops, b.prefix
         c = x.shape[0]
         spatial = x[0].numel()
-        pro = ops.norm_finalize(self._sums(cache, x), spatial, 1, groups=32, weight=self.p[p + ".norm.weight"],
-                                bias=self.p[p + ".norm.bias"])
+        pro = self._norm(cache, x, spatial, 1, groups=32, weight=self.p[p + ".norm.weight"], bias=self.p[p + ".norm.bias"])
         qkv = self._conv(cache, [x], p + ".qkv", 3 * c, 1, pro=pro, bound=self._norm_bound(p + ".norm", spatial * (c // 32)))
         att = ops.attention(qkv.reshape(3 * c, spatial), c, spatial).reshape(x.shape)
         return self._conv(cache, [att], p + ".proj_out", c, 1, residual=x)
@@ -395,24 +439,23 @@
             if cfg.projector_hidden is None:
                 g = max(cfg.cond_dim // 2, 1)
                 x = self._conv(cache, [x], q + "0", cfg.cond_dim, 1)
-                pro_in = ops.norm_finalize(self._sums(cache, x), spatial, 1, groups=g,
-                                           weight=self.p[q + "1.weight"], bias=self.p[q + "1.bias"])
+                pro_in = self._norm(cache, x, spatial, 1, groups=g, weight=self.p[q + "1.weight"], bias=self.p[q + "1.bias"])
                 act_in = ACT_SILU
                 bound_in = self._norm_bound(q + "1", spatial * (cfg.cond_dim // g))
             else:
                 hid = cfg.projector_hidden
                 x = proj0 if proj0 is not None else self._conv(cache, [x], q + "0", hid, 1)
-                pro = ops.norm_finalize(self._sums(cache, x), spatial, 1, groups=32, weight=self.p[q + "1.weight"], bias=self.p[q + "1.bias"])
+                pro = self._norm(cache, x, spatial, 1, groups=32, weight=self.p[q + "1.weight"], bias=self.p[q + "1.bias"])
                 x = self._conv(cache, [x], q + "3", hid, 3, pro=pro, act=ACT_SILU, bound=self._norm_bound(q + "1", spatial * (hid // 32)))
-                pro = ops.norm_finalize(self._sums(cache, x), spatial, 1, groups=32, weight=self.p[q + "4.weight"], bias=self.p[q + "4.bias"])
+                pro = self._norm(cache, x, spatial, 1, groups=32, weight=self.p[q + "4.weight"], bias=self.p[q + "4.bias"])
                 x = self._conv(cache, [x], q + "6", cfg.cond_dim, 1, pro=pro, act=ACT_SILU, bound=self._norm_bound(q + "4", spatial * (hid // 32)))
-                pro_in = ops.norm_finalize(self._sums(cache, x), spatial, 1, groups=32, weight=self.p[q + "7.weight"], bias=self.p[q + "7.bias"])
+                pro_in = self._norm(cache, x, spatial, 1, groups=32, weight=self.p[q + "7.weight"], bias=self.p[q + "7.bias"])
                 bound_in = self._norm_bound(q + "7", spatial * max(cfg.cond_dim // 32, 1))
         first = self.plan.input_blocks[0][0]
         return self._conv(cache, [x], first.prefix, first.cout, 3, pro=pro_in, act=act_in, bound=bound_in)
 
     def _head(self, h: torch.Tensor, cache: dict) -> torch.Tensor:
-        pro = self.ops.norm_finalize(self._sums(cache, h), h[0].numel(), 0)
+        pro = self._norm(cache, h, h[0].numel(), 0)
         return self._conv(cache, [h], "unet.out.2", self.cfg.out_channels, 3, pro=pro, affine_key="unet.out.0", act=ACT_LEAKY,
                           bound=self._norm_bound("unet.out.0", h[0].numel()))
 
```

Result: slower. 23.19 million voxels/s (-4.4%).
